# n00b001/neuro-genetic-pong-self-play

Hardware: AMD Instinct MI355X
Metric: env-steps/sec (GA evaluation loop, self-play) + generations/sec at pop=65536 per GPU (higher is better)
Workload: dtype f32 hidden + certified f64 argmax; genomes f64

## Files before the change

### include/pong_ga.h

```cpp
#ifndef PONG_GA_H
#define PONG_GA_H

#include <stddef.h>
#include <stdint.h>

#ifdef __cplusplus
extern "C" {
#endif

#define PG_ABI_VERSION 13
#define PG_MAX_NODES 9

typedef enum pg_status {
  PG_OK = 0,
  PG_ERR_INVALID = -1,
  PG_ERR_HIP = -2,
  PG_ERR_UNSUPPORTED = -3
} pg_status;

typedef enum pg_dtype { PG_F32 = 0, PG_F64 = 1 } pg_dtype;

typedef enum pg_activation {
  PG_ACT_SIGMOID = 0,
  PG_ACT_RELU = 1
} pg_activation;

typedef enum pg_opp_kind {
  PG_OPP_HARDCODED = 0,
  PG_OPP_ROM_CPU = 1,
  PG_OPP_SCORE = 2,
  PG_OPP_NN = 3
} pg_opp_kind;

typedef enum pg_precision {
  PG_PREC_CERTIFIED = 0,
  PG_PREC_F64 = 1
} pg_precision;

typedef enum pg_kernel {
  PG_KERNEL_AUTO = 0,
  PG_KERNEL_GENERAL = 1,
  PG_KERNEL_RESIDENT = 2,
  PG_KERNEL_SPLIT = 3      ,
  PG_KERNEL_WIDE = 4,
  PG_KERNEL_STAGED = 5,
  PG_KERNEL_RELU = 6
} pg_kernel;

typedef enum pg_prep {
  PG_PREP_ALL = 0,
  PG_PREP_GENOMES = 1,
  PG_PREP_REST = 2
} pg_prep;

typedef struct pg_net {
  int32_t n_nodes;
  int32_t nodes[PG_MAX_NODES];
  int32_t bias;
  int32_t dtype;
  int32_t activation;
} pg_net;

typedef struct pg_eval_args {
  uint32_t struct_size;
  pg_net net;
  int32_t n_genomes;
  int32_t n_games;
  const void *genomes;
  int64_t genome_stride;
  const void *opponents;
  int64_t opponent_stride;
  int32_t n_opponents;
  int32_t precision;
  const int32_t *game_kind;
  const int32_t *game_opp;
  const double *game_mult;
  uint64_t seed;
  double *fitness;
  double *rewards;
  int32_t *scores;
  int32_t *frames;
  double *total_frames;
  int32_t *status;
  uint64_t *counters;
  uint8_t *trace;
  int32_t trace_games;
  int32_t trace_cap;
  int32_t kernel;
  int32_t group_lanes;
  void *workspace;
  size_t workspace_bytes;
  uint32_t *hard_log;
  int32_t hard_cap;
  const int32_t *genome_rows;
  const int32_t *n_active;
  int32_t prep;
  int32_t horizon;
  int32_t timeout_thresh;
  int32_t win_score;
} pg_eval_args;


typedef struct pg_forward_args {
  pg_net net;
  int32_t n;
  const void *genomes;
  int64_t genome_stride;
  const int32_t *genome_index;
  const double *x;
  int32_t precision;
  int32_t *index;
  double *act;
  uint64_t *counters;
  double *z_all;
  double *h_all;
} pg_forward_args;

typedef struct pg_decide_args {
  pg_net net;
  int32_t n;
  const void *genomes;
  int64_t genome_stride;
  const int32_t *genome_index;
  const int32_t *k;
  int32_t *index;
  int32_t *stage;
} pg_decide_args;

typedef struct pg_wide_decide_args {
  pg_net net;
  int32_t n;
  const void *genomes;
  int64_t genome_stride;
  const int32_t *genome_index;
  const int32_t *k;
  int32_t *index;
  double *act;
  void *workspace;
  size_t workspace_bytes;
} pg_wide_decide_args;

typedef struct pg_relu_decide_args {
  pg_net net;
  int32_t n;
  const void *genomes;
  int64_t genome_stride;
  const int32_t *genome_index;
  const int32_t *k;
  int32_t *index;
  int32_t *stage;
  float *z32;
  float *bound;
} pg_relu_decide_args;

enum {
  PG_S_BALL_X = 0, PG_S_BALL_Y, PG_S_BALL_VX, PG_S_BALL_VY, PG_S_BALL_VISIBLE,
  PG_S_SERVE_TIMER, PG_S_SERVE_DIR, PG_S_HITS, PG_S_POINT, PG_S_LEFT_Y, PG_S_RIGHT_Y,
  PG_S_SCORE1, PG_S_SCORE2, PG_S_ONE_PLAYER, PG_S_SEED_LO, PG_S_SEED_HI,
  PG_STATE_FIELDS
};

typedef struct pg_ga_args {
  int32_t n;
  int64_t genes;
  int32_t dtype;
  const void *parents;
  int64_t stride;
  int32_t n_parents;
  const int32_t *chosen;
  void *offspring;
  uint8_t *invalid;
  double cxpb, mutpb;
  double alpha;
  double mu, sigma, indpb;
  uint64_t seed;
  uint64_t generation;
  const uint8_t *pair_mask;
  const int32_t *pair_list;
  const int32_t *pair_count;
  int32_t pair_cap;
} pg_ga_args;

typedef struct pg_select_args {
  int32_t n_pop;
  int32_t k;
  int32_t tournsize;
  const double *fitness;
  int32_t *chosen;
  uint64_t seed;
  uint64_t generation;
} pg_select_args;

typedef enum pg_schedule_mode {
  PG_SCHED_REFERENCE = 0,
  PG_SCHED_SELFPLAY = 1
} pg_schedule_mode;

typedef struct pg_schedule_args {
  int32_t mode;
  int32_t n;
  int32_t n_games;
  int64_t row_offset;
  int32_t n_hof;
  const double *hof_fitness;
  uint64_t seed;
  uint64_t generation;
  int32_t *kind;
  int32_t *opp;
  double *mult;
  const int32_t *rows;
  int32_t hof_slices;
  int32_t block_rows;
  int32_t slice_local;
} pg_schedule_args;

typedef struct pg_hof_args {
  int32_t maxsize;
  int32_t hof_n;
  const double *hof_fitness;
  const uint64_t *hof_hash;
  int32_t pop_n;
  const double *pop_fitness;
  const uint64_t *pop_hash;
  const int32_t *rank;
  int32_t *new_n;
  int32_t *new_src;
  double *new_fitness;
} pg_hof_args;

typedef struct pg_hof_packed_args {
  int32_t maxsize;
  int32_t hof_n;
  const double *hof_fitness;
  int32_t k;
  const int64_t *packed;
  int32_t *new_n;
  int32_t *new_src;
  double *new_fitness;
  const int32_t *slot_in;
  int32_t *slot_out;
} pg_hof_packed_args;
int32_t pg_hof_update_packed(const pg_hof_packed_args *args);

typedef struct pg_hof_rank_args {
  int32_t hof_n;
  const double *hof_fitness;
  const uint64_t *hof_hash;
  int32_t k;
  const double *cand_fitness;
  const uint64_t *cand_hash;
  int64_t *packed;
  void *workspace;
  size_t workspace_bytes;
} pg_hof_rank_args;

typedef struct pg_hof_prepare_args {
  const double *fitness;
  int32_t pop_n;
  int32_t filter;
  double worst;
  const void *rows;
  int64_t stride;
  int64_t genes;
  int32_t dtype;
  int32_t hof_n;
  const double *hof_fitness;
  const uint64_t *hof_hash;
  int32_t *k;
  int64_t *cand;
  uint64_t *hashes;
  int64_t *packed;
  void *workspace;
  size_t workspace_bytes;
} pg_hof_prepare_args;

const char *pg_version(void);
int32_t pg_abi_version(void);
int32_t pg_build_flags(void);
const char *pg_last_error(void);
int32_t pg_device_count(void);
size_t pg_eval_workspace_bytes(const pg_eval_args *args);
int32_t pg_gene_count(const pg_net *net);

int32_t pg_eval_population(const pg_eval_args *args, void *stream);
int32_t pg_forward(const pg_forward_args *args, void *stream);
int32_t pg_decide(const pg_decide_args *args, void *stream);
size_t pg_wide_decide_workspace_bytes(const pg_wide_decide_args *args);
int32_t pg_wide_decide(const pg_wide_decide_args *args, void *stream);
int32_t pg_relu_decide(const pg_relu_decide_args *args, void *stream);
int32_t pg_physics_reset(int32_t *state, int32_t n, const uint64_t *seeds,
                         const int32_t *one_player, void *stream);
int32_t pg_physics_step(int32_t *state, int32_t n, const uint8_t *actions, void *stream);
int32_t pg_ga_select_tournament(const pg_select_args *args, void *stream);
int32_t pg_ga_select_tournament_ranked(const pg_select_args *args, const double *sorted_fitness,
                                       const int32_t *order, void *stream);
int32_t pg_ga_vary(const pg_ga_args *args, void *stream);
int32_t pg_ga_mark_pairs(uint8_t *pair_mask, int32_t n_pairs, const int32_t *rows, int32_t n_rows,
                         int32_t skip_lo, int32_t skip_hi, const uint8_t *exclude, void *stream);
int32_t pg_ga_list_pairs(const uint8_t *pair_mask, int32_t n_pairs, int32_t *list, int32_t *count, void *stream);
int32_t pg_ga_schedule(const pg_schedule_args *args, void *stream);
int32_t pg_row_hash(const void *rows, int64_t stride, const int32_t *index, int32_t n, int64_t genes,
                    int32_t dtype, uint64_t *hash, void *stream);
int32_t pg_hof_update(const pg_hof_args *args);
size_t pg_hof_rank_classes_workspace_bytes(int32_t n);
int32_t pg_hof_rank_classes(const pg_hof_rank_args *args, void *stream);
size_t pg_hof_prepare_workspace_bytes(int32_t hof_n, int32_t pop_n);
int32_t pg_hof_prepare(const pg_hof_prepare_args *args, void *stream);

typedef struct pg_scatter_args {
  int32_t n;
  int32_t n_games;
  int32_t row_lo;
  const double *fitness;
  const int32_t *frames;
  const int32_t *rows;
  const int32_t *n_active;
  double *shard_fitness;
  float *lineage;
} pg_scatter_args;
int32_t pg_ga_scatter_fitness(const pg_scatter_args *args, void *stream);

typedef struct pg_merge_args {
  int32_t pop_n;
  const double *fitness;
  const uint8_t *invalid;
  const double *inherited;
  double *new_fitness;
  int32_t filter;
  double worst;
  int32_t *cand;
  double *cand_fitness;
  double *summary;
  void *workspace;
  size_t workspace_bytes;
} pg_merge_args;
size_t pg_ga_merge_workspace_bytes(int32_t pop_n);
int32_t pg_ga_merge_fitness(const pg_merge_args *args, void *stream);

size_t pg_ga_select_workspace_bytes(int32_t n_pop);
int32_t pg_ga_select_ranked(const pg_select_args *args, void *workspace, size_t workspace_bytes, void *stream);

int32_t pg_ga_inherit(const int32_t *chosen, int32_t n, const double *fitness, double *inherited,
                      const float *lineage_in, float *lineage_out, void *stream);

size_t pg_ga_order_workspace_bytes(int32_t n);
int32_t pg_ga_order(int32_t n, int32_t row_lo, const uint8_t *invalid, const float *lineage, int32_t by_length,
                    int32_t *rows, int32_t *count, void *workspace, size_t workspace_bytes, void *stream);

typedef struct pg_hof_cand_args {
  int32_t hof_n;
  const double *hof_fitness;
  const uint64_t *hof_hash;
  int32_t k;
  const int32_t *cand;
  const double *cand_fitness;
  const void *rows;
  int64_t stride;
  int64_t genes;
  int32_t dtype;
  uint64_t *cand_hash;
  int64_t *packed;
  void *workspace;
  size_t workspace_bytes;
} pg_hof_cand_args;
size_t pg_hof_prepare_cand_workspace_bytes(int32_t hof_n, int32_t k);
int32_t pg_hof_prepare_cand(const pg_hof_cand_args *args, void *stream);

typedef struct pg_hof_commit_args {
  void *dst;
  int64_t dst_stride;
  const void *old_rows;
  int64_t old_stride;
  const void *rows;
  int64_t rows_stride;
  const int32_t *cand;
  const int32_t *src;
  int32_t n_old;
  int32_t m;
  int64_t genes;
  int32_t dtype;
  const uint64_t *old_hash;
  const uint64_t *cand_hash;
  uint64_t *new_hash;
  const double *fitness_in;
  double *new_fitness;
  const int32_t *dst_slot;
} pg_hof_commit_args;
int32_t pg_hof_commit(const pg_hof_commit_args *args, void *stream);

int32_t pg_gather_rows(void *dst, int64_t dst_stride, const void *old_rows, int64_t old_stride, const void *rows,
                       int64_t rows_stride, const int64_t *index, const int32_t *src, int32_t n_old, int32_t n,
                       int64_t genes, int32_t dtype, void *stream);
int32_t pg_render_frames(const int32_t *state, int32_t n, uint8_t *frames, void *stream);
int32_t pg_find_stuff(const uint8_t *frames, int64_t frame_stride, int32_t n, double *out, void *stream);

#ifdef __cplusplus
}
#endif
#endif
```

### neuro-genetic-pong-self-play_amd/csrc/pg_cascade.hpp

```cpp
#pragma once

#include <hip/hip_runtime.h>
#include <stdint.h>

#include "pg_device.hpp"
#include "pg_eval.hpp"
#include "pg_f64math.h"

namespace pg {

#ifndef PG_SLOW_INLINE
#define PG_SLOW_INLINE __forceinline__
#endif
#ifndef PG_LOAD_BATCH
#define PG_LOAD_BATCH 2
#endif
#ifndef PG_RES_WAVES
#define PG_RES_WAVES 0
#endif
#if PG_RES_WAVES > 0
#define PG_RES_BOUNDS __launch_bounds__(256, PG_RES_WAVES)
#else
#define PG_RES_BOUNDS __launch_bounds__(256)
#endif
// ... 211 lines not shown

template <int U, int O>
__device__ __forceinline__ void load_rec_out(NetP<U, O> &n, const float *__restrict__ r) {
  constexpr int P = NetP<U, O>::P;
  constexpr int F = rec_floats<U, O>();
  constexpr int B = P * 14 / 4 * 4;
  constexpr int D = P * 14 - B;
  const float4 *s = reinterpret_cast<const float4 *>(r + B);
  float v[F - B];
#pragma unroll
  for (int q = 0; q < (F - B) / 4; ++q) {
    const float4 x = s[q];
    v[4 * q] = x.x;
    v[4 * q + 1] = x.y;
    v[4 * q + 2] = x.z;
    v[4 * q + 3] = x.w;
  }
#pragma unroll
  for (int p = 0; p < P; ++p)
#pragma unroll
    for (int o = 0; o < O; ++o) n.w2[p][o] = float2v{v[D + (p * O + o) * 2], v[D + (p * O + o) * 2 + 1]};
#pragma unroll
  for (int o = 0; o < O; ++o) n.c[o] = v[D + P * O * 2 + o];
  n.e = v[D + P * O * 2 + O];
  n.ct = make_cert(n.e);
}

template <int U, int O>
__device__ __forceinline__ void load_rec(NetP<U, O> &n, const float *__restrict__ r) {
  constexpr int P = NetP<U, O>::P;
  constexpr int F = rec_floats<U, O>();
  const float4 *s = reinterpret_cast<const float4 *>(r);
  float v[F];
#pragma unroll
  for (int q = 0; q < F / 4; ++q) {
    const float4 x = s[q];
    v[4 * q] = x.x;
    v[4 * q + 1] = x.y;
    v[4 * q + 2] = x.z;
    v[4 * q + 3] = x.w;
  }
#pragma unroll
  for (int p = 0; p < P; ++p)
#pragma unroll
    for (int i = 0; i < 7; ++i) n.w1[p][i] = float2v{v[(p * 7 + i) * 2], v[(p * 7 + i) * 2 + 1]};
#pragma unroll
  for (int p = 0; p < P; ++p)
#pragma unroll
    for (int o = 0; o < O; ++o) n.w2[p][o] = float2v{v[P * 14 + (p * O + o) * 2], v[P * 14 + (p * O + o) * 2 + 1]};
#pragma unroll
  for (int o = 0; o < O; ++o) n.c[o] = v[P * 14 + P * O * 2 + o];
  n.e = v[P * 14 + P * O * 2 + O];
  n.ct = make_cert(n.e);
}

template <int U, int O, bool kBiasIn = false>
__device__ __forceinline__ void partial_pk(const NetP<U, O> &n, const int k[6], float acc[O]) {
  constexpr int P = NetP<U, O>::P;
  float2v kx[6];
#pragma unroll
  for (int i = 0; i < 6; ++i) {
    const float f = (float)k[i];
    kx[i] = float2v{f, f};
  }
  float2v a2[O];
#pragma unroll
  for (int o = 0; o < O; ++o) a2[o] = kBiasIn ? float2v{n.c[o], n.c[o]} : float2v{0.f, 0.f};
#pragma unroll
  for (int p = 0; p < P; p += 2) {
    constexpr int kStep = 2;
    const bool two = p + 1 < P;
    float2v a = n.w1[p][6], b = two ? n.w1[p + 1][6] : float2v{0.f, 0.f};
#pragma unroll
    for (int i = 0; i < 6; ++i) {
      a = __builtin_elementwise_fma(n.w1[p][i], kx[i], a);
      if (two) b = __builtin_elementwise_fma(n.w1[p + 1][i], kx[i], b);
    }
    const float2v qa = float2v{__builtin_amdgcn_exp2f(a.x), __builtin_amdgcn_exp2f(a.y)} + 1.0f;
    const float2v qb = float2v{__builtin_amdgcn_exp2f(b.x), __builtin_amdgcn_exp2f(b.y)} + 1.0f;
    const float2v sa = float2v{__builtin_amdgcn_rcpf(qa.x), __builtin_amdgcn_rcpf(qa.y)};
    const float2v sb = float2v{__builtin_amdgcn_rcpf(qb.x), __builtin_amdgcn_rcpf(qb.y)};
#pragma unroll
    for (int o = 0; o < O; ++o) {
      a2[o] = __builtin_elementwise_fma(n.w2[p][o], sa, a2[o]);
      if (two) a2[o] = __builtin_elementwise_fma(n.w2[p + 1][o], sb, a2[o]);
    }
    (void)kStep;
  }
#pragma unroll
  for (int o = 0; o < O; ++o) acc[o] = a2[o].x + a2[o].y;
}

template <int HL, int U, int O>
__device__ __forceinline__ float frame_bound_wave(const float *__restrict__ rec, const int k[6], int lane64) {
  constexpr int P = NetP<U, O>::P;
  constexpr int F = rec_floats<U, O>();
  constexpr float kOR = (float)out_roundings<HL, U>();
  float acc[O];
#pragma unroll
  for (int o = 0; o < O; ++o) acc[o] = 0.f;
#pragma unroll 1
  for (int t = lane64; t < HL * 2 * P; t += 64) {
    const int hl = t % HL, u = t / HL, p = u >> 1, h = u & 1;
    const float *r = rec + hl * F;
    float w[7];
#pragma unroll
// ... 516 lines not shown
```

### neuro-genetic-pong-self-play_amd/csrc/pg_eval.hpp

```cpp
#pragma once

#include <hip/hip_runtime.h>
#include <stdint.h>

#include "../../include/pong_ga.h"
#include "pg_device.hpp"

namespace pg {

int32_t fail(int32_t code, const char *fmt, ...);

#define PG_HIP(call)                                                                  \
  do {                                                                                \
    hipError_t e_ = (call);                                                           \
    if (e_ != hipSuccess)                                                             \
      return fail(PG_ERR_HIP, "%s failed: %s", #call, hipGetErrorString(e_));        \
  } while (0)

struct EvalParams {
  const void *genomes;
  const void *opponents;
  const int32_t *rows;
  const int32_t *n_active;
  const int32_t *kind;
  const int32_t *opp;
  const double *mult;
  double *rewards;
  int32_t *scores;
  int32_t *frames;
  double *total_frames;
  int32_t *status_game;
  uint64_t *counters;
  uint8_t *trace;
  uint32_t *hard_log;
  int hard_cap;
  unsigned int *work;
  int64_t gstride, ostride;
  uint64_t seed;
  int n_genomes, n_games, total, n_opponents;
  int trace_games, trace_cap;
  int nodes[PG_MAX_NODES];
  int n_nodes, bias, max_width;
  float *recs;
  int horizon;
  int timeout_thresh;
  int win_score;
  int prep;
  void *wide_scratch;
  int wide_w3_resident;
  const int32_t *wide_probe_k;
  int32_t *wide_probe_index;
  double *wide_probe_act;
  int activation;
};

__device__ inline int active_genomes(const EvalParams &p) {
  if (!p.n_active) return p.n_genomes;
  const int a = __builtin_amdgcn_readfirstlane(*p.n_active);
  return a < 0 ? 0 : (a < p.n_genomes ? a : p.n_genomes);
}
__device__ inline int active_total(const EvalParams &p) {
  return p.n_active ? active_genomes(p) * p.n_games : p.total;
}

__device__ inline int genome_row(const EvalParams &p, int i) { return p.rows ? p.rows[i] : i; }

template <class S>
__device__ inline double episode_reward(const S &st, int total, double mult, int &zero_div) {
  zero_div = 0;
  if (st.s1 == st.s2) return 0.0;
  const double tf = (double)total;
  if (tf == 0.0) {
    zero_div = 1;
    return __builtin_nan("");
  }
  const double diff = (double)(st.s2 - st.s1);
  const double bonus = __dmul_rn((double)st.s2, mult);
  return __dadd_rn(diff, bonus) / (tf / 100.0);
}

template <class S>
__device__ inline void finish_game(const EvalParams &p, int w, const S &st, int frames, int total) {
  int zero_div;
  const double reward = episode_reward(st, total, p.mult[w], zero_div);
  p.rewards[w] = reward;
  p.scores[2 * w] = st.s1;
  p.scores[2 * w + 1] = st.s2;
  p.frames[w] = frames;
  p.total_frames[w] = (double)total;
  p.status_game[w] = zero_div;
}

__device__ inline double feat64(int k) { return __dmul_rn(0.5, (double)k) / 160.0; }
__device__ inline double feat64_flip(int k) { return (160.0 - __dmul_rn(0.5, (double)k)) / 160.0; }


int num_cus();

__device__ inline void log_hard_raw(uint32_t *hard_log, uint64_t *counters, int hard_cap, int row, int is_opp, int idx,
                                    int source, const int k[6]) {
  if (!hard_log || !counters) return;
  const unsigned long long r = atomicAdd((unsigned long long *)&counters[9], 1ull);
  if (r >= (unsigned long long)hard_cap) return;
  uint32_t *rec = hard_log + r * 8;
  rec[0] = (uint32_t)row;
  rec[1] = (uint32_t)(is_opp & 1) | ((uint32_t)(idx & 255) << 8) | ((uint32_t)(source & 255) << 16);
  for (int i = 0; i < 6; ++i) rec[2 + i] = (uint32_t)k[i];
}
__device__ inline void log_hard(const EvalParams &p, int row, int is_opp, int idx, int source, const int k[6]) {
  log_hard_raw(p.hard_log, p.counters, p.hard_cap, row, is_opp, idx, source, k);
}

struct DecideParams {
  const void *genomes;
  const int32_t *gidx;
  const int32_t *k;
  int32_t *index;
  int32_t *stage;
  int64_t gstride;
  int n, H, b;
};
int32_t launch_decide(const DecideParams &p, int L, int O, bool f64, size_t lds, hipStream_t s);

bool wide_shape_ok(const pg_net &n, int n_games);
size_t wide_workspace_bytes(const pg_eval_args *a);
int32_t launch_wide(const EvalParams &p, int dtype, void *scratch, hipStream_t s);

bool relu_shape_ok(const pg_net &n);
int32_t launch_relu(const EvalParams &p, int dtype, hipStream_t s);


}
```

### neuro-genetic-pong-self-play_amd/csrc/pg_gen.hip

```cpp
#include <hip/hip_runtime.h>

#include <algorithm>

#include <rocprim/device/device_radix_sort.hpp>

#include "pg_eval.hpp"


namespace pg {
namespace {

constexpr int kT = 256;
constexpr int kChunk = 8 * kT;
inline unsigned blocks(long n, int per = kT) { return (unsigned)((n + per - 1) / per); }
inline size_t align_up(size_t x) { return (x + 255) & ~size_t(255); }

__global__ void k_scatter_fitness(pg_scatter_args a) {
  const int i = blockIdx.x * kT + threadIdx.x;
  if (i >= a.n) return;
  const int played = a.n_active ? __builtin_amdgcn_readfirstlane(*a.n_active) : a.n;
  const int row = a.rows ? a.rows[i] : a.row_lo + i;
  const bool p = i < played;
  a.shard_fitness[row - a.row_lo] = p ? a.fitness[i] : 0.0;
  if (p && a.lineage) {
    int m = 0;
    for (int g = 0; g < a.n_games; ++g) m = max(m, a.frames[(long)i * a.n_games + g]);
    a.lineage[row] = (float)m;
  }
}

struct Part {
  double n, mean, m2, mn, mx;
  int32_t nan, nevals, cand, pad;
};

__device__ inline void chan(double &n, double &mean, double &m2, double nb, double meanb, double m2b) {
  if (nb == 0.0) return;
  if (n == 0.0) {
    n = nb, mean = meanb, m2 = m2b;
    return;
  }
  const double t = n + nb, d = meanb - mean;
  mean += d * (nb / t);
  m2 += m2b + d * d * (n * nb / t);
  n = t;
}

__device__ inline void part_merge(Part &x, const Part &y) {
  chan(x.n, x.mean, x.m2, y.n, y.mean, y.m2);
  x.mn = fmin(x.mn, y.mn);
  x.mx = fmax(x.mx, y.mx);
  x.nan |= y.nan;
  x.nevals += y.nevals;
  x.cand += y.cand;
}

__device__ inline bool is_cand(const pg_merge_args &a, double f) { return !a.filter || f > a.worst; }

__device__ inline double merged(const pg_merge_args &a, int i) {
// ... 206 lines not shown
    packed[hn + j] = (int64_t)(uint32_t)rank | ((int64_t)cls << 32);
    return;
  }
  packed[e] = (int64_t)(uint32_t)rank | ((int64_t)cls << 32);
}

unsigned table_cap(int n) {
  unsigned c = 64;
  while (c < 2u * (unsigned)(n > 0 ? n : 1)) c <<= 1;
  return c;
}

struct CandLayout {
  size_t mt, ct, sort_keys, sort_vals, sort_temp, total, temp_bytes;
  unsigned mcap, ccap;
};

int32_t cand_layout(int hn, int k, CandLayout *L) {
  size_t tb = 0;
  if (rocprim::radix_sort_pairs(nullptr, tb, (const double *)nullptr, (double *)nullptr, (const int32_t *)nullptr,
                                (int32_t *)nullptr, (unsigned)(k > 0 ? k : 1)) != hipSuccess)
    return fail(PG_ERR_HIP, "hof_prepare_cand: rocPRIM storage query failed");
  L->mcap = table_cap(hn);
  L->ccap = table_cap(k);
  size_t off = 0;
  auto take = [&](size_t b) {
    const size_t at = off;
    off += align_up(b);
    return at;
  };
  L->mt = take((size_t)(L->mcap + 1) * sizeof(Slot));
  L->ct = take((size_t)(L->ccap + 1) * sizeof(Slot));
  const size_t kk = (size_t)(k > 0 ? k : 1);
  L->sort_keys = take(kk * 8 * 2);
  L->sort_vals = take(kk * 4 * 2);
  L->temp_bytes = tb > 0 ? tb : 1;
  L->sort_temp = take(L->temp_bytes);
  L->total = off;
  return PG_OK;
}

__global__ void k_iota(int32_t *v, int n) {
  const int i = blockIdx.x * kT + threadIdx.x;
  if (i < n) v[i] = i;
}

__global__ void k_cand_keys(const double *f, int k, double *keys, int32_t *iota) {
  const int i = blockIdx.x * kT + threadIdx.x;
  if (i >= k) return;
  keys[i] = f[i] + 0.0;
  iota[i] = i;
}

template <typename WT>
__global__ __launch_bounds__(256) void k_hof_commit(WT *dst, int64_t dst_stride, const WT *old_rows, int64_t old_stride,
                                                    const WT *rows, int64_t rows_stride, const int32_t *cand,
                                                    const int32_t *src, int m, int n_old, int64_t genes,
                                                    const uint64_t *old_hash, const uint64_t *cand_hash,
                                                    uint64_t *new_hash, const double *fit_in, double *new_fitness,
                                                    const int32_t *dst_slot) {
  const int lane = threadIdx.x & 63;
  for (int j = blockIdx.x * 4 + (threadIdx.x >> 6); j < m; j += gridDim.x * 4) {
    const int s = src[j];
    if (!dst_slot || s >= n_old) {
      const WT *from = s < n_old ? old_rows + (long)s * old_stride : rows + (long)cand[s - n_old] * rows_stride;
      WT *to = dst + (long)(dst_slot ? dst_slot[j] : j) * dst_stride;
      for (int64_t g = lane; g < genes; g += 64) to[g] = from[g];
    }
    if (lane == 0) {
      new_hash[j] = s < n_old ? old_hash[s] : cand_hash[s - n_old];
      new_fitness[j] = fit_in[j];
    }
  }
}

}
}

using namespace pg;

extern "C" {

int32_t pg_ga_scatter_fitness(const pg_scatter_args *a, void *stream) {
  if (!a) return fail(PG_ERR_INVALID, "args is NULL");
  if (a->n < 0 || a->n_games < 1 || a->row_lo < 0 || (a->n > 0 && (!a->fitness || !a->shard_fitness)) ||
      (a->n > 0 && a->lineage && !a->frames))
    return fail(PG_ERR_INVALID, "ga_scatter_fitness: bad sizes or NULL buffers");
  if (a->n == 0) return PG_OK;
  hipLaunchKernelGGL(k_scatter_fitness, dim3(blocks(a->n)), dim3(kT), 0, (hipStream_t)stream, *a);
  PG_HIP(hipGetLastError());
  return PG_OK;
}

size_t pg_ga_merge_workspace_bytes(int32_t pop_n) {
  if (pop_n < 0) return 0;
  const size_t nb = blocks(pop_n > 0 ? pop_n : 1, kChunk);
  return align_up(nb * sizeof(Part)) + align_up(nb * sizeof(int32_t));
}

int32_t pg_ga_merge_fitness(const pg_merge_args *a, void *stream) {
  if (!a) return fail(PG_ERR_INVALID, "args is NULL");
  const int n = a->pop_n;
  if (n < 0 || !a->summary || (n > 0 && (!a->fitness || !a->new_fitness || !a->cand || !a->cand_fitness)) ||
      (n > 0 && a->invalid && !a->inherited))
    return fail(PG_ERR_INVALID, "ga_merge_fitness: bad sizes or NULL buffers");
  const size_t need = pg_ga_merge_workspace_bytes(n);
  if (!a->workspace || a->workspace_bytes < need)
    return fail(PG_ERR_INVALID, "ga_merge_fitness: workspace of %zu bytes needed", need);
  const unsigned nb = blocks(n > 0 ? n : 1, kChunk);
  Part *parts = (Part *)a->workspace;
  int32_t *offsets = (int32_t *)((char *)a->workspace + align_up(nb * sizeof(Part)));
  const hipStream_t s = (hipStream_t)stream;
  hipLaunchKernelGGL(k_merge_partials, dim3(nb), dim3(kT), 0, s, *a, parts);
  hipLaunchKernelGGL(k_merge_finish, dim3(1), dim3(64), 0, s, *a, (const Part *)parts, (int)nb, offsets);
  hipLaunchKernelGGL(k_merge_compact, dim3(nb), dim3(kT), 0, s, *a, (const int32_t *)offsets);
  PG_HIP(hipGetLastError());
  return PG_OK;
}

size_t pg_ga_select_workspace_bytes(int32_t n_pop) {
// ... 65 lines not shown
  hipLaunchKernelGGL(k_order_keys, dim3(blocks(n)), dim3(kT), 0, s, (int)n, (int)row_lo, invalid, lineage,
                     (int)by_length, keys, vals, count);
  PG_HIP(rocprim::radix_sort_pairs(temp, tb, keys, keys_out, vals, rows, (unsigned)n, 0, 32, s));
  return PG_OK;
}

size_t pg_hof_prepare_cand_workspace_bytes(int32_t hof_n, int32_t k) {
  CandLayout L;
  if (hof_n < 0 || k < 0 || cand_layout(hof_n, k, &L) != PG_OK) return 0;
  return L.total;
}

int32_t pg_hof_prepare_cand(const pg_hof_cand_args *a, void *stream) {
  if (!a) return fail(PG_ERR_INVALID, "args is NULL");
  const int hn = a->hof_n, k = a->k;
  if (hn < 0 || k < 0 || (long)hn + k > 0x7fffffffL || (hn > 0 && (!a->hof_fitness || !a->hof_hash)) ||
      (k > 0 && (!a->cand || !a->cand_fitness || !a->rows || !a->cand_hash || !a->packed)) || a->genes < 0 ||
      (k > 0 && a->stride < a->genes) || (a->dtype != PG_F32 && a->dtype != PG_F64))
    return fail(PG_ERR_INVALID, "hof_prepare_cand: bad sizes, dtype or NULL buffers");
  if (k == 0) return PG_OK;
  CandLayout L;
  if (cand_layout(hn, k, &L) != PG_OK) return PG_ERR_HIP;
  if (!a->workspace || a->workspace_bytes < L.total)
    return fail(PG_ERR_INVALID, "hof_prepare_cand: workspace of %zu bytes needed", L.total);
  char *ws = (char *)a->workspace;
  const hipStream_t s = (hipStream_t)stream;
  const int32_t rc = pg_row_hash(a->rows, a->stride, a->cand, k, a->genes, a->dtype, a->cand_hash, stream);
  if (rc != PG_OK) return rc;
  Slot *mt = (Slot *)(ws + L.mt), *ct = (Slot *)(ws + L.ct);
  PG_HIP(hipMemsetAsync(ws + L.mt, 0xFF, L.ct + (size_t)(L.ccap + 1) * sizeof(Slot) - L.mt, s));
  hipLaunchKernelGGL(k_hof_insert, dim3(blocks(hn + k)), dim3(kT), 0, s, a->hof_hash, hn, mt, L.mcap,
                     a->cand_hash, k, ct, L.ccap);
  double *keys = (double *)(ws + L.sort_keys), *sorted = keys + k;
  int32_t *iota = (int32_t *)(ws + L.sort_vals), *order = iota + k;
  hipLaunchKernelGGL(k_cand_keys, dim3(blocks(k)), dim3(kT), 0, s, a->cand_fitness, k, keys, iota);
  size_t tb = L.temp_bytes;
  PG_HIP(rocprim::radix_sort_pairs(ws + L.sort_temp, tb, (const double *)keys, sorted, iota, order, (unsigned)k, 0, 64,
                                   s));
  hipLaunchKernelGGL(k_hof_rank_pack, dim3(blocks(hn + k)), dim3(kT), 0, s, a->hof_fitness,
                     a->hof_hash, hn, a->cand_fitness, a->cand_hash, k,
                     (const double *)sorted, (const int32_t *)order, (const Slot *)mt, L.mcap, (const Slot *)ct,
                     L.ccap, a->packed);
  PG_HIP(hipGetLastError());
  return PG_OK;
}

int32_t pg_hof_commit(const pg_hof_commit_args *a, void *stream) {
  if (!a) return fail(PG_ERR_INVALID, "args is NULL");
  if (a->m < 0 || a->n_old < 0 || a->genes < 0 || (a->dtype != PG_F32 && a->dtype != PG_F64) ||
      (a->m > 0 && (!a->dst || !a->src || !a->new_hash || !a->fitness_in || !a->new_fitness)) ||
      (a->m > 0 && a->n_old > 0 && ((!a->old_rows && !a->dst_slot) || !a->old_hash)) ||
      (a->m > 0 && (!a->rows || !a->cand || !a->cand_hash)))
    return fail(PG_ERR_INVALID, "hof_commit: bad sizes, dtype or NULL buffers");
  if (a->m == 0) return PG_OK;
  const hipStream_t s = (hipStream_t)stream;
  const dim3 grid((unsigned)std::min<int64_t>(((int64_t)a->m + 3) / 4, 2048));
  if (a->dtype == PG_F64)
    hipLaunchKernelGGL(k_hof_commit<double>, grid, dim3(256), 0, s, (double *)a->dst, a->dst_stride,
                       (const double *)a->old_rows, a->old_stride, (const double *)a->rows, a->rows_stride, a->cand,
                       a->src, (int)a->m, a->n_old, a->genes, a->old_hash, a->cand_hash,
                       a->new_hash, a->fitness_in, a->new_fitness, a->dst_slot);
  else
    hipLaunchKernelGGL(k_hof_commit<float>, grid, dim3(256), 0, s, (float *)a->dst, a->dst_stride,
                       (const float *)a->old_rows, a->old_stride, (const float *)a->rows, a->rows_stride, a->cand,
                       a->src, (int)a->m, a->n_old, a->genes, a->old_hash, a->cand_hash,
                       a->new_hash, a->fitness_in, a->new_fitness, a->dst_slot);
  PG_HIP(hipGetLastError());
  return PG_OK;
}

}
```

### neuro-genetic-pong-self-play_amd/csrc/pg_service.hpp

```cpp
#pragma once

#include <hip/hip_runtime.h>

#include "../../include/pong_ga.h"
#include "pg_cascade.hpp"
#include "pg_device.hpp"
#include "pg_eval.hpp"
#include "pg_f64math.h"

namespace pg {

#ifndef PG_SVC_PRIO
#define PG_SVC_PRIO 3
#endif
#ifndef PG_SVC_BATCH
#define PG_SVC_BATCH 1
#endif

#ifndef PG_INLINE_SVC
#define PG_INLINE_SVC 1
#endif
#ifndef PG_INLINE_PRIO
#define PG_INLINE_PRIO 3
#endif
// ... 48 lines not shown
  uint64_t st_t = __builtin_amdgcn_s_memtime();
  const auto stage_mark = [&](int i) {
    asm volatile("s_waitcnt vmcnt(0) lgkmcnt(0)" ::: "memory");
    const uint64_t now = __builtin_amdgcn_s_memtime();
    st_acc[i] += now - st_t;
    st_acc[6 + i] += 1;
    st_t = now;
  };
#define PG_STAGE(i) stage_mark(i)
#else
#define PG_STAGE(i)
#endif
  int d = PG_INLINE_FRAME_BOUND ? -1 : plateau_decide<O>(zf, r.e, lane64);
  PG_STAGE(0);
  if (d >= 0) PG_LOG_REQ(1, d);
  if (PG_INLINE_FRAME_BOUND && d < 0 && r.e < __builtin_inff()) {
    const float ef = fminf(r.e, frame_bound_wave<HL, U, O>(r.rec, r.kr, lane64));
#ifdef PG_INLINE_LOG
    ef_log = ef;
#endif
    PG_STAGE(1);
    d = certify_c<O>(zf, make_cert(ef));
    if (d < 0) d = plateau_f32<O>(zf, ef);
    if (d < 0) d = plateau_decide<O>(zf, ef, lane64);
    PG_STAGE(2);
    if (d >= 0) {
      PG_LOG_REQ(2, d);
      return d | 1024;
    }
  }
  if (d < 0) {
    d = fast_f64_decide<O, WT>(g, H, b, r.k, lane64);
    PG_STAGE(3);
    if (d >= 0) PG_LOG_REQ(3, d);
  }
  if (d >= 0) return d | 512;
  d = forward_f64_group<64, (U * HL + 63) / 64, O, WT>(g, H, b, r.k, lds, lane64);
  PG_LOG_REQ(4, d);
  PG_STAGE(4);
#undef PG_LOG_REQ
#undef PG_STAGE
#if defined(PG_INLINE_LOG) || defined(PG_SERVE_STAGES)
  if (false) {
#else
  if (p.hard_log && lane64 == 0) {
#endif
    const long oo = g - (const WT *)p.opponents;
    const bool opp = p.opponents != p.genomes && oo >= 0 && oo < (long)p.n_opponents * p.ostride;
    log_hard(p, (int)(opp ? oo / p.ostride : (g - (const WT *)p.genomes) / p.gstride), opp ? 1 : 0, d, 0, r.k);
  }
  return d | 256;
}

template <int L, int U, int O, typename WT>
__global__ __launch_bounds__(256) void k_prep_records(EvalParams p) {
  constexpr int HL = L / 2;
  constexpr int F = rec_floats<U, O>();
  if (p.prep != PG_PREP_GENOMES && blockIdx.x == 0) {
    if (threadIdx.x < 64) p.work[threadIdx.x] = 0u;
    if (p.counters && threadIdx.x < 16) p.counters[threadIdx.x] = 0ull;
  }
  const long t = (long)blockIdx.x * 256 + threadIdx.x;
  const long net = t / HL + (p.prep == PG_PREP_REST ? p.n_genomes : 0);
  const int hl = (int)(t % HL);
  const long end = p.prep == PG_PREP_GENOMES ? (long)p.n_genomes : (long)p.n_genomes + p.n_opponents;
  if (net >= end) return;
  const WT *g;
  int flip;
  if (net < p.n_genomes) {
    if (net >= active_genomes(p)) return;
    g = (const WT *)p.genomes + (long)genome_row(p, (int)net) * p.gstride;
    flip = 0;
  } else {
    g = (const WT *)p.opponents + (net - p.n_genomes) * p.ostride;
    flip = 1;
  }
  NetP<U, O> n;
  load_net_pk<HL, U, O, WT>(n, g, p.nodes[1], p.bias, hl, flip);
  store_rec<U, O>(n, p.recs + (net * HL + hl) * F);
}

#ifdef PG_PROBE_EXTRA
template <int M>
__device__ __forceinline__ void pg_probe_extra(float2v w, float2v w2, float a, float b, float &v, float2v &pp,
                                               int &sv) {
#pragma unroll
  for (int r = 0; r < (M == 4 || M == 9 ? 48 : (M <= 2 ? 16 : 24)); ++r) {
    if constexpr (M == 1) asm volatile("v_rcp_f32 %0, %1" : "=v"(v) : "v"((r & 1) ? a : b));
    if constexpr (M == 2) asm volatile("v_exp_f32 %0, %1" : "=v"(v) : "v"((r & 1) ? a : b));
    if constexpr (M == 3) asm volatile("v_pk_fma_f32 %0, %1, %2, %3" : "=v"(pp) : "v"(w), "v"(w2), "v"((r & 1) ? w : w2));
    if constexpr (M == 4) asm volatile("v_fma_f32 %0, %1, %2, %3" : "=v"(v) : "v"(a), "v"(b), "v"((r & 1) ? a : b));
    if constexpr (M == 5) asm volatile("v_add_u32 %0, %1, %2" : "=v"(v) : "v"(a), "v"(b));
    if constexpr (M == 7) asm volatile("v_mov_b32 %0, %1" : "=v"(v) : "v"((r & 1) ? a : b));
    if constexpr (M == 8) asm volatile("v_pk_add_f32 %0, %1, %2" : "=v"(pp) : "v"(w), "v"((r & 1) ? w : w2));
    if constexpr (M == 9) asm volatile("v_add_f32 %0, %1, %2" : "=v"(v) : "v"(a), "v"((r & 1) ? a : b));
  }
}
#endif

template <int L, int U, int O, typename WT, bool kUntraced = false, bool kHorizon = false>
__global__ __launch_bounds__(svc_threads<U>()) void k_service(EvalParams p) {
  constexpr int kSvcThreads = svc_threads<U>();
  constexpr bool kInline = inline_service<L, U, kHorizon>();
  static_assert(!kInline || O <= 4, "InlineReq.z");
  constexpr int kSvcGameWaves = kSvcThreads / 64 - (kInline ? 0 : 1);
  constexpr int HL = L / 2;
  constexpr int kSlots = kSvcGameWaves * (64 / L) * 2;
  __shared__ SlowSlot slots[kSlots];
  __shared__ HorizonSlot hz[kHorizon ? kSlots / 2 : 1];
  __shared__ int waves_done;
  __shared__ int posted;
  __shared__ uint32_t serve_tab[kServeTabSlots * kServeTabPoints];
  extern __shared__ double lds_svc[];
  const int H = p.nodes[1];
  const int b = p.bias;
  const int wave = threadIdx.x >> 6;
  const int lane64 = threadIdx.x & 63;
  for (int i = threadIdx.x; i < kSlots; i += kSvcThreads) {
    lds_st(&slots[i].flag, 0);
    slots[i].rec = 0;
  }
  const bool tabbed = p.n_games <= kServeTabSlots;
  if (tabbed)
    for (int i = threadIdx.x; i < p.n_games * kServeTabPoints; i += kSvcThreads)
      serve_tab[i] = Pong::serve_entry(game_seed(p.seed, i / kServeTabPoints), i % kServeTabPoints);
  if (threadIdx.x == 0) {
    lds_st(&waves_done, 0);
    lds_st(&posted, 0);
  }
  __syncthreads();

  if (!kInline && wave == kSvcGameWaves) {
// ... 123 lines not shown
    tend = 0x7fffffff;
    fstart = 0x3fffffff;
    fresh = false;
  };
  if (kInline && !live) park();
  int w_scripted = 1, w_onep = 1;
  int top = 1;
#ifdef PG_PROBE_EXTRA
  float probe_v = 0.f;
  float2v probe_p = float2v{0.f, 0.f};
  int probe_s = 0;
#endif
#ifdef PG_START_PROBE
  uint64_t probe_fresh = 0;
  const uint64_t probe_t0 = __builtin_amdgcn_s_memtime();
#endif
#ifdef PG_SERVE_STAGES
  uint64_t st_acc[24];
#pragma unroll
  for (int i = 0; i < 24; ++i) st_acc[i] = 0;
#endif
#ifdef PG_DECIDE_PROBE
  uint64_t probe_dec = 0;
  const uint64_t probe_t0 = __builtin_amdgcn_s_memtime();
#endif
#ifdef PG_TIMELINE
  uint64_t t_start = 0;
  uint32_t g_fails = 0, g_slow = 0;
#endif
#ifdef PG_PATH_PROBE
  uint32_t pp_frames = 0, pp_rally = 0, pp_face = 0, pp_fail = 0, pp_hidden = 0;
#define PG_PP(cnt, cond) \
  if (__builtin_amdgcn_ballot_w64(cond) != 0) cnt += 1
#else
#define PG_PP(cnt, cond)
#endif
  if (kInline ? __builtin_amdgcn_ballot_w64(live) != 0 : live) for (;;) {
#ifdef PG_START_PROBE
    const bool any_fresh = __builtin_amdgcn_ballot_w64(fresh) != 0;
    const uint64_t probe_f0 = __builtin_amdgcn_s_memtime();
#endif
    PG_PP(pp_frames, true);
    sframe += 1;
#ifdef PG_TIMELINE
    constexpr bool kJumps = !kHorizon;
#else
    const bool kJumps = !kHorizon && (kUntraced || p.trace == nullptr);
#endif
    if (top) {
    if (fresh) {
      const int i = w / p.n_games;
      const int g = w - i * p.n_games;
      kind = p.kind[w];
      const WT *gr = genomes + (long)genome_row(p, i) * p.gstride;
      const bool nn = side && kind == kOppNN && p.n_opponents > 0;
      const int oj = nn ? min(max(p.opp[w], 0), p.n_opponents - 1) : 0;
      gm = nn ? opponents + (long)oj * p.ostride : gr;
      const int rec = nn ? p.n_genomes + oj : i;
      load_rec<U, O>(net, p.recs + ((long)rec * HL + hl) * rec_floats<U, O>());
      const int sx = slot_me();
      if (kInline && hl == 0) slots[sx].rec = rec;
#pragma unroll
      for (int o = 0; o < O; ++o) net.c[o] = hl == 0 ? 0.5f * net.c[o] : 0.f;
      st.reset(0, kind == kOppRomCpu);
      if (kHorizon || !tabbed) st.seed = game_seed(p.seed, g);
      tab_off = g * kServeTabPoints;
      act_r = act_l = total = 0;
      c_vis = kVisByFrames ? sframe - 1 : 0;
      fstart = sframe - 1;
      tend = sframe + p.timeout_thresh;
      fresh = false;
      if (hl == 0) slots[sx].n_memo = 0;
      if (lig == 0) slots[sx].rally_at = -1;
      if (kHorizon && lig == 0) {
        const int gx = threadIdx.x / L;
        hz[gx].sum = 0.0;
        hz[gx].eps = hz[gx].s1 = hz[gx].s2 = hz[gx].zd = 0;
      }
#ifdef PG_TIMELINE
      t_start = wall_clock64();
      g_fails = g_slow = 0;
#endif
    }
#ifdef PG_START_PROBE
    if (any_fresh) probe_fresh += __builtin_amdgcn_s_memtime() - probe_f0;
#endif
#ifndef PG_NO_HIDDEN_JUMP
    {
      const bool hid = !st.vis && st.timer >= 2;
      PG_PP(pp_hidden, hid);
      if (kJumps && hid) {
        const int h = st.timer - 1;
        st.rc2 = PongK::drift2(st.rc2, h);
        if (!st.one_player) st.lc2 = PongK::drift2(st.lc2, h);
        st.timer = 1;
        act_r = clamp_move(st.rc2, 0);
        act_l = clamp_move(st.lc2, 0);
        fstart -= h;
        tend -= h;
        hidden += h;
      }
    }
#endif
    w_scripted = __builtin_amdgcn_readfirstlane(__builtin_amdgcn_ballot_w64(kind != kOppNN) != 0);
    w_onep = __builtin_amdgcn_readfirstlane(__builtin_amdgcn_ballot_w64(st.one_player != 0) != 0);
    top = 0;
    }
    const int pvis = st.vis, pbx2 = st.bx2, pby2 = st.by2;
#ifdef PG_PATH_PROBE
    const int pt_b = st.point, hits_b = st.hits;
#endif
    const int ev = st.step(act_r, act_l, [&](int pt) {
// ... 27 lines not shown
      if (PG_ANY(code == -1)) {
      if (code == -1) {
        fails += 1;
#ifdef PG_TIMELINE
        g_fails += 1;
#endif
#ifndef PG_NO_TIGHT
        int mv = tight_gap_move<O>(z, net.e, net.ct);
        if (mv == -1)
#else
        int mv = -1;
#endif
        {
          const int idx = plateau_f32<O>(z, net.e);
          mv = idx >= 0 ? index_to_move(idx) : -1;
        }
        inwave += mv != -1 ? 1 : 0;
        code = mv;
      }
#ifdef PG_ABLATE_SERVE
      if (code == -1) code = z[1] > z[0] ? 6 : -6;
#endif
      if (kInline && PG_ANY(code == -1)) {
        uint64_t key = 0;
        int nm = 0;
        const int sx = slot_me();
        if (code == -1) {
          key = memo_key(k);
          nm = slots[sx].n_memo;
          int hit = -1;
#pragma unroll 1
          for (int c = 0; c < kMemo && c < nm; ++c)
            if (slots[sx].memo_key[c] == key) hit = slots[sx].memo_idx[c];
          code = hit;
        }
        const int kn[6] = {side ? 320 - bx2 : bx2, by2, side ? 320 - lbx2 : lbx2, lby2, side ? lc2 : rc2,
                           side ? rc2 : lc2};
        const float my_e = net.e;
        uint64_t need = __builtin_amdgcn_ballot_w64(code == -1 && hl == 0);
        if (need) {
#ifdef PG_DECIDE_PROBE
        const uint64_t probe_d0 = __builtin_amdgcn_s_memtime();
#endif
        if constexpr (PG_INLINE_PRIO > 0) __builtin_amdgcn_s_setprio(PG_INLINE_PRIO);
#pragma unroll 1
        do {
          const int src = (int)__builtin_ctzll(need);
          need &= need - 1;
          InlineReq r;
#pragma unroll
          for (int i = 0; i < 6; ++i) r.k[i] = __builtin_amdgcn_readlane(kn[i], src);
#pragma unroll
          for (int i = 0; i < 6; ++i) r.kr[i] = __builtin_amdgcn_readlane(k[i], src);
          r.rec = p.recs + (long)__builtin_amdgcn_readlane(slots[sx].rec, src) * HL * rec_floats<U, O>();
#pragma unroll
          for (int o = O; o < 4; ++o) r.z[o] = 0.f;
#pragma unroll
          for (int o = 0; o < O; ++o) r.z[o] = __int_as_float(__builtin_amdgcn_readlane(__float_as_int(z[o]), src));
          r.e = __int_as_float(__builtin_amdgcn_readlane(__float_as_int(my_e), src));
          const uint64_t ga = (uint64_t)gm;
          const WT *g = (const WT *)(((uint64_t)__builtin_amdgcn_readlane((int)(ga >> 32), src) << 32) |
                                     (uint32_t)__builtin_amdgcn_readlane((int)(uint32_t)ga, src));
#if defined(PG_SERVE_TWICE)
          serve_inline<U, HL, O, WT>(p, g, r, lds_svc + wave * f64_lds_doubles(H, O), lane64, st_acc);
          const int ans = serve_inline<U, HL, O, WT>(p, g, r, lds_svc + wave * f64_lds_doubles(H, O), lane64, st_acc + 12);
#elif defined(PG_SERVE_STAGES)
          const int ans = serve_inline<U, HL, O, WT>(p, g, r, lds_svc + wave * f64_lds_doubles(H, O), lane64, st_acc);
#else
          const int ans = serve_inline<U, HL, O, WT>(p, g, r, lds_svc + wave * f64_lds_doubles(H, O), lane64);
#endif
          if ((lane64 & ~(HL - 1)) == src) {
            slow += (ans >> 8) & 1;
            plateau += (ans >> 9) & 1;
            inwave += ans >> 10;
            code = index_to_move(ans & 255);
            if (hl == 0) {
              const int c = nm % kMemo;
              slots[sx].memo_key[c] = key;
              slots[sx].memo_idx[c] = code;
              slots[sx].n_memo = nm + 1;
            }
          }
        } while (need);
        if constexpr (PG_INLINE_PRIO > 0) __builtin_amdgcn_s_setprio(0);
        {
#if defined(PG_RELOAD_ALL)
          load_rec<U, O>(net, p.recs + ((long)slots[sx].rec * HL + hl) * rec_floats<U, O>());
#elif !defined(PG_NO_RELOAD)
          load_rec_out<U, O>(net, p.recs + ((long)slots[sx].rec * HL + hl) * rec_floats<U, O>());
#endif
#ifndef PG_NO_RELOAD
#pragma unroll
          for (int o = 0; o < O; ++o) net.c[o] = hl == 0 ? 0.5f * net.c[o] : 0.f;
#endif
#ifdef PG_SERVE_STAGES
          {
            const uint64_t r0 = __builtin_amdgcn_s_memtime();
            asm volatile("s_waitcnt vmcnt(0) lgkmcnt(0)" ::: "memory");
            st_acc[5] += __builtin_amdgcn_s_memtime() - r0;
            st_acc[11] += 1;
          }
#endif
#ifdef PG_DECIDE_PROBE
          asm volatile("s_waitcnt vmcnt(0)" ::: "memory");
          probe_dec += __builtin_amdgcn_s_memtime() - probe_d0;
#endif
        }
        }
      }
      if (!kInline && PG_ANY(code == -1) && code == -1) {
        const int sx = slot_me();
        const uint64_t key = memo_key(k);
        const int nm = slots[sx].n_memo;
        int hit = -1;
#pragma unroll 1
        for (int c = 0; c < kMemo && c < nm; ++c)
          if (slots[sx].memo_key[c] == key) hit = slots[sx].memo_idx[c];
        if (hit != -1) {
          code = hit;
        } else {
          if (hl == 0) {
            const int kn[6] = {side ? 320 - bx2 : bx2, by2, side ? 320 - lbx2 : lbx2, lby2, side ? lc2 : rc2,
                               side ? rc2 : lc2};
            slots[sx].g = gm;
#pragma unroll
            for (int i = 0; i < 6; ++i) slots[sx].k[i] = kn[i];
#pragma unroll
            for (int o = 0; o < O; ++o) slots[sx].z[o] = z[o];
            slots[sx].e = net.e;
            __threadfence_block();
            lds_st(&slots[sx].flag, 1);
            __hip_atomic_fetch_add(&posted, 1, __ATOMIC_RELAXED, __HIP_MEMORY_SCOPE_WORKGROUP);
          }
          while (lds_ld(&slots[sx].flag) != 2) __builtin_amdgcn_s_sleep(1);
          __threadfence_block();
          const int ans = slots[sx].idx;
          slow += (ans >> 8) & 1;
#ifdef PG_TIMELINE
          g_slow += 1;
#endif
          plateau += ans >> 9;
          code = index_to_move(ans & 255);
// ... 155 lines not shown
    if (lig == 0) {
      atomicAdd((unsigned long long *)&p.counters[0], (unsigned long long)(c_steps - skipped - hidden));
      if (hidden) atomicAdd((unsigned long long *)&p.counters[12], (unsigned long long)hidden);
      atomicAdd((unsigned long long *)&p.counters[1], (unsigned long long)c_fwd);
      atomicAdd((unsigned long long *)&p.counters[3], (unsigned long long)c_games);
      if (skipped) atomicAdd((unsigned long long *)&p.counters[8], (unsigned long long)skipped);
    }
    if (hl == 0 && slow) atomicAdd((unsigned long long *)&p.counters[2], (unsigned long long)slow);
    if (hl == 0 && fails) atomicAdd((unsigned long long *)&p.counters[4], (unsigned long long)fails);
    if (hl == 0 && plateau) atomicAdd((unsigned long long *)&p.counters[5], (unsigned long long)plateau);
    if (hl == 0 && inwave) atomicAdd((unsigned long long *)&p.counters[6], (unsigned long long)inwave);
  }
#ifdef PG_DECIDE_PROBE
  if (p.counters && lane64 == 0) {
    atomicAdd((unsigned long long *)&p.counters[13], (unsigned long long)probe_dec);
    atomicAdd((unsigned long long *)&p.counters[14], (unsigned long long)(__builtin_amdgcn_s_memtime() - probe_t0));
    atomicAdd((unsigned long long *)&p.counters[15], 1ull);
  }
#endif
#ifdef PG_START_PROBE
  if (p.counters && lane64 == 0) {
    atomicAdd((unsigned long long *)&p.counters[13], (unsigned long long)probe_fresh);
    atomicAdd((unsigned long long *)&p.counters[14], (unsigned long long)(__builtin_amdgcn_s_memtime() - probe_t0));
    atomicAdd((unsigned long long *)&p.counters[15], 1ull);
  }
#endif
#ifdef PG_PATH_PROBE
  if (p.counters && lane64 == 0) {
    atomicAdd((unsigned long long *)&p.counters[11], (unsigned long long)pp_frames);
    atomicAdd((unsigned long long *)&p.counters[10], (unsigned long long)pp_rally);
    atomicAdd((unsigned long long *)&p.counters[13], (unsigned long long)pp_face);
    atomicAdd((unsigned long long *)&p.counters[14], (unsigned long long)pp_fail);
    atomicAdd((unsigned long long *)&p.counters[15], (unsigned long long)pp_hidden);
  }
#endif
#ifdef PG_PROBE_EXTRA
  if (p.counters && probe_v == 1234.5f && probe_p.x == 1234.5f && probe_s == 1234567) p.counters[15] = 1;
#endif
#ifdef PG_SERVE_STAGES
  if (p.hard_log && lane64 == 0)
#pragma unroll
    for (int i = 0; i < 24; ++i)
      if (st_acc[i]) atomicAdd((unsigned long long *)&((uint64_t *)p.hard_log)[i], (unsigned long long)st_acc[i]);
#endif
  if (lane64 == 0) atomicAdd(&waves_done, 1);
}

inline size_t service_records_bytes(int n_genomes, int n_opponents, int L, int U, int O) {
  const int F = ((U + 1) / 2 * 2 * (7 + O) + O + 1 + 3) / 4 * 4;
  return ((size_t)n_genomes + (size_t)(n_opponents > 0 ? n_opponents : 0)) * (size_t)(L / 2) * F * sizeof(float);
}

template <int L, int U, int O, typename WT, bool kSplitTrace = false>
inline int32_t launch_service(const EvalParams &p, hipStream_t s) {
  constexpr int kSvcThreads = svc_threads<U>();
  const bool inl = p.horizon > 0 ? inline_service<L, U, true>() : inline_service<L, U, false>();
  const int GPB = (kSvcThreads / 64 - (inl ? 0 : 1)) * (64 / L);
  const size_t lds = (size_t)f64_lds_doubles(p.nodes[1], O) * sizeof(double) * (inl ? kSvcThreads / 64 : 1);
  const int want = (p.total + GPB - 1) / GPB;
  const int cap = num_cus() * 2;
  const int grid = want < cap ? want : cap;
  if (grid <= 0) return PG_OK;
  if (!p.recs) return fail(PG_ERR_INVALID, "split kernel: no lane-record workspace");
  if (!kSplitTrace && p.horizon > 0)
    return fail(PG_ERR_UNSUPPORTED, "horizon mode: [6, 33..64, 3] networks on 8-lane groups only");
  const long nets = p.prep == PG_PREP_GENOMES ? (long)p.n_genomes
                   : (p.prep == PG_PREP_REST ? (long)p.n_opponents : (long)p.n_genomes + p.n_opponents);
  const long prep_threads = nets * (L / 2);
  const unsigned prep_blocks = (unsigned)((prep_threads + 255) / 256);
  hipLaunchKernelGGL((k_prep_records<L, U, O, WT>), dim3(prep_blocks > 0 ? prep_blocks : 1u), dim3(256), 0, s, p);
  if (p.prep == PG_PREP_GENOMES) {
    PG_HIP(hipGetLastError());
    return PG_OK;
  }
  if (kSplitTrace && p.horizon > 0)
    hipLaunchKernelGGL((k_service<L, U, O, WT, true, true>), dim3(grid), dim3(kSvcThreads), lds, s, p);
  else if (kSplitTrace && !p.trace)
    hipLaunchKernelGGL((k_service<L, U, O, WT, true>), dim3(grid), dim3(kSvcThreads), lds, s, p);
  else
    hipLaunchKernelGGL((k_service<L, U, O, WT, false>), dim3(grid), dim3(kSvcThreads), lds, s, p);
  PG_HIP(hipGetLastError());
  return PG_OK;
}

int32_t launch_service_more(const EvalParams &p, int L, int O, bool f64, hipStream_t s);

inline int service_units(int L, int H) {
  if (L == 8 && H > 32 && H <= 64) return 16;
  for (int u = 1; u <= 8; u *= 2)
    if ((L / 2) * u >= H) return u;
  return 0;
}

}
```

### neuro-genetic-pong-self-play_amd/csrc/pong_ga.hip

```cpp
#include <hip/hip_runtime.h>

#include <cmath>
#include <cstdarg>
#include <cstdio>
#include <cstring>
#include <string>
#include <algorithm>
#include <memory>
#include <unordered_map>
#include <utility>
#include <vector>

#include "../../include/pong_ga.h"
#include "pg_device.hpp"
#include "pg_eval.hpp"
#include "pg_f64math.h"
#include "pg_cascade.hpp"
#include "pg_service.hpp"

#ifndef PG_VERSION_STRING
#define PG_VERSION_STRING "pong_ga 0.1.0 (gfx950)"
#endif

namespace pg {
// ... 259 lines not shown
}

__device__ __forceinline__ double u01(uint64_t seed, uint64_t gen, uint64_t stream, uint64_t a,
                                      uint64_t b) {
  uint64_t k = splitmix64(seed + 0x9E3779B97F4A7C15ull * (gen + 1));
  k = splitmix64(k ^ (stream * 0xD6E8FEB86659FD93ull + a));
  k = splitmix64(k ^ b);
  return (double)(k >> 11) * 0x1.0p-53;
}

__global__ void k_select(pg_select_args a) {
  const int j = blockIdx.x * blockDim.x + threadIdx.x;
  if (j >= a.k) return;
  int best = -1;
  double bf = 0.0;
  for (int t = 0; t < a.tournsize; ++t) {
    const int idx = (int)(u01(a.seed, a.generation, 1, (uint64_t)j, (uint64_t)t) * (double)a.n_pop);
    const double f = a.fitness[idx];
    if (best < 0 || f > bf) {
      best = idx;
      bf = f;
    }
  }
  a.chosen[j] = best;
}

__global__ void k_select_ranked(pg_select_args a, const double *sorted, const int32_t *order) {
  const int j = blockIdx.x * blockDim.x + threadIdx.x;
  if (j >= a.k) return;
  const int n = a.n_pop;
  const double v = u01(a.seed, a.generation, 8, (uint64_t)j, 0);
  int r = (int)((double)n * exp(log(v) / (double)a.tournsize));
  r = r < 0 ? 0 : (r > n - 1 ? n - 1 : r);
  const double f = sorted[r];
  int lo = 0, hi = n;
  int a0 = 0, b0 = r;
  while (a0 < b0) { const int m = (a0 + b0) >> 1; if (sorted[m] < f) a0 = m + 1; else b0 = m; }
  lo = a0;
  a0 = r; b0 = n;
  while (a0 < b0) { const int m = (a0 + b0) >> 1; if (sorted[m] <= f) a0 = m + 1; else b0 = m; }
  hi = a0;
  const int pick = lo + (int)(u01(a.seed, a.generation, 9, (uint64_t)j, 0) * (double)(hi - lo));
  a.chosen[j] = order[pick < hi ? pick : hi - 1];
}

__device__ __forceinline__ uint64_t rng_key(uint64_t seed, uint64_t gen, uint64_t stream, uint64_t a) {
  const uint64_t k = splitmix64(seed + 0x9E3779B97F4A7C15ull * (gen + 1));
  return splitmix64(k ^ (stream * 0xD6E8FEB86659FD93ull + a));
}
__device__ __forceinline__ double rng_u01(uint64_t key, uint64_t b) {
  return (double)(splitmix64(key ^ b) >> 11) * 0x1.0p-53;
}

template <typename WT>
__device__ __forceinline__ void vary_pair(const pg_ga_args &a, int pair);

template <typename WT>
__global__ __launch_bounds__(256) void k_vary(pg_ga_args a) {
  const int wave = (int)blockIdx.x * 4 + __builtin_amdgcn_readfirstlane((int)(threadIdx.x >> 6));
  if (a.pair_list) {
    const int count = __builtin_amdgcn_readfirstlane(*a.pair_count);
    const int waves = (int)gridDim.x * 4;
#pragma unroll 1
    for (int w = wave; w < count; w += waves) vary_pair<WT>(a, __builtin_amdgcn_readfirstlane(a.pair_list[w]));
    return;
  }
  vary_pair<WT>(a, wave);
}

template <typename WT>
__device__ __forceinline__ void vary_pair(const pg_ga_args &a, int pair) {
  const int pairs = (a.n + 1) / 2;
  if (pair >= pairs) return;
  const int lane = threadIdx.x & 63;
  const int i0 = 2 * pair, i1 = 2 * pair + 1;
  const bool has1 = i1 < a.n;
  const bool cx = has1 && rng_u01(rng_key(a.seed, a.generation, 2, (uint64_t)pair), 0) < a.cxpb;
  const bool mut0 = rng_u01(rng_key(a.seed, a.generation, 4, (uint64_t)i0), 0) < a.mutpb;
  const bool mut1 = has1 && rng_u01(rng_key(a.seed, a.generation, 4, (uint64_t)i1), 0) < a.mutpb;
  if (lane == 0) {
    a.invalid[i0] = (uint8_t)(cx || mut0);
    if (has1) a.invalid[i1] = (uint8_t)(cx || mut1);
  }
  if (!a.pair_list && a.pair_mask && !a.pair_mask[pair]) return;
  const uint64_t k3 = rng_key(a.seed, a.generation, 3, (uint64_t)pair);
  const uint64_t k5 = rng_key(a.seed, a.generation, 5, (uint64_t)pair);
  const uint64_t k6 = rng_key(a.seed, a.generation, 6, (uint64_t)pair);
  const WT *p1 = (const WT *)a.parents + (long)a.chosen[i0] * a.stride;
  const WT *p2 = (const WT *)a.parents + (long)(has1 ? a.chosen[i1] : a.chosen[i0]) * a.stride;
  WT *o1 = (WT *)a.offspring + (long)i0 * a.stride;
  WT *o2 = (WT *)a.offspring + (long)i1 * a.stride;
  const auto one = [&](long gene, double x1, double x2) {
    if (cx) {
      const double u = rng_u01(k3, (uint64_t)gene);
      const double gamma = __dadd_rn(__dmul_rn(1.0 + 2.0 * a.alpha, u), -a.alpha);
      const double y1 = __dadd_rn(__dmul_rn(1.0 - gamma, x1), __dmul_rn(gamma, x2));
      const double y2 = __dadd_rn(__dmul_rn(gamma, x1), __dmul_rn(1.0 - gamma, x2));
      x1 = y1;
      x2 = y2;
    }
    const uint64_t hb = splitmix64(k5 ^ (uint64_t)gene);
    const bool h0 = mut0 && (double)(uint32_t)hb * 0x1.0p-32 < a.indpb;
    const bool h1 = mut1 && (double)(uint32_t)(hb >> 32) * 0x1.0p-32 < a.indpb;
    if (h0 || h1) {
      const uint64_t nb = splitmix64(k6 ^ (uint64_t)gene);
      const float u1 = 1.0f - (float)(nb >> 40) * 0x1.0p-24f;
      const float u2 = (float)((nb >> 8) & 0xFFFFFFu) * 0x1.0p-24f;
      const float r = sqrtf(-2.0f * logf(u1));
      float sn, cs;
      sincosf(6.2831853f * u2, &sn, &cs);
      if (h0) x1 = __dadd_rn(x1, __dadd_rn(a.mu, __dmul_rn(a.sigma, (double)(r * cs))));
      if (h1) x2 = __dadd_rn(x2, __dadd_rn(a.mu, __dmul_rn(a.sigma, (double)(r * sn))));
    }
    o1[gene] = (WT)x1;
    if (has1) o2[gene] = (WT)x2;
  };
  constexpr int kVaryChunk = 4;
  for (long g0 = 0; g0 < a.genes; g0 += 128 * kVaryChunk) {
    double x[kVaryChunk][2][2];
#pragma unroll
    for (int c = 0; c < kVaryChunk; ++c) {
#pragma unroll
      for (int h = 0; h < 2; ++h) {
        const long g = g0 + c * 128 + h * 64 + lane;
        const bool v = g < a.genes;
        x[c][h][0] = v ? (double)p1[g] : 0.0;
        x[c][h][1] = v && has1 ? (double)p2[g] : 0.0;
      }
    }
#pragma unroll
    for (int c = 0; c < kVaryChunk; ++c) {
#pragma unroll
      for (int h = 0; h < 2; ++h) {
        const long g = g0 + c * 128 + h * 64 + lane;
        if (g < a.genes) one(g, x[c][h][0], x[c][h][1]);
      }
    }
  }
}

__global__ void k_mark_pairs(uint8_t *mask, int n_pairs, const int32_t *rows, int n_rows, int skip_lo, int skip_hi,
                             const uint8_t *exclude) {
  const int i = blockIdx.x * blockDim.x + threadIdx.x;
  if (i >= n_rows) return;
  const int r = rows[i];
  if (r < 0 || r >= 2 * n_pairs) return;
  const int j = r >> 1;
  if ((j < skip_lo || j >= skip_hi) && !(exclude && exclude[j])) mask[j] = 1;
}

__global__ void k_list_pairs(const uint8_t *mask, int n_pairs, int32_t *list, int32_t *count) {
  const int j = blockIdx.x * blockDim.x + threadIdx.x;
  if (j < n_pairs && mask[j]) list[atomicAdd(count, 1)] = j;
}

__global__ void k_schedule(pg_schedule_args a) {
  const long w = (long)blockIdx.x * blockDim.x + threadIdx.x;
  if (w >= (long)a.n * a.n_games) return;
  const long i = w / a.n_games;
  const int g = (int)(w % a.n_games);
  const long row = a.rows ? (long)a.rows[i] : a.row_offset + i;
  int kind = kOppHard, opp = 0;
  double mult = 1.0;
  if (a.mode == PG_SCHED_SELFPLAY) {
    if (a.n_hof > 0) {
      kind = kOppNN;
      const int K = a.hof_slices > 1 && a.n_hof >= a.hof_slices ? a.hof_slices : 1;
      if (K == 1) {
        opp = (int)((row * a.n_games + g) % a.n_hof);
      } else {
        const int b = (int)((row / a.block_rows) % K);
        const long m = (a.n_hof - b + K - 1) / K;
        const int k = (int)((row * a.n_games + g) % m);
        opp = a.slice_local ? k : k * K + b;
      }
    }
  } else if (g < 3) {
    kind = g == 0 ? kOppHard : (g == 1 ? kOppRomCpu : kOppScore);
  } else if (a.n_hof > 0) {
    kind = kOppNN;
    opp = (int)(u01(a.seed, a.generation, 10, (uint64_t)row, (uint64_t)g) * (double)a.n_hof);
    opp = opp < a.n_hof ? opp : a.n_hof - 1;
    mult = a.hof_fitness[opp];
  }
  a.kind[w] = kind;
  a.opp[w] = opp;
  a.mult[w] = mult;
}

template <typename WT>
// ... 97 lines not shown
  return 64;
}

template <typename WT>
static int32_t launch_service_any(const EvalParams &p, int L, int O, hipStream_t s) {
  const int H = p.nodes[1];
#ifdef PG_DEV_MIN
  const bool here = L == 8 && H <= 64;
#else
  const bool here = L == 8 && H > 32 && H <= 64;
#endif
  if (here && O == 3) return launch_service<8, 16, 3, WT, true>(p, s);
#ifdef PG_DEV_MIN
  return fail(PG_ERR_UNSUPPORTED, "no service kernel for L=%d H=%d O=%d", L, H, O);
#else
  return launch_service_more(p, L, O, sizeof(WT) == 8, s);
#endif
}


template <int L, int U, int O, typename WT>
static int32_t launch_fwd_resident(const FwdParams &p, hipStream_t s) {
  constexpr int GPB = 256 / L;
  const size_t lds = (size_t)GPB * f64_lds_doubles(p.nodes[1], O) * sizeof(double);
  const int want = (p.n + GPB - 1) / GPB;
  const int cap = num_cus() * 8;
  const int grid = want < cap ? want : cap;
  if (grid <= 0) return PG_OK;
  hipLaunchKernelGGL((k_forward_resident<L, U, O, WT>), dim3(grid), dim3(256), lds, s, p);
  PG_HIP(hipGetLastError());
  return PG_OK;
}

template <typename WT>
static int32_t launch_fwd_resident_any(const FwdParams &p, ResidentChoice c, int O, hipStream_t s) {
#define PG_FRES(LL, UU)                                                  \
  if (c.L == LL && c.U == UU) {                                          \
    if (O == 2) return launch_fwd_resident<LL, UU, 2, WT>(p, s);         \
    if (O == 3) return launch_fwd_resident<LL, UU, 3, WT>(p, s);         \
    if (O == 4) return launch_fwd_resident<LL, UU, 4, WT>(p, s);         \
  }
#ifndef PG_DEV_MIN
  PG_FRES(4, 1) PG_FRES(8, 1) PG_FRES(16, 1) PG_FRES(32, 1) PG_FRES(64, 1)
  PG_FRES(16, 2) PG_FRES(32, 2) PG_FRES(64, 2) PG_FRES(16, 4) PG_FRES(32, 4) PG_FRES(64, 4)
#endif
#undef PG_FRES
  return fail(PG_ERR_UNSUPPORTED, "no resident forward kernel for L=%d U=%d O=%d", c.L, c.U, O);
}

static bool resident_shape_ok(const pg_net &n) {
  return n.n_nodes == 3 && n.nodes[0] == 6 && n.nodes[1] <= 256 && n.nodes[2] >= 2 && n.nodes[2] <= 4;
}

}

using namespace pg;

extern "C" {

const char *pg_version(void) { return PG_VERSION_STRING; }
int32_t pg_abi_version(void) { return PG_ABI_VERSION; }
int32_t pg_build_flags(void) { return 0; }
const char *pg_last_error(void) { return g_last_error.c_str(); }

int32_t pg_device_count(void) {
  int n = 0;
  hipError_t e = hipGetDeviceCount(&n);
  if (e != hipSuccess) return fail(PG_ERR_HIP, "hipGetDeviceCount: %s", hipGetErrorString(e));
  return n;
}

static size_t eval_base_workspace(const pg_eval_args *a) {
  const size_t games = a ? (size_t)(a->n_genomes > 0 ? a->n_genomes : 0) * (size_t)(a->n_games > 0 ? a->n_games : 0) : 0;
  return 256 + ((games * sizeof(int32_t) + 255) / 256) * 256;
}

static int resolve_kernel(const pg_eval_args *a) {
  if (a->kernel != PG_KERNEL_AUTO) return a->kernel;
  if (a->net.activation == PG_ACT_RELU)
    return relu_shape_ok(a->net) && a->precision == PG_PREC_CERTIFIED ? PG_KERNEL_RELU : PG_KERNEL_GENERAL;
  if (resident_shape_ok(a->net) && a->precision == PG_PREC_CERTIFIED) return PG_KERNEL_SPLIT;
  if (wide_shape_ok(a->net, a->n_games) && (a->net.nodes[1] >= 64 || a->net.nodes[2] >= 64)) return PG_KERNEL_WIDE;
  return PG_KERNEL_GENERAL;
}

static size_t split_records_bytes(const pg_eval_args *a) {
  if (!resident_shape_ok(a->net) || a->n_genomes <= 0) return 0;
  const int H = a->net.nodes[1];
  const int L = a->group_lanes > 0 ? a->group_lanes : choose_split_lanes(H);
  const int U = (L == 8 && H <= 64) ? 16 : service_units(L, H);
  if (U <= 0) return 0;
  return (service_records_bytes(a->n_genomes, a->opponents ? a->n_opponents : 0, L, U, a->net.nodes[2]) + 255) /
         256 * 256;
}

static int32_t check_struct_size(const pg_eval_args *a) {
  if (a->struct_size != sizeof(pg_eval_args))
    return fail(PG_ERR_INVALID, "pg_eval_args.struct_size=%u, this library's struct is %zu bytes (ABI %d)",
                a->struct_size, sizeof(pg_eval_args), PG_ABI_VERSION);
  return PG_OK;
}

size_t pg_eval_workspace_bytes(const pg_eval_args *a) {
  if (a && check_struct_size(a) != PG_OK) return 0;
  size_t n = eval_base_workspace(a);
  if (!a) return n;
  const int kernel = resolve_kernel(a);
  if (kernel == PG_KERNEL_SPLIT) n += split_records_bytes(a);
  if (kernel == PG_KERNEL_WIDE && wide_shape_ok(a->net, a->n_games)) n += (wide_workspace_bytes(a) + 255) / 256 * 256;
  return n;
}

int32_t pg_gene_count(const pg_net *net) {
  if (!net) return fail(PG_ERR_INVALID, "net is NULL");
  int32_t rc = check_net(*net, false);
  if (rc != PG_OK) return rc;
  return gene_count(*net);
}

int32_t pg_eval_population(const pg_eval_args *a, void *stream) {
  if (!a) return fail(PG_ERR_INVALID, "args is NULL");
  int32_t rc = check_struct_size(a);
  if (rc != PG_OK) return rc;
  rc = check_net(a->net, true);
  if (rc != PG_OK) return rc;
  if (a->n_genomes < 0) return fail(PG_ERR_INVALID, "n_genomes=%d < 0", a->n_genomes);
  if (a->n_games < 1 || a->n_games > 64) return fail(PG_ERR_INVALID, "n_games=%d not in [1, 64]", a->n_games);
  if (a->horizon < 0) return fail(PG_ERR_INVALID, "horizon=%d < 0", a->horizon);
  if (a->timeout_thresh != 0 && (a->timeout_thresh < 32 || a->timeout_thresh > (1 << 20)))
    return fail(PG_ERR_INVALID, "timeout_thresh=%d not 0 or in [32, 1048576]", a->timeout_thresh);
  if (a->win_score < 0) return fail(PG_ERR_INVALID, "win_score=%d < 0", a->win_score);
  if (a->n_genomes == 0) {
    if (a->counters) PG_HIP(hipMemsetAsync(a->counters, 0, 16 * sizeof(uint64_t), (hipStream_t)stream));
    return PG_OK;
  }
  const long total = (long)a->n_genomes * a->n_games;
  if (total > 0x7fffffffL) return fail(PG_ERR_INVALID, "too many games (%ld)", total);
  const int G = gene_count(a->net);
  if (!a->genomes || a->genome_stride < G)
    return fail(PG_ERR_INVALID, "genomes NULL or genome_stride=%lld < gene count %d", (long long)a->genome_stride, G);
  if (!a->game_kind || !a->game_opp || !a->game_mult || !a->fitness || !a->rewards || !a->scores ||
      !a->frames || !a->total_frames || !a->status)
    return fail(PG_ERR_INVALID, "a required per-game array is NULL");
  if (a->n_opponents > 0 && (!a->opponents || a->opponent_stride < G))
    return fail(PG_ERR_INVALID, "opponents NULL or opponent_stride < gene count");
  if (a->precision != PG_PREC_CERTIFIED && a->precision != PG_PREC_F64)
    return fail(PG_ERR_INVALID, "precision=%d", a->precision);
  if (a->trace && (a->trace_games < 0 || a->trace_cap < 1))
    return fail(PG_ERR_INVALID, "trace needs trace_games >= 0 and trace_cap >= 1");
  if (a->prep < PG_PREP_ALL || a->prep > PG_PREP_REST) return fail(PG_ERR_INVALID, "prep=%d", a->prep);
  if (a->net.activation == PG_ACT_RELU) {
    if (a->kernel == PG_KERNEL_SPLIT || a->kernel == PG_KERNEL_WIDE)
      return fail(PG_ERR_UNSUPPORTED, "activation relu: the %s kernel evaluates sigmoid networks only (use RELU or GENERAL)",
                  a->kernel == PG_KERNEL_SPLIT ? "split" : "wide");
    if (a->horizon > 0) return fail(PG_ERR_UNSUPPORTED, "activation relu: no fixed-horizon mode (horizon must be 0)");
    if (a->hard_log) return fail(PG_ERR_UNSUPPORTED, "activation relu: no hard-case log (hard_log must be NULL)");
  } else if (a->kernel == PG_KERNEL_RELU) {
    return fail(PG_ERR_UNSUPPORTED, "activation sigmoid: the relu kernel evaluates PG_ACT_RELU networks only");
  }
  if (a->horizon > 0 && a->trace) return fail(PG_ERR_INVALID, "horizon mode runs untraced (trace must be NULL)");
  if (a->horizon > 0 && resolve_kernel(a) != PG_KERNEL_SPLIT)
    return fail(PG_ERR_UNSUPPORTED, "horizon mode runs on the SPLIT kernel ([6, H<=64, 3], certified)");
  const size_t need = pg_eval_workspace_bytes(a);
  if (!a->workspace || a->workspace_bytes < need)
    return fail(PG_ERR_INVALID, "workspace of %zu bytes required (got %zu)", need, a->workspace_bytes);

  hipStream_t s = (hipStream_t)stream;
  EvalParams p;
  memset(&p, 0, sizeof(p));
  p.genomes = a->genomes;
  p.opponents = a->opponents ? a->opponents : a->genomes;
  p.kind = a->game_kind;
  p.opp = a->game_opp;
  p.mult = a->game_mult;
  p.rewards = a->rewards;
  p.scores = a->scores;
  p.frames = a->frames;
  p.total_frames = a->total_frames;
  p.counters = a->counters;
  p.trace = a->trace;
  p.trace_games = a->trace ? a->trace_games : 0;
  p.trace_cap = a->trace_cap;
  p.hard_log = a->hard_cap > 0 ? a->hard_log : nullptr;
  p.hard_cap = a->hard_cap;
  p.work = (unsigned int *)a->workspace;
  p.status_game = (int32_t *)((char *)a->workspace + 256);
  p.gstride = a->genome_stride;
  p.ostride = a->opponent_stride;
  p.n_opponents = a->opponents ? a->n_opponents : 0;
  p.rows = a->genome_rows;
  p.n_active = a->n_active;
  p.seed = a->seed;
  p.n_genomes = a->n_genomes;
  p.n_games = a->n_games;
  p.total = (int)total;
  for (int i = 0; i < a->net.n_nodes; ++i) p.nodes[i] = a->net.nodes[i];
  p.n_nodes = a->net.n_nodes;
  p.bias = a->net.bias ? 1 : 0;
  p.max_width = max_width(a->net);
  p.activation = a->net.activation;

  p.prep = a->prep;
  p.horizon = a->horizon;
  p.timeout_thresh = a->timeout_thresh > 0 ? a->timeout_thresh : kTimeoutThresh;
  p.win_score = a->win_score > 0 ? (a->win_score < kDoneScore ? a->win_score : kDoneScore) : kWinScore;
  const int kernel = resolve_kernel(a);
  if (kernel != PG_KERNEL_SPLIT) {
    if (a->prep == PG_PREP_GENOMES) return PG_OK;
    p.prep = PG_PREP_ALL;
    PG_HIP(hipMemsetAsync(a->workspace, 0, 256, s));
    if (a->counters) PG_HIP(hipMemsetAsync(a->counters, 0, 16 * sizeof(uint64_t), s));
  }
  const bool res_ok = resident_shape_ok(a->net);
  const bool wide_ok = wide_shape_ok(a->net, a->n_games);
  if (kernel == PG_KERNEL_WIDE) {
    if (!wide_ok)
      return fail(PG_ERR_UNSUPPORTED, "wide kernel needs NETWORK_SHAPE [6, H1<=512, H2<=512, 1..4] and n_games <= 8");
    rc = launch_wide(p, a->net.dtype, (char *)a->workspace + eval_base_workspace(a), s);
    if (rc != PG_OK) return rc;
  } else if (kernel == PG_KERNEL_SPLIT) {
    if (!res_ok) return fail(PG_ERR_UNSUPPORTED, "split kernel needs NETWORK_SHAPE [6, H<=256, 2..4]");
    if (a->precision != PG_PREC_CERTIFIED) return fail(PG_ERR_UNSUPPORTED, "split kernel is the certified-precision path");
    const int H = a->net.nodes[1];
    const int L = a->group_lanes > 0 ? a->group_lanes : choose_split_lanes(H);
    p.recs = (float *)((char *)a->workspace + eval_base_workspace(a));
    rc = a->net.dtype == PG_F64 ? launch_service_any<double>(p, L, a->net.nodes[2], s)
                                : launch_service_any<float>(p, L, a->net.nodes[2], s);
    if (rc != PG_OK) return rc;
    if (a->prep == PG_PREP_GENOMES) return PG_OK;
  } else if (kernel == PG_KERNEL_RESIDENT || kernel == PG_KERNEL_STAGED) {
    return fail(PG_ERR_UNSUPPORTED, "the %s kernel was retired (DESIGN 4.1b-c); use SPLIT",
                kernel == PG_KERNEL_RESIDENT ? "resident" : "staged");
  } else if (kernel == PG_KERNEL_RELU) {
    if (!relu_shape_ok(a->net))
      return fail(PG_ERR_UNSUPPORTED, "relu kernel needs NETWORK_SHAPE [6, H<=256, 2..4] with bias");
    if (a->precision != PG_PREC_CERTIFIED) return fail(PG_ERR_UNSUPPORTED, "relu kernel is the certified-precision path");
    rc = launch_relu(p, a->net.dtype, s);
    if (rc != PG_OK) return rc;
  } else if (kernel == PG_KERNEL_GENERAL) {
    const size_t lds = 2 * (size_t)(p.max_width + 1) * sizeof(double);
    if (lds > 160 * 1024) return fail(PG_ERR_UNSUPPORTED, "layer width %d too large for LDS", p.max_width);
    const int cap = num_cus() * 16;
    const int grid = total < cap ? (int)total : cap;
    if (a->net.dtype == PG_F64)
      hipLaunchKernelGGL(k_general<double>, dim3(grid), dim3(64), lds, s, p);
    else
      hipLaunchKernelGGL(k_general<float>, dim3(grid), dim3(64), lds, s, p);
    PG_HIP(hipGetLastError());
  } else {
    return fail(PG_ERR_INVALID, "kernel=%d", a->kernel);
  }
  hipLaunchKernelGGL(k_fitness, dim3((a->n_genomes + 255) / 256), dim3(256), 0, s, a->rewards,
                     p.status_game, a->n_genomes, a->n_active, a->n_games, a->fitness, a->status);
  PG_HIP(hipGetLastError());
  return PG_OK;
}

int32_t pg_forward(const pg_forward_args *a, void *stream) {
  if (!a) return fail(PG_ERR_INVALID, "args is NULL");
  int32_t rc = check_net(a->net, false);
  if (rc != PG_OK) return rc;
  if (a->n < 0) return fail(PG_ERR_INVALID, "n=%d < 0", a->n);
  if (a->n == 0) return PG_OK;
  const int G = gene_count(a->net);
  if (!a->genomes || a->genome_stride < G || !a->x || !a->index)
    return fail(PG_ERR_INVALID, "genomes/x/index NULL or genome_stride < gene count %d", G);
  hipStream_t s = (hipStream_t)stream;
  FwdParams p;
  memset(&p, 0, sizeof(p));
  p.genomes = a->genomes;
  p.gidx = a->genome_index;
  p.x = a->x;
  p.index = a->index;
  p.act = a->act;
  p.z_all = a->z_all;
  p.h_all = a->h_all;
  p.counters = a->counters;
  p.gstride = a->genome_stride;
// ... 112 lines not shown
int32_t pg_physics_reset(int32_t *state, int32_t n, const uint64_t *seeds, const int32_t *one_player,
                         void *stream) {
  if (n < 0 || (n > 0 && !state)) return fail(PG_ERR_INVALID, "state NULL or n < 0");
  if (n == 0) return PG_OK;
  hipLaunchKernelGGL(k_physics_reset, dim3((n + 255) / 256), dim3(256), 0, (hipStream_t)stream, state, n,
                     seeds, one_player);
  PG_HIP(hipGetLastError());
  return PG_OK;
}

int32_t pg_physics_step(int32_t *state, int32_t n, const uint8_t *actions, void *stream) {
  if (n < 0 || (n > 0 && (!state || !actions))) return fail(PG_ERR_INVALID, "state/actions NULL or n < 0");
  if (n == 0) return PG_OK;
  hipLaunchKernelGGL(k_physics_step, dim3((n + 255) / 256), dim3(256), 0, (hipStream_t)stream, state, n,
                     actions);
  PG_HIP(hipGetLastError());
  return PG_OK;
}

int32_t pg_ga_select_tournament(const pg_select_args *a, void *stream) {
  if (!a) return fail(PG_ERR_INVALID, "args is NULL");
  if (a->k < 0 || a->n_pop < 1 || a->tournsize < 1 || !a->fitness || !a->chosen)
    return fail(PG_ERR_INVALID, "selTournament needs k >= 0, n_pop >= 1, tournsize >= 1 and buffers");
  if (a->k == 0) return PG_OK;
  hipLaunchKernelGGL(k_select, dim3((a->k + 255) / 256), dim3(256), 0, (hipStream_t)stream, *a);
  PG_HIP(hipGetLastError());
  return PG_OK;
}

int32_t pg_ga_select_tournament_ranked(const pg_select_args *a, const double *sorted_fitness,
                                       const int32_t *order, void *stream) {
  if (!a || !sorted_fitness || !order) return fail(PG_ERR_INVALID, "args/sorted_fitness/order is NULL");
  if (a->k < 0 || a->n_pop < 1 || a->tournsize < 1 || !a->chosen)
    return fail(PG_ERR_INVALID, "selTournament needs k >= 0, n_pop >= 1, tournsize >= 1 and buffers");
  if (a->k == 0) return PG_OK;
  hipLaunchKernelGGL(k_select_ranked, dim3((a->k + 255) / 256), dim3(256), 0, (hipStream_t)stream, *a,
                     sorted_fitness, order);
  PG_HIP(hipGetLastError());
  return PG_OK;
}

int32_t pg_ga_vary(const pg_ga_args *a, void *stream) {
  if (!a) return fail(PG_ERR_INVALID, "args is NULL");
  if (a->n < 0 || a->genes < 1 || a->stride < a->genes || !a->parents || !a->chosen || !a->offspring ||
      !a->invalid || (a->dtype != PG_F32 && a->dtype != PG_F64))
    return fail(PG_ERR_INVALID, "varAnd: bad sizes or NULL buffers");
  if (a->n == 0) return PG_OK;
  const int pairs = (a->n + 1) / 2;
  if (a->pair_list && (!a->pair_count || a->pair_cap < 0)) return fail(PG_ERR_INVALID, "varAnd: pair_list needs pair_count and pair_cap >= 0");
  constexpr int kListWaves = 8192;
  int waves = a->pair_list ? (a->pair_cap < pairs ? a->pair_cap : pairs) : pairs;
  if (a->pair_list && waves > kListWaves) waves = kListWaves;
  if (waves == 0) return PG_OK;
  const dim3 grid((unsigned)((waves + 3) / 4));
  if (a->dtype == PG_F64)
    hipLaunchKernelGGL(k_vary<double>, grid, dim3(256), 0, (hipStream_t)stream, *a);
  else
    hipLaunchKernelGGL(k_vary<float>, grid, dim3(256), 0, (hipStream_t)stream, *a);
  PG_HIP(hipGetLastError());
  return PG_OK;
}

int32_t pg_ga_list_pairs(const uint8_t *mask, int32_t n_pairs, int32_t *list, int32_t *count, void *stream) {
  if (n_pairs < 0 || !count || (n_pairs && (!mask || !list))) return fail(PG_ERR_INVALID, "list_pairs: bad sizes or NULL buffers");
  PG_HIP(hipMemsetAsync(count, 0, sizeof(int32_t), (hipStream_t)stream));
  if (n_pairs == 0) return PG_OK;
  hipLaunchKernelGGL(k_list_pairs, dim3((unsigned)((n_pairs + 255) / 256)), dim3(256), 0, (hipStream_t)stream, mask,
                     n_pairs, list, count);
  PG_HIP(hipGetLastError());
  return PG_OK;
}

int32_t pg_ga_mark_pairs(uint8_t *mask, int32_t n_pairs, const int32_t *rows, int32_t n_rows, int32_t skip_lo,
                         int32_t skip_hi, const uint8_t *exclude, void *stream) {
  if (n_pairs < 0 || n_rows < 0 || (n_rows && (!mask || !rows)))
    return fail(PG_ERR_INVALID, "mark_pairs: bad sizes or NULL buffers");
  if (n_rows == 0) return PG_OK;
  hipLaunchKernelGGL(k_mark_pairs, dim3((unsigned)((n_rows + 255) / 256)), dim3(256), 0, (hipStream_t)stream, mask,
                     n_pairs, rows, n_rows, skip_lo, skip_hi, exclude);
  PG_HIP(hipGetLastError());
  return PG_OK;
}

int32_t pg_ga_schedule(const pg_schedule_args *a, void *stream) {
  if (!a) return fail(PG_ERR_INVALID, "args is NULL");
  if (a->n < 0 || a->n_games < 1 || a->n_hof < 0 || a->row_offset < 0 ||
      (a->mode != PG_SCHED_REFERENCE && a->mode != PG_SCHED_SELFPLAY))
    return fail(PG_ERR_INVALID, "schedule: bad sizes or mode");
  if (a->n == 0) return PG_OK;
  if (!a->kind || !a->opp || !a->mult || (a->mode == PG_SCHED_REFERENCE && a->n_hof > 0 && !a->hof_fitness))
    return fail(PG_ERR_INVALID, "schedule: NULL output or hof_fitness");
  const long total = (long)a->n * a->n_games;
  if (a->hof_slices > 1 && a->block_rows < 1) return fail(PG_ERR_INVALID, "schedule: hof_slices > 1 needs block_rows >= 1");
  hipLaunchKernelGGL(k_schedule, dim3((unsigned)((total + 255) / 256)), dim3(256), 0, (hipStream_t)stream, *a);
  PG_HIP(hipGetLastError());
  return PG_OK;
}

int32_t pg_gather_rows(void *dst, int64_t dst_stride, const void *old_rows, int64_t old_stride, const void *rows,
                       int64_t rows_stride, const int64_t *index, const int32_t *src, int32_t n_old, int32_t n,
                       int64_t genes, int32_t dtype, void *stream) {
  if (n < 0 || n_old < 0 || genes < 1 || (dtype != PG_F32 && dtype != PG_F64) ||
      (n > 0 && (!dst || !src || (n_old > 0 && !old_rows) || dst_stride < genes || old_stride < genes ||
                 rows_stride < genes)))
    return fail(PG_ERR_INVALID, "gather_rows: bad sizes, dtype or NULL buffers");
  if (n == 0) return PG_OK;
  if (dtype == PG_F64)
    hipLaunchKernelGGL(k_gather_rows<double>, dim3(n), dim3(256), 0, (hipStream_t)stream, (double *)dst, dst_stride,
                       (const double *)old_rows, old_stride, (const double *)rows, rows_stride, index, src, n_old,
                       genes);
  else
// ... 276 lines not shown
```

### neuro-genetic-pong-self-play_amd/pong_amd/_lib.py

```python
from __future__ import annotations

import ctypes
import os
import threading

PKG_DIR = os.path.dirname(os.path.dirname(os.path.abspath(__file__)))
REPO_DIR = os.path.dirname(PKG_DIR)
LIB_NAME = "libpong_ga.so"
LIB_PATH = os.environ.get("PONG_GA_LIB") or os.path.join(PKG_DIR, LIB_NAME)
HEADER_PATH = os.path.join(REPO_DIR, "include", "pong_ga.h")

PG_ABI_VERSION = 13
PG_MAX_NODES = 9

PG_OK, PG_ERR_INVALID, PG_ERR_HIP, PG_ERR_UNSUPPORTED = 0, -1, -2, -3
PG_F32, PG_F64 = 0, 1
PG_ACT_SIGMOID, PG_ACT_RELU = 0, 1
PG_OPP_HARDCODED, PG_OPP_ROM_CPU, PG_OPP_SCORE, PG_OPP_NN = 0, 1, 2, 3
PG_PREP_ALL, PG_PREP_GENOMES, PG_PREP_REST = 0, 1, 2
PG_PREC_CERTIFIED, PG_PREC_F64 = 0, 1
PG_SCHED_REFERENCE, PG_SCHED_SELFPLAY = 0, 1
PG_KERNEL_AUTO, PG_KERNEL_GENERAL, PG_KERNEL_RESIDENT, PG_KERNEL_SPLIT, PG_KERNEL_WIDE, PG_KERNEL_STAGED = 0, 1, 2, 3, 4, 5
PG_KERNEL_RELU = 6
PG_STATE_FIELDS = 16
STATE_FIELD_NAMES = ("ball_x", "ball_y", "ball_vx", "ball_vy", "ball_visible", "serve_timer",
                     "serve_dir", "hits", "point", "lpy", "rpy", "score1", "score2",
                     "one_player", "seed_lo", "seed_hi")

_vp = ctypes.c_void_p


class PgNet(ctypes.Structure):
    _fields_ = [("n_nodes", ctypes.c_int32), ("nodes", ctypes.c_int32 * PG_MAX_NODES),
                ("bias", ctypes.c_int32), ("dtype", ctypes.c_int32),
                ("activation", ctypes.c_int32)]


class PgEvalArgs(ctypes.Structure):
    _fields_ = [
        ("struct_size", ctypes.c_uint32),
        ("net", PgNet),
        ("n_genomes", ctypes.c_int32), ("n_games", ctypes.c_int32),
        ("genomes", _vp), ("genome_stride", ctypes.c_int64),
        ("opponents", _vp), ("opponent_stride", ctypes.c_int64), ("n_opponents", ctypes.c_int32),
        ("precision", ctypes.c_int32),
        ("game_kind", _vp), ("game_opp", _vp), ("game_mult", _vp),
        ("seed", ctypes.c_uint64),
        ("fitness", _vp), ("rewards", _vp), ("scores", _vp), ("frames", _vp),
        ("total_frames", _vp), ("status", _vp), ("counters", _vp),
        ("trace", _vp), ("trace_games", ctypes.c_int32), ("trace_cap", ctypes.c_int32),
        ("kernel", ctypes.c_int32), ("group_lanes", ctypes.c_int32),
        ("workspace", _vp), ("workspace_bytes", ctypes.c_size_t),
        ("hard_log", _vp), ("hard_cap", ctypes.c_int32), ("genome_rows", _vp),
        ("n_active", _vp),
        ("prep", ctypes.c_int32), ("horizon", ctypes.c_int32),
        ("timeout_thresh", ctypes.c_int32), ("win_score", ctypes.c_int32),
    ]

    def __init__(self, *args, **kw):
        super().__init__(*args, **kw)
        self.struct_size = ctypes.sizeof(PgEvalArgs)


class PgForwardArgs(ctypes.Structure):
    _fields_ = [
        ("net", PgNet), ("n", ctypes.c_int32), ("genomes", _vp), ("genome_stride", ctypes.c_int64),
        ("genome_index", _vp), ("x", _vp), ("precision", ctypes.c_int32), ("index", _vp),
        ("act", _vp), ("counters", _vp), ("z_all", _vp), ("h_all", _vp),
    ]


class PgDecideArgs(ctypes.Structure):
    _fields_ = [
        ("net", PgNet), ("n", ctypes.c_int32), ("genomes", _vp), ("genome_stride", ctypes.c_int64),
        ("genome_index", _vp), ("k", _vp), ("index", _vp), ("stage", _vp),
    ]


class PgWideDecideArgs(ctypes.Structure):
    _fields_ = [
        ("net", PgNet), ("n", ctypes.c_int32), ("genomes", _vp), ("genome_stride", ctypes.c_int64),
        ("genome_index", _vp), ("k", _vp), ("index", _vp), ("act", _vp),
        ("workspace", _vp), ("workspace_bytes", ctypes.c_size_t),
    ]


class PgReluDecideArgs(ctypes.Structure):
    _fields_ = [
        ("net", PgNet), ("n", ctypes.c_int32), ("genomes", _vp), ("genome_stride", ctypes.c_int64),
        ("genome_index", _vp), ("k", _vp), ("index", _vp), ("stage", _vp), ("z32", _vp), ("bound", _vp),
    ]


class PgGaArgs(ctypes.Structure):
    _fields_ = [
        ("n", ctypes.c_int32), ("genes", ctypes.c_int64), ("dtype", ctypes.c_int32),
        ("parents", _vp), ("stride", ctypes.c_int64), ("n_parents", ctypes.c_int32),
        ("chosen", _vp), ("offspring", _vp), ("invalid", _vp),
        ("cxpb", ctypes.c_double), ("mutpb", ctypes.c_double), ("alpha", ctypes.c_double),
        ("mu", ctypes.c_double), ("sigma", ctypes.c_double), ("indpb", ctypes.c_double),
        ("seed", ctypes.c_uint64), ("generation", ctypes.c_uint64), ("pair_mask", _vp),
        ("pair_list", _vp), ("pair_count", _vp), ("pair_cap", ctypes.c_int32),
    ]


class PgSelectArgs(ctypes.Structure):
    _fields_ = [
        ("n_pop", ctypes.c_int32), ("k", ctypes.c_int32), ("tournsize", ctypes.c_int32),
        ("fitness", _vp), ("chosen", _vp), ("seed", ctypes.c_uint64), ("generation", ctypes.c_uint64),
    ]


class PgScheduleArgs(ctypes.Structure):
    _fields_ = [
        ("mode", ctypes.c_int32), ("n", ctypes.c_int32), ("n_games", ctypes.c_int32),
        ("row_offset", ctypes.c_int64), ("n_hof", ctypes.c_int32), ("hof_fitness", _vp),
        ("seed", ctypes.c_uint64), ("generation", ctypes.c_uint64),
        ("kind", _vp), ("opp", _vp), ("mult", _vp), ("rows", _vp),
        ("hof_slices", ctypes.c_int32), ("block_rows", ctypes.c_int32), ("slice_local", ctypes.c_int32),
    ]


class PgHofPackedArgs(ctypes.Structure):
    _fields_ = [("maxsize", ctypes.c_int32), ("hof_n", ctypes.c_int32), ("hof_fitness", _vp), ("k", ctypes.c_int32),
                ("packed", _vp), ("new_n", _vp), ("new_src", _vp), ("new_fitness", _vp),
                ("slot_in", _vp), ("slot_out", _vp)]


class PgHofArgs(ctypes.Structure):
    _fields_ = [
        ("maxsize", ctypes.c_int32), ("hof_n", ctypes.c_int32), ("hof_fitness", _vp), ("hof_hash", _vp),
        ("pop_n", ctypes.c_int32), ("pop_fitness", _vp), ("pop_hash", _vp), ("rank", _vp),
        ("new_n", _vp), ("new_src", _vp), ("new_fitness", _vp),
    ]


class PgHofRankArgs(ctypes.Structure):
    _fields_ = [
        ("hof_n", ctypes.c_int32), ("hof_fitness", _vp), ("hof_hash", _vp), ("k", ctypes.c_int32),
        ("cand_fitness", _vp), ("cand_hash", _vp), ("packed", _vp), ("workspace", _vp),
        ("workspace_bytes", ctypes.c_size_t),
    ]


class PgHofPrepareArgs(ctypes.Structure):
    _fields_ = [
        ("fitness", _vp), ("pop_n", ctypes.c_int32), ("filter", ctypes.c_int32), ("worst", ctypes.c_double),
        ("rows", _vp), ("stride", ctypes.c_int64), ("genes", ctypes.c_int64), ("dtype", ctypes.c_int32),
        ("hof_n", ctypes.c_int32), ("hof_fitness", _vp), ("hof_hash", _vp), ("k", _vp), ("cand", _vp),
        ("hashes", _vp), ("packed", _vp), ("workspace", _vp), ("workspace_bytes", ctypes.c_size_t),
    ]


class PgScatterArgs(ctypes.Structure):
    _fields_ = [
        ("n", ctypes.c_int32), ("n_games", ctypes.c_int32), ("row_lo", ctypes.c_int32),
        ("fitness", _vp), ("frames", _vp), ("rows", _vp), ("n_active", _vp), ("shard_fitness", _vp),
        ("lineage", _vp),
    ]


class PgMergeArgs(ctypes.Structure):
    _fields_ = [
        ("pop_n", ctypes.c_int32), ("fitness", _vp), ("invalid", _vp), ("inherited", _vp), ("new_fitness", _vp),
        ("filter", ctypes.c_int32), ("worst", ctypes.c_double), ("cand", _vp), ("cand_fitness", _vp),
        ("summary", _vp), ("workspace", _vp), ("workspace_bytes", ctypes.c_size_t),
    ]


class PgHofCandArgs(ctypes.Structure):
    _fields_ = [
        ("hof_n", ctypes.c_int32), ("hof_fitness", _vp), ("hof_hash", _vp), ("k", ctypes.c_int32),
        ("cand", _vp), ("cand_fitness", _vp), ("rows", _vp), ("stride", ctypes.c_int64),
        ("genes", ctypes.c_int64), ("dtype", ctypes.c_int32), ("cand_hash", _vp), ("packed", _vp),
        ("workspace", _vp), ("workspace_bytes", ctypes.c_size_t),
    ]


class PgHofCommitArgs(ctypes.Structure):
    _fields_ = [
        ("dst", _vp), ("dst_stride", ctypes.c_int64), ("old_rows", _vp), ("old_stride", ctypes.c_int64),
        ("rows", _vp), ("rows_stride", ctypes.c_int64), ("cand", _vp), ("src", _vp), ("n_old", ctypes.c_int32),
        ("m", ctypes.c_int32), ("genes", ctypes.c_int64), ("dtype", ctypes.c_int32), ("old_hash", _vp),
        ("cand_hash", _vp), ("new_hash", _vp), ("fitness_in", _vp), ("new_fitness", _vp),
        ("dst_slot", _vp),
    ]


SIGNATURES = {
    "pg_version": (ctypes.c_char_p, []),
    "pg_abi_version": (ctypes.c_int32, []),
    "pg_build_flags": (ctypes.c_int32, []),
    "pg_last_error": (ctypes.c_char_p, []),
    "pg_device_count": (ctypes.c_int32, []),
    "pg_eval_workspace_bytes": (ctypes.c_size_t, [ctypes.POINTER(PgEvalArgs)]),
    "pg_gene_count": (ctypes.c_int32, [ctypes.POINTER(PgNet)]),
    "pg_eval_population": (ctypes.c_int32, [ctypes.POINTER(PgEvalArgs), _vp]),
    "pg_forward": (ctypes.c_int32, [ctypes.POINTER(PgForwardArgs), _vp]),
    "pg_decide": (ctypes.c_int32, [ctypes.POINTER(PgDecideArgs), _vp]),
    "pg_wide_decide_workspace_bytes": (ctypes.c_size_t, [ctypes.POINTER(PgWideDecideArgs)]),
    "pg_wide_decide": (ctypes.c_int32, [ctypes.POINTER(PgWideDecideArgs), _vp]),
    "pg_relu_decide": (ctypes.c_int32, [ctypes.POINTER(PgReluDecideArgs), _vp]),
    "pg_physics_reset": (ctypes.c_int32, [_vp, ctypes.c_int32, _vp, _vp, _vp]),
    "pg_physics_step": (ctypes.c_int32, [_vp, ctypes.c_int32, _vp, _vp]),
    "pg_ga_select_tournament": (ctypes.c_int32, [ctypes.POINTER(PgSelectArgs), _vp]),
    "pg_ga_select_tournament_ranked": (ctypes.c_int32, [ctypes.POINTER(PgSelectArgs), _vp, _vp, _vp]),
    "pg_ga_vary": (ctypes.c_int32, [ctypes.POINTER(PgGaArgs), _vp]),
    "pg_ga_list_pairs": (ctypes.c_int32, [_vp, ctypes.c_int32, _vp, _vp, _vp]),
    "pg_ga_mark_pairs": (ctypes.c_int32, [_vp, ctypes.c_int32, _vp, ctypes.c_int32, ctypes.c_int32, ctypes.c_int32,
                                          _vp, _vp]),
    "pg_ga_schedule": (ctypes.c_int32, [ctypes.POINTER(PgScheduleArgs), _vp]),
    "pg_row_hash": (ctypes.c_int32, [_vp, ctypes.c_int64, _vp, ctypes.c_int32, ctypes.c_int64, ctypes.c_int32, _vp,
                                     _vp]),
    "pg_hof_update": (ctypes.c_int32, [ctypes.POINTER(PgHofArgs)]),
    "pg_hof_update_packed": (ctypes.c_int32, [ctypes.POINTER(PgHofPackedArgs)]),
    "pg_hof_rank_classes_workspace_bytes": (ctypes.c_size_t, [ctypes.c_int32]),
    "pg_hof_rank_classes": (ctypes.c_int32, [ctypes.POINTER(PgHofRankArgs), _vp]),
    "pg_hof_prepare_workspace_bytes": (ctypes.c_size_t, [ctypes.c_int32, ctypes.c_int32]),
    "pg_hof_prepare": (ctypes.c_int32, [ctypes.POINTER(PgHofPrepareArgs), _vp]),
    "pg_gather_rows": (ctypes.c_int32, [_vp, ctypes.c_int64, _vp, ctypes.c_int64, _vp, ctypes.c_int64, _vp, _vp,
                                        ctypes.c_int32, ctypes.c_int32, ctypes.c_int64, ctypes.c_int32, _vp]),
    "pg_ga_scatter_fitness": (ctypes.c_int32, [ctypes.POINTER(PgScatterArgs), _vp]),
    "pg_ga_merge_workspace_bytes": (ctypes.c_size_t, [ctypes.c_int32]),
    "pg_ga_merge_fitness": (ctypes.c_int32, [ctypes.POINTER(PgMergeArgs), _vp]),
    "pg_ga_select_workspace_bytes": (ctypes.c_size_t, [ctypes.c_int32]),
    "pg_ga_select_ranked": (ctypes.c_int32, [ctypes.POINTER(PgSelectArgs), _vp, ctypes.c_size_t, _vp]),
    "pg_ga_inherit": (ctypes.c_int32, [_vp, ctypes.c_int32, _vp, _vp, _vp, _vp, _vp]),
    "pg_ga_order_workspace_bytes": (ctypes.c_size_t, [ctypes.c_int32]),
    "pg_ga_order": (ctypes.c_int32, [ctypes.c_int32, ctypes.c_int32, _vp, _vp, ctypes.c_int32, _vp, _vp, _vp,
                                     ctypes.c_size_t, _vp]),
    "pg_hof_prepare_cand_workspace_bytes": (ctypes.c_size_t, [ctypes.c_int32, ctypes.c_int32]),
    "pg_hof_prepare_cand": (ctypes.c_int32, [ctypes.POINTER(PgHofCandArgs), _vp]),
    "pg_hof_commit": (ctypes.c_int32, [ctypes.POINTER(PgHofCommitArgs), _vp]),
    "pg_render_frames": (ctypes.c_int32, [_vp, ctypes.c_int32, _vp, _vp]),
    "pg_find_stuff": (ctypes.c_int32, [_vp, ctypes.c_int64, ctypes.c_int32, _vp, _vp]),
}

_lock = threading.Lock()
_lib = None


class PongGAError(RuntimeError):

    def __init__(self, func: str, code: int, message: str):
        super().__init__(f"{func} failed ({code}): {message}")
        self.code = code


def lib() -> ctypes.CDLL:
    global _lib
    if _lib is not None:
        return _lib
    with _lock:
        if _lib is None:
            if not os.path.exists(LIB_PATH):
                raise RuntimeError(
                    f"{LIB_PATH} is missing: build it with `python -c 'import __graft_entry__ as g; g.build()'` "
                    "(hipcc --offload-arch=gfx950). There is no CPU fallback.")
            L = ctypes.CDLL(LIB_PATH)
            for name, (res, args) in SIGNATURES.items():
                fn = getattr(L, name)
                fn.restype = res
                fn.argtypes = args
            if L.pg_abi_version() != PG_ABI_VERSION:
                raise RuntimeError(f"{LIB_PATH}: ABI {L.pg_abi_version()} != {PG_ABI_VERSION}")
            _lib = L
    return _lib


def check(func: str, rc: int) -> None:
    if rc != PG_OK:
        msg = lib().pg_last_error()
        raise PongGAError(func, rc, msg.decode() if msg else "")


def make_net(nodes, bias=True, dtype=PG_F64, activation=PG_ACT_SIGMOID) -> PgNet:
    nodes = [int(n) for n in nodes]
    if not 2 <= len(nodes) <= PG_MAX_NODES:
        raise ValueError(f"NETWORK_SHAPE must have 2..{PG_MAX_NODES} entries, got {nodes}")
    arr = (ctypes.c_int32 * PG_MAX_NODES)(*(nodes + [0] * (PG_MAX_NODES - len(nodes))))
    return PgNet(len(nodes), arr, 1 if bias else 0, dtype, int(activation))
```

### neuro-genetic-pong-self-play_amd/pong_amd/device.py

```python
from __future__ import annotations

import ctypes
from dataclasses import dataclass
from typing import Optional

import torch

from . import _lib as L

PRECISIONS = {"certified": L.PG_PREC_CERTIFIED, "f64": L.PG_PREC_F64}
PREPS = {"all": L.PG_PREP_ALL, "genomes": L.PG_PREP_GENOMES, "rest": L.PG_PREP_REST}
KERNELS = {"auto": L.PG_KERNEL_AUTO, "general": L.PG_KERNEL_GENERAL, "split": L.PG_KERNEL_SPLIT,
           "wide": L.PG_KERNEL_WIDE, "relu": L.PG_KERNEL_RELU}
ACTIVATIONS = {"sigmoid": L.PG_ACT_SIGMOID, "relu": L.PG_ACT_RELU}
DTYPES = {torch.float32: L.PG_F32, torch.float64: L.PG_F64}


def gene_count(nodes, bias=True) -> int:
    b = 1 if bias else 0
    return sum((int(nodes[i]) + b) * int(nodes[i + 1]) for i in range(len(nodes) - 1))


def _ptr(t: Optional[torch.Tensor]):
    return ctypes.c_void_p(t.data_ptr()) if t is not None else None


def _stream(device) -> ctypes.c_void_p:
    return ctypes.c_void_p(torch.cuda.current_stream(device).cuda_stream)


def _need(t: torch.Tensor, name: str, dtype, device, shape=None):
    if t.dtype != dtype:
        raise TypeError(f"{name} must be {dtype}, got {t.dtype}")
    if t.device != device:
        raise ValueError(f"{name} must live on {device}, got {t.device}")
    if not t.is_contiguous():
        raise ValueError(f"{name} must be contiguous")
    if shape is not None and tuple(t.shape) != tuple(shape):
        raise ValueError(f"{name} must have shape {tuple(shape)}, got {tuple(t.shape)}")


def _need_rows(t: torch.Tensor, name: str, dtype, device):
    if t.dtype != dtype:
        raise TypeError(f"{name} must be {dtype}, got {t.dtype}")
    if t.device != device:
        raise ValueError(f"{name} must live on {device}, got {t.device}")
    if t.dim() != 2 or (t.shape[1] > 1 and t.stride(1) != 1) or (t.shape[0] > 1 and t.stride(0) < t.shape[1]):
        raise ValueError(f"{name} must be row-major rows (unit column stride, row stride >= row length)")


@dataclass
class EvalResult:

    fitness: torch.Tensor
    rewards: torch.Tensor
    scores: torch.Tensor
    frames: torch.Tensor
    total_frames: torch.Tensor
    status: torch.Tensor
    counters: torch.Tensor


class Evaluator:

    def __init__(self, nodes, bias=True, dtype=torch.float64, device=None, n_games=6,
                 precision="certified", kernel="auto", group_lanes=0, seed=0, horizon=0,
                 timeout_thresh=0, win_score=0, activation="sigmoid"):
        if activation not in ACTIVATIONS:
            raise ValueError(f"activation must be one of {sorted(ACTIVATIONS)}, got {activation!r}")
        if not torch.cuda.is_available():
            raise RuntimeError("pong_amd.Evaluator needs a HIP device (no CPU fallback)")
        L.lib()
        self.nodes = [int(n) for n in nodes]
        self.bias = bool(bias)
        self.dtype = dtype
        self.device = torch.device(device) if device is not None else torch.device("cuda", torch.cuda.current_device())
        self.n_games = int(n_games)
        self.precision = precision
        self.kernel = kernel
        self.group_lanes = int(group_lanes)
        self.seed = int(seed)
        self.horizon = int(horizon)
        self.timeout_thresh = int(timeout_thresh)
        self.win_score = int(win_score)
        self.genes = gene_count(self.nodes, self.bias)
        self.activation = activation
        self.net = L.make_net(self.nodes, self.bias, DTYPES[dtype], ACTIVATIONS[activation])
        self._ws = None
        self._prep_key = self._prep_ws = None

    def selfplay_schedule(self, n: int, n_opponents: int, offset: int = 0):
        dev = self.device
        gi = (torch.arange(n, device=dev, dtype=torch.int64) + offset)[:, None] * self.n_games
        gi = gi + torch.arange(self.n_games, device=dev, dtype=torch.int64)[None, :]
        kind = torch.full((n, self.n_games), L.PG_OPP_NN, dtype=torch.int32, device=dev)
        opp = (gi % max(n_opponents, 1)).to(torch.int32)
        mult = torch.ones((n, self.n_games), dtype=torch.float64, device=dev)
        return kind, opp, mult

    def _workspace(self, args: L.PgEvalArgs) -> torch.Tensor:
        need = L.lib().pg_eval_workspace_bytes(ctypes.byref(args))
        if self._ws is None or self._ws.numel() < need:
            self._ws = torch.empty(max(need, 4096), dtype=torch.uint8, device=self.device)
        return self._ws

    def evaluate(self, genomes: torch.Tensor, kind: torch.Tensor, opp: torch.Tensor, mult: torch.Tensor,
                 opponents: Optional[torch.Tensor] = None, trace_games: int = 0, trace_cap: int = 0,
                 out: Optional[EvalResult] = None, precision: Optional[str] = None,
                 kernel: Optional[str] = None, group_lanes: Optional[int] = None, validate: bool = True,
                 hard_log: Optional[torch.Tensor] = None, rows: Optional[torch.Tensor] = None,
                 n_active: Optional[torch.Tensor] = None, prep: str = "all", horizon: Optional[int] = None):
        dev = self.device
        n = genomes.shape[0] if rows is None else rows.shape[0]
        games = self.n_games
        _need(genomes, "genomes", self.dtype, dev)
        if genomes.dim() != 2 or genomes.shape[1] < self.genes:
            raise ValueError(f"genomes must be [n, >= {self.genes}], got {tuple(genomes.shape)}")
        _need(kind, "kind", torch.int32, dev, (n, games))
        _need(opp, "opp", torch.int32, dev, (n, games))
        _need(mult, "mult", torch.float64, dev, (n, games))
        if opponents is not None:
            _need_rows(opponents, "opponents", self.dtype, dev)
            if opponents.dim() != 2 or opponents.shape[1] < self.genes:
                raise ValueError(f"opponents must be [H, >= {self.genes}], got {tuple(opponents.shape)}")
        if rows is not None:
            _need(rows, "rows", torch.int32, dev, (n,))
        if validate and n:
            if rows is not None and bool(((rows < 0) | (rows >= genomes.shape[0])).any()):
                raise ValueError(f"rows must index the {genomes.shape[0]}-row genomes tensor")
            nn_games = kind == L.PG_OPP_NN
            if bool(((kind < 0) | (kind > L.PG_OPP_NN)).any()):
                raise ValueError("kind values must be pg_opp_kind codes 0..3")
            if bool(nn_games.any()):
                h = 0 if opponents is None else opponents.shape[0]
                bad = nn_games & ((opp < 0) | (opp >= h))
                if bool(bad.any()):
                    raise ValueError(f"opp rows must index the {h}-row opponents tensor")
        if out is None:
            out = EvalResult(
                fitness=torch.empty(n, dtype=torch.float64, device=dev),
                rewards=torch.empty((n, games), dtype=torch.float64, device=dev),
                scores=torch.empty((n, games, 2), dtype=torch.int32, device=dev),
                frames=torch.empty((n, games), dtype=torch.int32, device=dev),
                total_frames=torch.empty((n, games), dtype=torch.float64, device=dev),
                status=torch.empty(n, dtype=torch.int32, device=dev),
                counters=torch.empty(16, dtype=torch.int64, device=dev))
        trace = None
        if trace_games and trace_cap:
            trace = torch.zeros((trace_games, trace_cap), dtype=torch.uint8, device=dev)
        a = L.PgEvalArgs()
        a.net = self.net
        a.n_genomes = n
        a.n_games = games
        a.genomes = _ptr(genomes)
        a.genome_stride = genomes.stride(0) if genomes.shape[0] > 1 else genomes.shape[1]
        a.genome_rows = _ptr(rows)
        if n_active is not None:
            _need(n_active, "n_active", torch.int32, dev, (1,))
            a.n_active = _ptr(n_active)
        if opponents is not None and opponents.shape[0] > 0:
            a.opponents = _ptr(opponents)
            a.opponent_stride = opponents.stride(0) if opponents.shape[0] > 1 else opponents.shape[1]
            a.n_opponents = opponents.shape[0]
        a.precision = PRECISIONS[precision or self.precision]
        a.game_kind, a.game_opp, a.game_mult = _ptr(kind), _ptr(opp), _ptr(mult)
        a.seed = self.seed
        a.fitness, a.rewards, a.scores = _ptr(out.fitness), _ptr(out.rewards), _ptr(out.scores)
        a.frames, a.total_frames, a.status = _ptr(out.frames), _ptr(out.total_frames), _ptr(out.status)
        a.counters = _ptr(out.counters)
        if trace is not None:
            a.trace, a.trace_games, a.trace_cap = _ptr(trace), trace_games, trace_cap
        if hard_log is not None:
            _need(hard_log, "hard_log", torch.int32, dev)
            if hard_log.dim() != 2 or hard_log.shape[1] != 8:
                raise ValueError("hard_log must be [cap, 8] int32")
            a.hard_log, a.hard_cap = _ptr(hard_log), hard_log.shape[0]
        a.prep = PREPS[prep]
        if prep == "rest" and n and self._prep_key != self._prep_of(genomes, rows, n_active, n):
            raise ValueError("prep='rest' needs a preceding prep='genomes' call with the same genomes, rows, "
                             "n_active and row count on this evaluator")
        a.horizon = self.horizon if horizon is None else int(horizon)
        a.timeout_thresh, a.win_score = self.timeout_thresh, self.win_score
        a.kernel = KERNELS[kernel or self.kernel]
        a.group_lanes = self.group_lanes if group_lanes is None else int(group_lanes)
        ws = self._workspace(a)
        a.workspace, a.workspace_bytes = _ptr(ws), ws.numel()
        if prep == "rest" and n and self._prep_ws != ws.data_ptr():
            raise ValueError("prep='rest': the workspace holding the genome records was reallocated")
        with torch.cuda.device(dev):
            L.check("pg_eval_population", L.lib().pg_eval_population(ctypes.byref(a), _stream(dev)))
        self._prep_key = self._prep_of(genomes, rows, n_active, n) if prep == "genomes" else None
        self._prep_ws = ws.data_ptr() if prep == "genomes" else None
        return out, trace

    @staticmethod
    def _prep_of(genomes, rows, n_active, n):
        return (genomes.data_ptr(), genomes.stride(0), None if rows is None else rows.data_ptr(),
                None if n_active is None else n_active.data_ptr(), int(n))

    def forward(self, genomes: torch.Tensor, x: torch.Tensor, genome_index: Optional[torch.Tensor] = None,
                precision: Optional[str] = None, want_act: bool = True, want_layers: bool = False):
        dev = self.device
        _need(genomes, "genomes", self.dtype, dev)
        n = x.shape[0]
        _need(x, "x", torch.float64, dev, (n, self.nodes[0]))
        if genome_index is not None:
            _need(genome_index, "genome_index", torch.int32, dev, (n,))
        index = torch.empty(n, dtype=torch.int32, device=dev)
        act = torch.empty((n, self.nodes[-1]), dtype=torch.float64, device=dev) if want_act else None
        counters = torch.zeros(4, dtype=torch.int64, device=dev)
        a = L.PgForwardArgs()
        a.net = self.net
        a.n = n
        a.genomes = _ptr(genomes)
        a.genome_stride = genomes.stride(0) if genomes.shape[0] > 1 else genomes.shape[1]
        a.genome_index = _ptr(genome_index)
        a.x = _ptr(x)
        a.precision = PRECISIONS[precision or self.precision]
        a.index = _ptr(index)
        a.act = _ptr(act)
        a.counters = _ptr(counters)
        if want_layers:
            units = sum(self.nodes[1:])
            z_all = torch.empty((n, units), dtype=torch.float64, device=dev)
            h_all = torch.empty((n, units), dtype=torch.float64, device=dev)
            a.z_all, a.h_all = _ptr(z_all), _ptr(h_all)
            self.last_layers = (z_all, h_all)
        with torch.cuda.device(dev):
            L.check("pg_forward", L.lib().pg_forward(ctypes.byref(a), _stream(dev)))
        self.last_forward_counters = counters
# ... 77 lines not shown


class Physics:

    def __init__(self, n: int, device=None):
        L.lib()
        self.n = int(n)
        self.device = torch.device(device) if device is not None else torch.device("cuda", torch.cuda.current_device())
        self.state = torch.zeros((L.PG_STATE_FIELDS, self.n), dtype=torch.int32, device=self.device)

    def reset(self, seeds: torch.Tensor, one_player: Optional[torch.Tensor] = None):
        _need(seeds, "seeds", torch.int64, self.device, (self.n,))
        if one_player is not None:
            _need(one_player, "one_player", torch.int32, self.device, (self.n,))
        with torch.cuda.device(self.device):
            L.check("pg_physics_reset", L.lib().pg_physics_reset(
                _ptr(self.state), self.n, _ptr(seeds), _ptr(one_player), _stream(self.device)))

    def step(self, actions: torch.Tensor):
        _need(actions, "actions", torch.uint8, self.device, (self.n,))
        with torch.cuda.device(self.device):
            L.check("pg_physics_step", L.lib().pg_physics_step(
                _ptr(self.state), self.n, _ptr(actions), _stream(self.device)))

    def fields(self) -> dict:
        s = self.state.cpu()
        return {name: s[i] for i, name in enumerate(L.STATE_FIELD_NAMES)}


def select_tournament(fitness: torch.Tensor, k: int, tournsize: int, seed: int, generation: int) -> torch.Tensor:
    _need(fitness, "fitness", torch.float64, fitness.device)
    chosen = torch.empty(k, dtype=torch.int32, device=fitness.device)
    a = L.PgSelectArgs(fitness.shape[0], k, tournsize, _ptr(fitness), _ptr(chosen), seed, generation)
    with torch.cuda.device(fitness.device):
        L.check("pg_ga_select_tournament", L.lib().pg_ga_select_tournament(ctypes.byref(a), _stream(fitness.device)))
    return chosen


def select_tournament_ranked(fitness: torch.Tensor, k: int, tournsize: int, seed: int, generation: int) -> torch.Tensor:
    _need(fitness, "fitness", torch.float64, fitness.device)
    sorted_fit, order = torch.sort(fitness, stable=True)
    order = order.to(torch.int32)
    chosen = torch.empty(k, dtype=torch.int32, device=fitness.device)
    a = L.PgSelectArgs(fitness.shape[0], k, tournsize, _ptr(fitness), _ptr(chosen), seed, generation)
    with torch.cuda.device(fitness.device):
        L.check("pg_ga_select_tournament_ranked", L.lib().pg_ga_select_tournament_ranked(
            ctypes.byref(a), _ptr(sorted_fit), _ptr(order), _stream(fitness.device)))
    return chosen


def vary(parents: torch.Tensor, chosen: torch.Tensor, genes: int, cxpb: float, mutpb: float, alpha: float,
         mu: float, sigma: float, indpb: float, seed: int, generation: int, out: Optional[torch.Tensor] = None,
         pair_mask: Optional[torch.Tensor] = None, invalid: Optional[torch.Tensor] = None,
         pair_list: Optional[tuple] = None):
    dev = parents.device
    n = chosen.shape[0]
    _need(chosen, "chosen", torch.int32, dev, (n,))
    if pair_mask is not None:
        _need(pair_mask, "pair_mask", torch.uint8, dev, ((n + 1) // 2,))
    if out is None:
        out = torch.empty((n, parents.shape[1]), dtype=parents.dtype, device=dev)
    if invalid is None:
        invalid = torch.empty(n, dtype=torch.uint8, device=dev)
    _need(invalid, "invalid", torch.uint8, dev, (n,))
    a = L.PgGaArgs()
    a.n, a.genes, a.dtype = n, genes, DTYPES[parents.dtype]
    a.parents, a.stride, a.n_parents = _ptr(parents), parents.stride(0), parents.shape[0]
    a.chosen, a.offspring, a.invalid = _ptr(chosen), _ptr(out), _ptr(invalid)
    a.cxpb, a.mutpb, a.alpha, a.mu, a.sigma, a.indpb = cxpb, mutpb, alpha, mu, sigma, indpb
    a.seed, a.generation = seed, generation
    a.pair_mask = _ptr(pair_mask)
    if pair_list is not None:
        lst, cnt, cap = pair_list
        _need(lst, "pair_list", torch.int32, dev)
        _need(cnt, "pair_count", torch.int32, dev, (1,))
        a.pair_list, a.pair_count, a.pair_cap = _ptr(lst), _ptr(cnt), int(min(cap, lst.numel()))
    if out.stride(0) != parents.stride(0):
        raise ValueError("offspring and parents must share the row stride")
    with torch.cuda.device(dev):
        L.check("pg_ga_vary", L.lib().pg_ga_vary(ctypes.byref(a), _stream(dev)))
    return out, invalid


def list_pairs(mask: torch.Tensor, out: torch.Tensor, count: torch.Tensor) -> None:
    dev = mask.device
    _need(mask, "pair_mask", torch.uint8, dev)
    _need(out, "pair_list", torch.int32, dev)
    _need(count, "pair_count", torch.int32, dev, (1,))
    if out.numel() < mask.numel():
        raise ValueError("pair_list must hold every pair")
    with torch.cuda.device(dev):
        L.check("pg_ga_list_pairs", L.lib().pg_ga_list_pairs(_ptr(mask), mask.numel(), _ptr(out), _ptr(count),
                                                             _stream(dev)))


def mark_pairs(mask: torch.Tensor, rows: torch.Tensor, skip: tuple = (0, 0),
               exclude: Optional[torch.Tensor] = None) -> None:
    dev = mask.device
    _need(mask, "pair_mask", torch.uint8, dev)
    _need(rows, "rows", torch.int32, dev)
    if exclude is not None:
        _need(exclude, "exclude", torch.uint8, dev, tuple(mask.shape))
    with torch.cuda.device(dev):
        L.check("pg_ga_mark_pairs", L.lib().pg_ga_mark_pairs(_ptr(mask), mask.shape[0], _ptr(rows), rows.numel(),
                                                             int(skip[0]), int(skip[1]), _ptr(exclude), _stream(dev)))


SCHEDULES = {"reference": L.PG_SCHED_REFERENCE, "selfplay": L.PG_SCHED_SELFPLAY}


def schedule(mode: str, n: int, n_games: int, row_offset: int, hof_fitness: Optional[torch.Tensor], n_hof: int,
             seed: int, generation: int, device, rows: Optional[torch.Tensor] = None, hof_slices: int = 1,
             block_rows: int = 0, slice_local: bool = False, out: Optional[tuple] = None):
    dev = torch.device(device)
    if out is None:
        kind = torch.empty((n, n_games), dtype=torch.int32, device=dev)
        opp = torch.empty((n, n_games), dtype=torch.int32, device=dev)
        mult = torch.empty((n, n_games), dtype=torch.float64, device=dev)
    else:
        kind, opp, mult = out
        _need(kind, "kind", torch.int32, dev, (n, n_games))
        _need(opp, "opp", torch.int32, dev, (n, n_games))
        _need(mult, "mult", torch.float64, dev, (n, n_games))
    if hof_fitness is not None:
        _need(hof_fitness, "hof_fitness", torch.float64, dev)
        if hof_fitness.numel() < n_hof:
            raise ValueError(f"hof_fitness holds {hof_fitness.numel()} values, n_hof={n_hof}")
    elif n_hof and mode == "reference":
        raise ValueError("reference schedule with a hall of fame needs hof_fitness")
    if rows is not None:
        _need(rows, "rows", torch.int32, dev, (n,))
    a = L.PgScheduleArgs(SCHEDULES[mode], n, n_games, row_offset, n_hof, _ptr(hof_fitness), seed, generation,
                         _ptr(kind), _ptr(opp), _ptr(mult), _ptr(rows), int(hof_slices), int(block_rows),
                         1 if slice_local else 0)
# ... 240 lines not shown

def inherit(chosen: torch.Tensor, fitness: torch.Tensor, inherited: torch.Tensor, lineage_in: torch.Tensor,
            lineage_out: torch.Tensor) -> None:
    dev = chosen.device
    n = chosen.shape[0]
    _need(chosen, "chosen", torch.int32, dev, (n,))
    _need(inherited, "inherited", torch.float64, dev, (n,))
    _need(lineage_out, "lineage_out", torch.float32, dev, (n,))
    with torch.cuda.device(dev):
        L.check("pg_ga_inherit", L.lib().pg_ga_inherit(_ptr(chosen), n, _ptr(fitness), _ptr(inherited),
                                                       _ptr(lineage_in), _ptr(lineage_out), _stream(dev)))


def order(n: int, row_lo: int, invalid: Optional[torch.Tensor], lineage: Optional[torch.Tensor], by_length: bool,
          rows: torch.Tensor, count: torch.Tensor, ws: Workspaces) -> None:
    dev = rows.device
    _need(rows, "rows", torch.int32, dev, (n,))
    _need(count, "count", torch.int32, dev, (1,))
    nbytes = int(L.lib().pg_ga_order_workspace_bytes(n))
    w = ws.get("order", nbytes)
    with torch.cuda.device(dev):
        L.check("pg_ga_order", L.lib().pg_ga_order(n, row_lo, _ptr(invalid), _ptr(lineage), 1 if by_length else 0,
                                                   _ptr(rows), _ptr(count), _ptr(w), w.numel(), _stream(dev)))


def hof_prepare_cand(hof_fitness: torch.Tensor, hof_hash: torch.Tensor, cand: torch.Tensor,
                     cand_fitness: torch.Tensor, rows: torch.Tensor, genes: int, cand_hash: torch.Tensor,
                     packed: torch.Tensor, ws: Workspaces) -> None:
    dev = cand.device
    hn, k = hof_fitness.shape[0], cand.shape[0]
    _need(hof_fitness, "hof_fitness", torch.float64, dev, (hn,))
    _need(hof_hash, "hof_hash", torch.int64, dev, (hn,))
    _need(cand, "cand", torch.int32, dev, (k,))
    _need(cand_fitness, "cand_fitness", torch.float64, dev, (k,))
    _need(cand_hash, "cand_hash", torch.int64, dev, (k,))
    _need(packed, "packed", torch.int64, dev, (hn + 2 * k,))
    if rows.dim() != 2 or rows.dtype not in DTYPES or rows.stride(1) != 1 or rows.device != dev:
        raise ValueError("rows must be a row-major [n, G] f32/f64 tensor on the candidates' device")
    nbytes = int(L.lib().pg_hof_prepare_cand_workspace_bytes(hn, k))
    if nbytes == 0:
        msg = L.lib().pg_last_error()
        raise L.PongGAError("pg_hof_prepare_cand_workspace_bytes", -1, msg.decode() if msg else "")
    w = ws.get("hof_cand", nbytes)
    stride = rows.stride(0) if rows.shape[0] > 1 else rows.shape[1]
    a = L.PgHofCandArgs(hn, _ptr(hof_fitness), _ptr(hof_hash), k, _ptr(cand), _ptr(cand_fitness), _ptr(rows), stride,
                        int(genes), DTYPES[rows.dtype], _ptr(cand_hash), _ptr(packed), _ptr(w), w.numel())
    with torch.cuda.device(dev):
        L.check("pg_hof_prepare_cand", L.lib().pg_hof_prepare_cand(ctypes.byref(a), _stream(dev)))


def hof_commit(dst: torch.Tensor, old_rows: Optional[torch.Tensor], rows: torch.Tensor, cand: torch.Tensor,
               src: torch.Tensor, n_old: int, genes: int, old_hash: torch.Tensor, cand_hash: torch.Tensor,
               new_hash: torch.Tensor, fitness_in: torch.Tensor, new_fitness: torch.Tensor,
               dst_slot: Optional[torch.Tensor] = None) -> None:
    dev = dst.device
    m = src.shape[0]
    _need(src, "src", torch.int32, dev, (m,))
    _need(fitness_in, "fitness_in", torch.float64, dev, (m,))
    if dst_slot is not None:
        _need(dst_slot, "dst_slot", torch.int32, dev, (m,))
        old_rows = None
    elif old_rows is None:
        raise ValueError("old_rows is required without dst_slot")
    for name, t in (("dst", dst), ("old_rows", old_rows), ("rows", rows)):
        if t is None:
            continue
        if t.dim() != 2 or t.dtype != dst.dtype or t.device != dev or t.stride(1) != 1:
            raise ValueError(f"{name} must be a row-major [n, G] tensor of dst's dtype on dst's device")
    if m > dst.shape[0] or m > new_hash.shape[0] or m > new_fitness.shape[0]:
        raise ValueError("more members than destination rows")
    a = L.PgHofCommitArgs(_ptr(dst), dst.stride(0), _ptr(old_rows) if old_rows is not None else None,
                          old_rows.stride(0) if old_rows is not None else 0, _ptr(rows), rows.stride(0),
                          _ptr(cand), _ptr(src), int(n_old), m, int(genes), DTYPES[dst.dtype], _ptr(old_hash),
                          _ptr(cand_hash), _ptr(new_hash), _ptr(fitness_in), _ptr(new_fitness),
                          _ptr(dst_slot) if dst_slot is not None else None)
    with torch.cuda.device(dev):
        L.check("pg_hof_commit", L.lib().pg_hof_commit(ctypes.byref(a), _stream(dev)))
```

### neuro-genetic-pong-self-play_amd/pong_amd/evolve.py

```python
from __future__ import annotations

from typing import Optional

import numpy as np
import torch
import torch.distributed as dist

from . import device as D
from . import dist as PD

STAT_FIELDS = ("avg", "std", "min", "max")


class DeviceGA:

    def __init__(self, nodes, population_size: int, hof_size: Optional[int] = None,
                 tournsize: Optional[int] = None, *, bias: bool = True, dtype=torch.float64, device=None,
                 n_games: int = 6, schedule: str = "reference", cxpb: float = 0.9, mutpb: float = 0.9,
                 alpha: float = 0.9, mu: float = 0.0, sigma: float = 0.9, indpb: float = 0.9,
                 seed: int = 0, physics_seed: int = 0, precision: str = "certified", kernel: str = "auto",
                 group=None, hof_block_rows: int = 0, timeout_thresh: int = 0, win_score: int = 0,
                 activation: str = "sigmoid"):
        if schedule not in D.SCHEDULES:
            raise ValueError(f"schedule must be one of {sorted(D.SCHEDULES)}")
        self.nodes = [int(v) for v in nodes]
        self.P = int(population_size)
        self.H = int(hof_size) if hof_size is not None else max(self.P // 4, 1)
        self.tournsize = int(tournsize) if tournsize is not None else max(self.P // 4, 1)
        if self.P < 1 or self.H < 0 or self.tournsize < 1:
            raise ValueError("population_size >= 1, hof_size >= 0 and tournsize >= 1 required")
        self.ev = D.Evaluator(self.nodes, bias=bias, dtype=dtype, device=device, n_games=n_games,
                              precision=precision, kernel=kernel, seed=physics_seed,
                              timeout_thresh=timeout_thresh, win_score=win_score, activation=activation)
        self.activation = activation
        self.device, self.dtype, self.G = self.ev.device, dtype, self.ev.genes
        self.bias, self.n_games, self.schedule = bool(bias), int(n_games), schedule
        self.cxpb, self.mutpb, self.alpha = float(cxpb), float(mutpb), float(alpha)
        self.mu, self.sigma, self.indpb = float(mu), float(sigma), float(indpb)
        self.seed, self.physics_seed = int(seed), int(physics_seed)
        self.precision, self.kernel = precision, kernel
        self.group = group
        self.world = dist.get_world_size(group) if dist.is_initialized() else 1
        self.rank = dist.get_rank(group) if dist.is_initialized() else 0
        self.lo, self.hi = PD.shard_range(self.P, self.rank, self.world)
        self.hof_block_rows = int(hof_block_rows)
        self.hof_slices = 1
        if self.hof_block_rows > 0 and schedule == "selfplay":
            self.hof_slices = max(1, min(-(-self.P // self.hof_block_rows), max(self.H, 1)))
        B = self.hof_block_rows
        self._slice = ((self.lo // B) % self.hof_slices
                       if self.hof_slices > 1 and self.hi > self.lo and self.lo // B == (self.hi - 1) // B else None)
        self.store = torch.zeros((self.H + self.P, self.G), dtype=dtype, device=self.device)
        self.spare = torch.empty_like(self.store)
        self.in_place_hall = True
        self._hall_buf = self.store[: self.H]
        M = max(self.H, 1)
        self._up_dev = torch.zeros(4 * M, dtype=torch.int32, device=self.device)
        self.hof_slot = self._up_dev[3 * M:]
        self.hof_slot.copy_(torch.arange(M, dtype=torch.int32, device=self.device))
        self._hof_slot_h = np.zeros(0, np.int32)
        self._slots_identity = True
        self._up_keep = None
        self.fitness = torch.zeros(self.P, dtype=torch.float64, device=self.device)
        self.valid = torch.zeros(self.P, dtype=torch.bool, device=self.device)
        self.hof_fitness = torch.zeros(max(self.H, 1), dtype=torch.float64, device=self.device)
        self.hof_n = 0
        self._hof_fit_host = np.zeros(0, np.float64)
        self.hof_hash = torch.zeros(max(self.H, 1), dtype=torch.int64, device=self.device)
        self.generation = -1
        self.logbook = []
        self.last = None
        self.last_rows = None
        self.last_count = None
        self.eval_events = None
        self.profile = None
        self._t_mark = self._t_sub = 0.0
        self._next = None
        self.early_prep = True
        self.hard_log = None
        self.on_evaluate = None
        self.order_by_length = True
        self.lineage_frames = torch.zeros(self.P, dtype=torch.float32, device=self.device)
        self.native_prepare = True
        self.fused = True
        self.side_stream = True
        self._side = None
        self.prepare_first = True
        self.presubmit = True
        self._pinned = {}
        self.persistent_bufs = True
        self._up_flip = 0
        self._iota_P = None
        self.shard_vary = self.world > 1
        self.balance_shards = False
        self._dealt = {}
        self._n_pairs = (self.P + 1) // 2
        self._skip = (self.lo >> 1, (self.hi + 1) >> 1) if self.hi > self.lo else (0, 0)
        self._shard_pairs = None
        self.ws = D.Workspaces(self.device)
        self._lineage_alt = torch.zeros_like(self.lineage_frames)
        self._hof_hash_alt = torch.zeros_like(self.hof_hash)
        self._hof_fitness_alt = torch.zeros_like(self.hof_fitness)
        self._fit_alt = torch.zeros_like(self.fitness)
        self._summary_h = torch.zeros(8, dtype=torch.float64, pin_memory=True)

    def _sliced(self, n_hof: int) -> bool:
        return self._slice is not None and n_hof >= self.hof_slices

    def _opponents(self, buf: torch.Tensor, n_hof: int) -> Optional[torch.Tensor]:
        if not n_hof:
            return None
        if self._in_place():
            if self._sliced(n_hof):
                idx = self.hof_slot[self._slice:n_hof:self.hof_slices].long()
                out = self._buf("hall_slice", (idx.shape[0], self.G), self.dtype)
                torch.index_select(self._hall_buf, 0, idx, out=out)
                return out
            return self._hall_buf[:n_hof]
        return buf[self._slice:n_hof:self.hof_slices] if self._sliced(n_hof) else buf[:n_hof]

    def _in_place(self) -> bool:
        return bool(self.in_place_hall and self.fused and self.H > 0)

    def _opp_slots(self, opp: torch.Tensor, n_hof: int) -> torch.Tensor:
        if not self._in_place() or not n_hof or self._sliced(n_hof) or self._slots_identity:
            return opp
        out = self._buf("opp_slots", opp.numel(), torch.int32) if self.persistent_bufs else None
        return torch.index_select(self.hof_slot[:n_hof], 0, opp.reshape(-1), out=out).view_as(opp)

    def _opponents_by_position(self, n_hof: int) -> Optional[torch.Tensor]:
        if not n_hof:
# ... 58 lines not shown
    def hall_of_fame(self) -> torch.Tensor:
        if self._in_place():
            return self._hall_buf[self.hof_slot[: self.hof_n].long()]
        return self.store[: self.hof_n]

    @property
    def hof_member_fitness(self) -> np.ndarray:
        return self._hof_fit_host.copy()

    def initialize(self, init: str = "uniform", init_sigma: float = 3.0):
        gen = torch.Generator(device=self.device).manual_seed(self.seed)
        rows = max(1, (1 << 28) // (8 * self.G))
        for r0 in range(0, self.P, rows):
            r1 = min(self.P, r0 + rows)
            if init == "uniform":
                blk = torch.rand((r1 - r0, self.G), generator=gen, dtype=torch.float64, device=self.device)
            elif init == "normal":
                blk = torch.randn((r1 - r0, self.G), generator=gen, dtype=torch.float64,
                                  device=self.device).mul_(init_sigma)
            else:
                raise ValueError("init must be 'uniform' or 'normal'")
            self.store[self.H + r0:self.H + r1] = blk.to(self.dtype)
        self.valid.zero_()
        self.fitness.zero_()
        self._set_hof_empty()
        self._next = None
        self.generation = -1
        self.logbook = []

    def set_population(self, genomes: torch.Tensor, fitness: Optional[torch.Tensor] = None,
                       valid: Optional[torch.Tensor] = None):
        if tuple(genomes.shape) != (self.P, self.G):
            raise ValueError(f"genomes must be [{self.P}, {self.G}], got {tuple(genomes.shape)}")
        self._next = None
        self._rows.copy_(genomes.to(device=self.device, dtype=self.dtype))
        if fitness is None:
            self.valid.zero_()
            self.fitness.zero_()
        else:
            self.fitness.copy_(fitness.to(device=self.device, dtype=torch.float64))
            v = torch.ones(self.P, dtype=torch.bool) if valid is None else valid.to(torch.bool)
            self.valid.copy_(v.to(self.device))

    def set_hall_of_fame(self, genomes: Optional[torch.Tensor], fitness):
        fit = np.asarray(fitness, dtype=np.float64)
        n = fit.shape[0]
        if n > self.H or (genomes is not None and tuple(genomes.shape) != (n, self.G)):
            raise ValueError(f"hall of fame must be [<= {self.H}, {self.G}] with matching fitness")
        if n and np.any(np.diff(fit) > 0):
            raise ValueError("hall-of-fame members must be ordered best first")
        if genomes is not None:
            self.store[:n] = genomes.to(device=self.device, dtype=self.dtype)
        self._next = None
        self.hof_n = n
        self._hof_fit_host = fit.copy()
        if n and self._hall_buf.data_ptr() != self.store.data_ptr():
            self._hall_buf[:n] = self.store[:n]
        if self.H:
            self.hof_slot.copy_(torch.arange(self.hof_slot.shape[0], dtype=torch.int32, device=self.device))
        self._hof_slot_h = np.arange(n, dtype=np.int32)
        self._slots_identity = True
        if n:
            self.hof_fitness[:n] = torch.from_numpy(fit).to(self.device)
            self.hof_hash[:n] = D.row_hash(self.store[:n], self.G)

    def _set_hof_empty(self):
        self.hof_n = 0
        self._hof_fit_host = np.zeros(0, np.float64)
        self._hof_slot_h = np.zeros(0, np.int32)
        self._slots_identity = True

    def _evaluate(self, g: int, rows: torch.Tensor, inv: Optional[torch.Tensor] = None) -> torch.Tensor:
        lo, hi = self.lo, self.hi
        n = hi - lo
        local = count = None
        if inv is not None:
            inv_s = inv[lo:hi]
            c_inv = torch.cumsum(inv_s, 0, dtype=torch.int32)
            count = c_inv[-1:] if n else torch.zeros(1, dtype=torch.int32, device=self.device)
            if self.order_by_length:
                key = torch.where(inv_s, self.lineage_frames[lo:hi], torch.full_like(self.lineage_frames[lo:hi], -1.0))
                local = (torch.argsort(key, descending=True, stable=True) + lo).to(torch.int32)
            else:
                c_val = torch.cumsum(~inv_s, 0, dtype=torch.int32)
                dest = torch.where(inv_s, c_inv - 1, count + c_val - 1).long()
                local = torch.empty(n, dtype=torch.int32, device=self.device)
                local[dest] = torch.arange(lo, hi, dtype=torch.int32, device=self.device)
        kind, opp, mult = self.eval_schedule(g, rows=local)
        opponents = self._opponents(self.store, self.hof_n)
        out = self.last if (self.last is not None and self.last.fitness.shape[0] == n) else None
        if self.eval_events is not None:
            self.eval_events[0].record()
        if local is None:
            res, _ = self.ev.evaluate(rows[lo:hi], kind, opp, mult, opponents=opponents, out=out, validate=False,
                                      hard_log=self.hard_log)
        else:
            res, _ = self.ev.evaluate(rows, kind, opp, mult, opponents=opponents, out=out, validate=False,
                                      hard_log=self.hard_log, rows=local, n_active=count)
        if self.eval_events is not None:
            self.eval_events[1].record()
        self.last, self.last_rows, self.last_count = res, local, count
        if self.on_evaluate is not None:
            self.on_evaluate(g, rows if local is not None else rows[lo:hi], opponents, res)
        longest = res.frames.max(dim=1).values.to(torch.float32)
        if local is None:
            self.lineage_frames[lo:hi] = longest
        else:
            played = torch.arange(n, device=self.device) < count
            at = local.long()
            self.lineage_frames[at] = torch.where(played, longest, self.lineage_frames[at])
        fit = res.fitness
        if local is not None:
            shard = torch.zeros(n, dtype=torch.float64, device=self.device)
            shard[local.long() - lo] = fit
            fit = torch.where(inv_s, shard, torch.zeros_like(shard))
        return PD.gather_fitness(fit, self.P, self.group) if dist.is_initialized() else fit

    @staticmethod
    def _check(fit: torch.Tensor):
        if bool(torch.isnan(fit).any()):
            raise ZeroDivisionError("float division by zero (calculate_reward with total_frames == 0)")

    def _select_vary(self, g: int, parents: torch.Tensor, fitness: torch.Tensor, out: torch.Tensor):
        chosen = D.select_tournament_ranked(fitness, self.P, self.tournsize, seed=self.seed, generation=g)
        _, invalid = D.vary(parents, chosen, self.G, self.cxpb, self.mutpb, self.alpha, self.mu,
                            self.sigma, self.indpb, seed=self.seed, generation=g, out=out)
        inherited = fitness[chosen.long()]
        self.lineage_frames = self.lineage_frames[chosen.long()]
        return invalid.bool(), inherited

    def _hof_update(self, fit: torch.Tensor, rows: torch.Tensor, dst: torch.Tensor, overlap=None):
        if self.H == 0:
            if overlap:
                overlap()
            return
        old_n = self.hof_n
        worst = float(self._hof_fit_host[-1]) if old_n >= self.H else None
        if self.native_prepare:
            k, cand, hashes, packed_d = D.hof_prepare(fit, worst, rows, self.G, self.hof_fitness[:old_n],
                                                      self.hof_hash[:old_n])
        elif worst is not None:
            cand = torch.nonzero(fit > worst).flatten()
        else:
            cand = torch.arange(self.P, device=self.device)
        if not self.native_prepare:
            k = int(cand.numel())
        if k == 0:
            dst[:old_n] = self.store[:old_n]
            if overlap:
                overlap()
            return
        n = old_n + k
        if self.profile is not None:
            self.profile["hof_candidates"] = self.profile.get("hof_candidates", 0) + k
        if not self.native_prepare:
            h = D.row_hash(rows, self.G, index=cand.to(torch.int32))
            fc = fit[cand]
            hashes = torch.cat([self.hof_hash[:old_n], h])
            by_age = torch.cat([self.hof_fitness[:old_n].flip(0), fc])
            order = torch.sort(by_age, stable=True).indices
            rank_age = torch.empty_like(order)
            rank_age[order] = torch.arange(n, device=self.device)
            rank = torch.cat([rank_age[:old_n].flip(0), rank_age[old_n:]])
            cls = torch.unique(hashes, return_inverse=True)[1]
            packed_d = torch.cat([rank | (cls << 32), fc.view(torch.int64)])
        packed_h = torch.empty(packed_d.shape, dtype=torch.int64, pin_memory=True)
        packed_h.copy_(packed_d, non_blocking=True)
        copied = torch.cuda.Event()
        copied.record()
        if overlap:
            overlap()
        copied.synchronize()
        packed = packed_h.numpy()
        self._mark("hof_prepare", sub=True)
        rank_np = (packed[:n] & 0xFFFFFFFF).astype(np.int32)
        cls_np = packed[:n] >> 32
        src, new_fit = D.hof_update(self.H, self._hof_fit_host, cls_np[:old_n], packed[n:].view(np.float64),
                                    cls_np[old_n:], rank=rank_np)
        self._mark("hof_scan", sub=True)
        m = src.shape[0]
        up = torch.empty(3 * m, dtype=torch.int32, pin_memory=True)
        upn = up.numpy()
        upn[: 2 * m].view(np.float64)[:] = new_fit
        upn[2 * m:] = src
# ... 11 lines not shown
                         invalid.sum().double()]).tolist()
        if v[0]:
            raise ZeroDivisionError("float division by zero (calculate_reward with total_frames == 0)")
        return v[1:5], int(v[5])

    def _record(self, g: int, nevals: int, vals=None) -> dict:
        if vals is None:
            f = self.fitness
            vals = torch.stack([f.mean(), f.std(unbiased=False), f.min(), f.max()]).tolist()
        rec = {"gen": g, "nevals": nevals, **dict(zip(STAT_FIELDS, vals))}
        self.logbook.append(rec)
        return rec

    def step(self) -> dict:
        return self._step_fused() if self.fused else self._step_torch()

    def _step_torch(self) -> dict:
        if self.generation < 0:
            fit = self._evaluate(0, self._rows, ~self.valid)
            nevals = int((~self.valid).sum())
            new_fit = torch.where(self.valid, self.fitness, fit)
            self._check(new_fit)
            self.fitness, self.valid = new_fit, torch.ones_like(self.valid)
            self._hof_update(new_fit, self._rows, self.spare,
                             overlap=lambda: self._prefetch(1, self._rows, new_fit, self.spare))
            self.store[: self.hof_n] = self.spare[: self.hof_n]
            self.generation = 0
            return self._record(0, nevals)
        g = self.generation + 1
        self._mark(None)
        off = self.spare[self.H:]
        if self._next is not None and self._next[0] == g:
            inv, inherited = self._next[1:]
        else:
            inv, inherited = self._select_vary(g, self._rows, self.fitness, off)
        self._next = None
        self._mark("select_vary")
        fit = self._evaluate(g, off, inv)
        new_fit = torch.where(inv, fit, inherited)
        self._mark("evaluate")
        stats, nevals = self._summary(new_fit, inv)
        self._hof_update(new_fit, off, self.spare, overlap=lambda: self._prefetch(g + 1, off, new_fit, self.store))
        self._mark("hall_of_fame")
        self.fitness = new_fit
        self.store, self.spare = self.spare, self.store
        self.generation = g
        rec = self._record(g, nevals, stats)
        self._mark("record")
        return rec

    def _buf(self, name, shape, dtype):
        return self.ws.tensor(name, shape, dtype)

    def _select(self, g: int, fitness: torch.Tensor) -> torch.Tensor:
        chosen = self._buf("chosen%d" % (g & 1), self.P, torch.int32)
        D.select_ranked(fitness, self.P, self.tournsize, self.seed, g, self.ws, chosen=chosen)
        return chosen

    def _shard_mask(self) -> torch.Tensor:
        if self._shard_pairs is None:
            self._shard_pairs = torch.zeros(self._n_pairs, dtype=torch.uint8, device=self.device)
            self._shard_pairs[self._skip[0]:self._skip[1]] = 1
        return self._shard_pairs

    def _complete(self, g: int, off: torch.Tensor, parents: torch.Tensor, rows: torch.Tensor, name: str,
                  exclude: Optional[torch.Tensor] = None) -> torch.Tensor:
        mask = self._buf("complete_" + name, self._n_pairs, torch.uint8)
        mask.zero_()
        D.mark_pairs(mask, rows, skip=self._skip, exclude=exclude)
        lst = self._buf("complete_list_" + name, self._n_pairs, torch.int32)
        cnt = self._buf("complete_count_" + name, 1, torch.int32)
        D.list_pairs(mask, lst, cnt)
        chosen = self._buf("chosen%d" % (g & 1), self.P, torch.int32)
        D.vary(parents, chosen, self.G, self.cxpb, self.mutpb, self.alpha, self.mu, self.sigma, self.indpb,
               seed=self.seed, generation=g, out=off, pair_list=(lst, cnt, min(rows.numel(), self._n_pairs)),
               invalid=self._buf("complete_inv_" + name, self.P, torch.uint8))
        return mask

    def _deal(self, inv_u8: torch.Tensor, g: int):
        P = self.P
        grows = self._buf("deal_rows", P, torch.int32)
        gcount = self._buf("deal_count", 1, torch.int32)
        D.order(P, 0, inv_u8, self.lineage_frames, True, grows, gcount, self.ws)
        n = self._n_eval
        pos = PD.deal_positions(n, self.rank, self.world, self.device)
        local = self._buf("local_rows%d" % (g & 1), n, torch.int32)
        local.copy_(grows[pos.clamp(max=P - 1)])
        count = self._buf("local_count%d" % (g & 1), 1, torch.int32)
        count.copy_((pos < gcount.long()).sum().to(torch.int32).reshape(1))
        return local, count

    def _gather_dealt(self, res, local: torch.Tensor, count: torch.Tensor) -> torch.Tensor:
        P, n = self.P, local.shape[0]
        played = torch.arange(n, device=self.device) < count
        rid = torch.where(played, local.long(), torch.full_like(local, P, dtype=torch.int64))
        longest = res.frames.max(dim=1).values.double()
        pack = torch.stack([rid.double(), res.fitness, longest], dim=1)
        allp = PD.gather_equal(pack, self.group)
        at = allp[:, 0].long()
        fit = torch.zeros(P + 1, dtype=torch.float64, device=self.device)
        fit.index_copy_(0, at, allp[:, 1])
        lin = torch.cat([self.lineage_frames, self.lineage_frames.new_zeros(1)])
        lin.index_copy_(0, at, allp[:, 2].float())
        self.lineage_frames.copy_(lin[:P])
        return fit[:P]

    def _next_gen_prep(self, g: int, parents: torch.Tensor, fitness: torch.Tensor, store: torch.Tensor,
                       cand_pairs: Optional[torch.Tensor] = None):
        chosen = self._select(g, fitness)
        if cand_pairs is not None:
            prev = self._dealt.get((g - 1) & 1)
            self._complete(g - 1, parents, store[self.H:], chosen, "parents",
                           exclude=cand_pairs if prev is None else (cand_pairs | prev))
        _, inv = D.vary(parents, chosen, self.G, self.cxpb, self.mutpb, self.alpha, self.mu, self.sigma, self.indpb,
                        seed=self.seed, generation=g, out=store[self.H:],
                        pair_mask=self._shard_mask() if self._sharded() else None,
                        invalid=self._buf("invalid%d" % (g & 1), self.P, torch.uint8) if self.persistent_bufs else None)
        inherited = self._buf("inherited", self.P, torch.float64)
        D.inherit(chosen, fitness, inherited, self.lineage_frames, self._lineage_alt)
        self.lineage_frames, self._lineage_alt = self._lineage_alt, self.lineage_frames
        if self._balanced():
            order = self._deal(inv, g)
            if self._sharded():
                self._dealt[g & 1] = self._complete(g, store[self.H:], parents, order[0], "dealt%d" % (g & 1))
        else:
            order = self._order(inv, g)
        self._next = (g, inv, inherited, order, self._early_prep(g, store[self.H:], order))

    def _early_prep(self, g: int, off: torch.Tensor, order):
        n = self._n_eval
        if (not self.early_prep or self.schedule != "selfplay" or self.H == 0 or self.hof_n != self.H or self.last is None
                or self.last.fitness.shape[0] != n):
            return None
        local, count = order
        sched = self.eval_schedule(g, n_hof=self.H, rows=local, out=self._sched_bufs(g, n))
        opponents = self._hall_buf[: self.H] if self._in_place() else self._opponents(self.spare, self.H)
        if self._in_place() and self._sliced(self.H):
            opponents = self._hall_buf[self._slice:self.H:self.hof_slices]
        self.ev.evaluate(off, *sched, opponents=opponents, out=self.last, validate=False,
                         hard_log=self.hard_log, rows=local, n_active=count, prep="genomes")
        return sched

    def _order(self, inv_u8: Optional[torch.Tensor], g: int = 0):
        n = self.hi - self.lo
        local = self._buf("local_rows%d" % (g & 1), n, torch.int32)
        count = self._buf("local_count%d" % (g & 1), 1, torch.int32)
        D.order(n, self.lo, inv_u8, self.lineage_frames, self.order_by_length, local, count, self.ws)
        return local, count

    def _evaluate_fused(self, g: int, rows: torch.Tensor, order, sched=None) -> torch.Tensor:
        lo, hi = self.lo, self.hi
        n = self._n_eval
        local, count = order
        if sched is None:
            kind, opp, mult = self.eval_schedule(g, rows=local, out=self._sched_bufs(g, n))
        else:
            kind, opp, mult = sched
        opponents = self._opponents(self.store, self.hof_n)
        opp = self._opp_slots(opp, self.hof_n)
        out = self.last if (self.last is not None and self.last.fitness.shape[0] == n) else None
        if self.eval_events is not None:
            self.eval_events[0].record()
        res, _ = self.ev.evaluate(rows, kind, opp, mult, opponents=opponents, out=out, validate=False,
                                  hard_log=self.hard_log, rows=local, n_active=count,
                                  prep="all" if sched is None else "rest")
        if self.eval_events is not None:
            self.eval_events[1].record()
        self.last, self.last_rows, self.last_count = res, local, count
        if self.on_evaluate is not None:
            self.on_evaluate(g, rows, self._opponents_by_position(self.hof_n), res)
        if self._balanced():
            return self._gather_dealt(res, local, count)
        shard = self._buf("shard_fit", n, torch.float64)
        D.scatter_fitness(res, n, lo, local, count, shard, self.lineage_frames)
        if not dist.is_initialized():
            return shard
        both = torch.stack([shard, self.lineage_frames[lo:hi].double()], dim=1)
        full = PD.gather_fitness(both, self.P, self.group)
        self.lineage_frames.copy_(full[:, 1].float())
        return full[:, 0].contiguous()

    def _merge(self, fit: torch.Tensor, inv: Optional[torch.Tensor], inherited: Optional[torch.Tensor],
               worst: Optional[float]):
        new_fit, cand, cand_fit, ev = self._merge_start(fit, inv, inherited, worst)
        return (new_fit, cand, cand_fit) + self._merge_finish(ev)

    def _merge_start(self, fit, inv, inherited, worst):
        new_fit = self._fit_alt
        cand = self._buf("cand", self.P, torch.int32)
        cand_fit = self._buf("cand_fit", self.P, torch.float64)
        summ = self._buf("summary", 8, torch.float64)
        D.merge_fitness(fit, inv, inherited, new_fit, worst, cand, cand_fit, summ, self.ws)
        self._summary_h.copy_(summ, non_blocking=True)
        ev = torch.cuda.Event()
        ev.record()
        return new_fit, cand, cand_fit, ev

    def _merge_finish(self, ev):
        ev.synchronize()
        v = self._summary_h.tolist()
        if v[0]:
            raise ZeroDivisionError("float division by zero (calculate_reward with total_frames == 0)")
        self._fit_alt = self.fitness
        return v[1:5], int(v[5]), int(v[6])

    def _hof_update_fused(self, rows: torch.Tensor, cand: torch.Tensor, cand_fit: torch.Tensor, k: int,
                          dst: torch.Tensor, overlap=None):
        if self.H == 0:
            if overlap:
                overlap()
            return
        old_n = self.hof_n
        in_place = self._in_place()
        if k == 0:
            if not in_place:
                dst[:old_n] = self.store[:old_n]
            if overlap:
                overlap()
            return
        if self.profile is not None:
            self.profile["hof_candidates"] = self.profile.get("hof_candidates", 0) + k
        main = torch.cuda.current_stream(self.device)
        side = ready = None
        if overlap and self.side_stream:
            if self._side is None:
                self._side = torch.cuda.Stream(self.device)
            side = self._side
            ready = torch.cuda.Event()
            ready.record(main)
            if not self.prepare_first:
                side.wait_event(ready)
                with torch.cuda.stream(side):
                    overlap()
                self._keep_on(main)
                overlap = None
        n = old_n + k
        cand, cand_fit = cand[:k], cand_fit[:k]
        cand_hash = self._buf("cand_hash", k, torch.int64)
        packed = self._buf("packed", n + k, torch.int64)
        D.hof_prepare_cand(self.hof_fitness[:old_n], self.hof_hash[:old_n], cand, cand_fit, rows, self.G, cand_hash,
                           packed, self.ws)
        packed_h = self._pin("packed", n + k, torch.int64)
        packed_h.copy_(packed, non_blocking=True)
        copied = torch.cuda.Event()
        copied.record()
        self._mark("hof_prepare", sub=True)
        if overlap and side is not None:
            side.wait_event(ready)
            with torch.cuda.stream(side):
                overlap()
            self._keep_on(main)
        elif overlap:
            overlap()
        if overlap:
            self._mark("next_select_vary", sub=True)
        copied.synchronize()
        M = max(self.H, 1)
        self._up_flip ^= 1
        up = self._pin("up%d" % self._up_flip, 4 * M, torch.int32)
        res = D.hof_update_packed(self.H, self._hof_fit_host, packed_h.numpy(), k, out=up.numpy(),
                                  slot_in=self._hof_slot_h if in_place else None, slots=in_place)
        src, new_fit = res[0], res[1]
        self._mark("hof_scan", sub=True)
        m = src.shape[0]
        up_d = self._up_dev
        up_d.copy_(up, non_blocking=True)
        src_d, fit_d = up_d[2 * M:2 * M + m], up_d[: 2 * M].view(torch.float64)[:m]
        if in_place:
            slot_d = up_d[3 * M:3 * M + m]
            D.hof_commit(self._hall_buf, None, rows, cand, src_d, old_n, self.G, self.hof_hash, cand_hash,
                         self._hof_hash_alt, fit_d, self._hof_fitness_alt, dst_slot=slot_d)
            self._hof_slot_h = res[2]
            self._slots_identity = False
        else:
            D.hof_commit(dst, self.store, rows, cand, src_d, old_n, self.G, self.hof_hash, cand_hash,
                         self._hof_hash_alt, fit_d, self._hof_fitness_alt)
        self.hof_hash, self._hof_hash_alt = self._hof_hash_alt, self.hof_hash
        self.hof_fitness, self._hof_fitness_alt = self._hof_fitness_alt, self.hof_fitness
        self.hof_n = int(m)
        self._hof_fit_host = new_fit
        self._up_keep = up
        if side is not None:
            main.wait_stream(side)

    def _pin(self, name: str, n: int, dtype) -> torch.Tensor:
        buf = self._pinned.get(name)
        if buf is None or buf.shape[0] < n or buf.dtype != dtype:
            buf = torch.empty(max(n, 1), dtype=dtype, pin_memory=True)
            self._pinned[name] = buf
        return buf[:n]

    def _keep_on(self, stream):
        if self._next is None:
            return
        for t in self._next[1:]:
            for x in (t if isinstance(t, tuple) else (t,)):
                if isinstance(x, torch.Tensor) and x.is_cuda:
                    x.record_stream(stream)

    def _step_fused(self) -> dict:
        worst = float(self._hof_fit_host[-1]) if (self.H and self.hof_n >= self.H) else None
        if self.generation < 0:
            inv = (~self.valid).to(torch.uint8)
            fit = self._evaluate_fused(0, self._rows, self._deal(inv, 0) if self._balanced() else self._order(inv))
            new_fit, cand, cand_fit, stats, nevals, k = self._merge(fit, inv, self.fitness, worst)
            self.fitness, self.valid = new_fit, torch.ones_like(self.valid)
            self._hof_update_fused(self._rows, cand, cand_fit, k, self.spare,
                                   overlap=lambda: self._next_gen_prep(1, self._rows, new_fit, self.spare))
            if not self._in_place():
                self.store[: self.hof_n] = self.spare[: self.hof_n]
            self.generation = 0
            return self._record(0, nevals, stats)
        g = self.generation + 1
        self._mark(None)
        off = self.spare[self.H:]
        if self._next is None or self._next[0] != g:
            self._next_gen_prep(g, self._rows, self.fitness, self.spare)
        _, inv, inherited, order, sched = self._next
        self._next = None
        self._mark("select_vary")
        fit = self._evaluate_fused(g, off, order, sched)
        new_fit, cand, cand_fit, merged = self._merge_start(fit, inv, inherited, worst)
        early_side = self.side_stream and self.presubmit and not self._balanced()
        cand_pairs = None
        if early_side:
            main = torch.cuda.current_stream(self.device)
            if self._side is None:
                self._side = torch.cuda.Stream(self.device)
            after = merged
            if self._sharded():
                if self.H:
                    if self._iota_P is None:
                        self._iota_P = torch.arange(self.P, dtype=torch.float64, device=self.device)
                    k_dev = self._buf("summary", 8, torch.float64)[6]
                    rows_all = torch.where(self._iota_P < k_dev, cand, torch.full_like(cand, -1))
                else:
                    rows_all = cand[:0]
                cand_pairs = self._complete(g, off, self._rows, rows_all, "cand")
                after = torch.cuda.Event()
                after.record(main)
            self._side.wait_event(after)
            with torch.cuda.stream(self._side):
                self._next_gen_prep(g + 1, off, new_fit, self.store, cand_pairs)
            self._keep_on(main)
        stats, nevals, k = self._merge_finish(merged)
        self._mark("evaluate")
        if self._sharded() and not early_side:
            cand_pairs = self._complete(g, off, self._rows, cand[:k] if self.H else cand[:0], "cand",
                                        exclude=self._dealt.get(g & 1) if self._balanced() else None)
            self._mark("complete", sub=True)
        self._hof_update_fused(off, cand, cand_fit, k, self.spare,
                               overlap=None if early_side else
                               (lambda: self._next_gen_prep(g + 1, off, new_fit, self.store, cand_pairs)))
        if early_side:
            torch.cuda.current_stream(self.device).wait_stream(self._side)
        self._mark("hall_of_fame")
        self.fitness = new_fit
        self.store, self.spare = self.spare, self.store
        self.generation = g
        rec = self._record(g, nevals, stats)
        self._mark("record")
        return rec

    def _prefetch(self, g: int, parents: torch.Tensor, fitness: torch.Tensor, store: torch.Tensor):
        self._next = (g,) + self._select_vary(g, parents, fitness, store[self.H:])

    def _mark(self, phase, sub: bool = False):
        if self.profile is None:
            return
        import time
        torch.cuda.synchronize(self.device)
        now = time.perf_counter()
        if sub:
            self.profile[phase] = self.profile.get(phase, 0.0) + (now - self._t_sub) * 1e3
# ... 25 lines not shown
```

Measured before the change: 13.11 billion.

## Build lane records inline in vary and hof_commit, skip eval prep pass

Builds the per-lane network records (scaled float weights plus certification bound) directly inside the variation kernel for offspring and inside the hall-of-fame commit kernel for opponents. The records are stored in persistent buffers indexed by row, which lets evaluation skip the separate k_prep_records launch (PG_PREP_NONE) and only reset counters. The aim is to remove a full pass that reads the f64 genomes and writes the records before each evaluation. In exchange, vary and commit do extra LDS work per row, and the new validity tracking (_hall_recs_ok) falls back to full prep whenever the records may be stale.

```diff
diff --git a/include/pong_ga.h b/include/pong_ga.h
--- a/include/pong_ga.h
+++ b/include/pong_ga.h
@@ -9,6 +9,7 @@
 #endif
 
 #define PG_ABI_VERSION 13
+#define PG_ABI_REVISION 1
 #define PG_MAX_NODES 9
 
 typedef enum pg_status {
@@ -50,7 +51,8 @@
 typedef enum pg_prep {
   PG_PREP_ALL = 0,
   PG_PREP_GENOMES = 1,
-  PG_PREP_REST = 2
+  PG_PREP_REST = 2      ,
+  PG_PREP_NONE = 3
 } pg_prep;
 
 typedef struct pg_net {
@@ -98,6 +100,8 @@
   int32_t horizon;
   int32_t timeout_thresh;
   int32_t win_score;
+  void *genome_records;
+  void *opponent_records;
 } pg_eval_args;
 
 
@@ -179,6 +183,9 @@
   const int32_t *pair_list;
   const int32_t *pair_count;
   int32_t pair_cap;
+  void *records;
+  pg_net rec_net;
+  int32_t rec_lanes;
 } pg_ga_args;
 
 typedef struct pg_select_args {
@@ -276,11 +283,13 @@
 
 const char *pg_version(void);
 int32_t pg_abi_version(void);
+int32_t pg_abi_revision(void);
 int32_t pg_build_flags(void);
 const char *pg_last_error(void);
 int32_t pg_device_count(void);
 size_t pg_eval_workspace_bytes(const pg_eval_args *args);
 int32_t pg_gene_count(const pg_net *net);
+int32_t pg_record_floats(const pg_net *net, int32_t group_lanes);
 
 int32_t pg_eval_population(const pg_eval_args *args, void *stream);
 int32_t pg_forward(const pg_forward_args *args, void *stream);
@@ -385,6 +394,9 @@
   const double *fitness_in;
   double *new_fitness;
   const int32_t *dst_slot;
+  void *records;
+  pg_net rec_net;
+  int32_t rec_lanes;
 } pg_hof_commit_args;
 int32_t pg_hof_commit(const pg_hof_commit_args *args, void *stream);
 
diff --git a/neuro-genetic-pong-self-play_amd/csrc/pg_cascade.hpp b/neuro-genetic-pong-self-play_amd/csrc/pg_cascade.hpp
--- a/neuro-genetic-pong-self-play_amd/csrc/pg_cascade.hpp
+++ b/neuro-genetic-pong-self-play_amd/csrc/pg_cascade.hpp
@@ -287,6 +287,103 @@
   for (int o = 0; o < O; ++o) n.c[o] = v[P * 14 + P * O * 2 + o];
   n.e = v[P * 14 + P * O * 2 + O];
   n.ct = make_cert(n.e);
+}
+
+__host__ __device__ constexpr int rec_floats_of(int U, int O) {
+  return ((U + 1) / 2 * 2 * (7 + O) + O + 1 + 3) / 4 * 4;
+}
+
+template <bool kFlip, typename RT>
+__device__ __forceinline__ void build_records_wave(const RT *row, int H, int b, int U, int O, float *st, float *rr,
+                                                   float *__restrict__ out, int lane) {
+  constexpr int HL = 4;
+  constexpr float kScaleX = -1.4426950408889634f / 320.f;
+  constexpr float kScaleB = -1.4426950408889634f;
+  const int P = (U + 1) / 2;
+  const int F = rec_floats_of(U, O);
+  const float orf = (float)(P + 2 + 3);
+  const int cols = 6 + b;
+  const long off2 = (long)H * cols;
+#pragma unroll 1
+  for (int t = lane; t < HL * 2 * P; t += 64) {
+    const int hl = t % HL, u = t / HL, p = u >> 1, h = u & 1;
+    const int j = hl + HL * u;
+    const bool ok = u < U && j < H;
+    const int jj = ok ? j : 0;
+    RT raw[7];
+#pragma unroll
+    for (int i = 0; i < 7; ++i) raw[i] = row[(long)jj * cols + ((i < 6 || b) ? i : 0)];
+    float wf[7];
+#pragma unroll
+    for (int i = 0; i < 7; ++i) wf[i] = (float)raw[i] * ((ok && (i < 6 || b)) ? 1.f : 0.f);
+    if (kFlip) {
+      const double bias = (((ok && b) ? (double)raw[6] : 0.0) + (ok ? (double)raw[0] : 0.0)) +
+                          (ok ? (double)raw[2] : 0.0);
+      const float w4 = wf[4];
+      wf[0] = -wf[0];
+      wf[2] = -wf[2];
+      wf[4] = wf[5];
+      wf[5] = w4;
+      wf[6] = (float)bias;
+    }
+    float *s = st + hl * F;
+    float r = 0.f;
+#pragma unroll
+    for (int i = 0; i < 7; ++i) {
+      r += fabsf(wf[i]);
+      s[(p * 7 + i) * 2 + h] = wf[i] * (i < 6 ? kScaleX : kScaleB);
+    }
+    rr[hl * 2 * P + u] = r;
+#pragma unroll
+    for (int o = 0; o < 4; ++o)
+      if (o < O) s[P * 14 + (p * O + o) * 2 + h] = (float)row[off2 + (long)o * (H + b) + jj] * (ok ? 1.f : 0.f);
+  }
+  wave_lds_sync();
+  {
+    const int hl = lane % HL;
+    float *s = st + hl * F;
+    float acc[4] = {0.f, 0.f, 0.f, 0.f};
+    float big = 0.f;
+#pragma unroll 4
+    for (int u = 0; u < 2 * P; ++u) {
+      const int p = u >> 1, h = u & 1;
+      const float r = rr[hl * 2 * P + u];
+      big += r;
+#pragma unroll
+      for (int o = 0; o < 4; ++o)
+        if (o < O) {
+          const float w = s[P * 14 + (p * O + o) * 2 + h];
+          acc[o] += fabsf(w) * (3.f * r + 5.f + orf);
+          big += fabsf(w);
+        }
+    }
+    float c[4] = {0.f, 0.f, 0.f, 0.f};
+#pragma unroll
+    for (int o = 0; o < 4; ++o)
+      if (o < O) {
+        c[o] = (float)row[off2 + (long)o * (H + b) + (b ? H : 0)] * (b ? 1.f : 0.f);
+        big += fabsf(c[o]);
+      }
+    float e = 0.f;
+#pragma unroll
+    for (int o = 0; o < 4; ++o)
+      if (o < O) e = fmaxf(e, 2.f * kU * (group_sum<HL>(acc[o]) + orf * fabsf(c[o])));
+    e = group_sum<HL>(weights_ok(big) ? 0.f : 1.f) > 0.f ? __builtin_inff() : e;
+    if (lane < HL) {
+      const int at = P * 14 + P * O * 2;
+#pragma unroll
+      for (int o = 0; o < 4; ++o)
+        if (o < O) s[at + o] = c[o];
+      s[at + O] = e;
+      for (int f = at + O + 1; f < F; ++f) s[f] = 0.f;
+    }
+  }
+  wave_lds_sync();
+  const float4 *s4 = reinterpret_cast<const float4 *>(st);
+  float4 *d4 = reinterpret_cast<float4 *>(out);
+#pragma unroll 1
+  for (int q = lane; q < HL * F / 4; q += 64) d4[q] = s4[q];
+  wave_lds_sync();
 }
 
 template <int U, int O, bool kBiasIn = false>
diff --git a/neuro-genetic-pong-self-play_amd/csrc/pg_eval.hpp b/neuro-genetic-pong-self-play_amd/csrc/pg_eval.hpp
--- a/neuro-genetic-pong-self-play_amd/csrc/pg_eval.hpp
+++ b/neuro-genetic-pong-self-play_amd/csrc/pg_eval.hpp
@@ -42,6 +42,8 @@
   int nodes[PG_MAX_NODES];
   int n_nodes, bias, max_width;
   float *recs;
+  float *orecs;
+  int rec_rows;
   int horizon;
   int timeout_thresh;
   int win_score;
@@ -97,6 +99,8 @@
 
 int num_cus();
 
+int32_t record_layout(const pg_net &n, int group_lanes, int *L_out, int *U_out);
+
 __device__ inline void log_hard_raw(uint32_t *hard_log, uint64_t *counters, int hard_cap, int row, int is_opp, int idx,
                                     int source, const int k[6]) {
   if (!hard_log || !counters) return;
diff --git a/neuro-genetic-pong-self-play_amd/csrc/pg_gen.hip b/neuro-genetic-pong-self-play_amd/csrc/pg_gen.hip
--- a/neuro-genetic-pong-self-play_amd/csrc/pg_gen.hip
+++ b/neuro-genetic-pong-self-play_amd/csrc/pg_gen.hip
@@ -1,10 +1,12 @@
 #include <hip/hip_runtime.h>
 
 #include <algorithm>
+#include <cstring>
 
 #include <rocprim/device/device_radix_sort.hpp>
 
 #include "pg_eval.hpp"
+#include "pg_cascade.hpp"
 
 
 namespace pg {
@@ -317,20 +319,34 @@
   iota[i] = i;
 }
 
+struct CommitRec {
+  float *recs;
+  int H, b, U, O;
+};
+constexpr int kCommitRecFloats = 4 * rec_floats_of(16, 4) + 4 * 16;
+
 template <typename WT>
 __global__ __launch_bounds__(256) void k_hof_commit(WT *dst, int64_t dst_stride, const WT *old_rows, int64_t old_stride,
                                                     const WT *rows, int64_t rows_stride, const int32_t *cand,
                                                     const int32_t *src, int m, int n_old, int64_t genes,
                                                     const uint64_t *old_hash, const uint64_t *cand_hash,
                                                     uint64_t *new_hash, const double *fit_in, double *new_fitness,
-                                                    const int32_t *dst_slot) {
+                                                    const int32_t *dst_slot, CommitRec cr) {
+  __shared__ float4 rec_lds[4][kCommitRecFloats / 4];
   const int lane = threadIdx.x & 63;
-  for (int j = blockIdx.x * 4 + (threadIdx.x >> 6); j < m; j += gridDim.x * 4) {
-    const int s = src[j];
+  const int wib = __builtin_amdgcn_readfirstlane((int)(threadIdx.x >> 6));
+  for (int j = blockIdx.x * 4 + wib; j < m; j += gridDim.x * 4) {
+    const int s = __builtin_amdgcn_readfirstlane(src[j]);
     if (!dst_slot || s >= n_old) {
       const WT *from = s < n_old ? old_rows + (long)s * old_stride : rows + (long)cand[s - n_old] * rows_stride;
-      WT *to = dst + (long)(dst_slot ? dst_slot[j] : j) * dst_stride;
+      const int slot = dst_slot ? __builtin_amdgcn_readfirstlane(dst_slot[j]) : j;
+      WT *to = dst + (long)slot * dst_stride;
       for (int64_t g = lane; g < genes; g += 64) to[g] = from[g];
+      if (cr.recs) {
+        const int F4 = 4 * rec_floats_of(cr.U, cr.O);
+        float *st = reinterpret_cast<float *>(rec_lds[wib]);
+        build_records_wave<true>(from, cr.H, cr.b, cr.U, cr.O, st, st + F4, cr.recs + (long)slot * F4, lane);
+      }
     }
     if (lane == 0) {
       new_hash[j] = s < n_old ? old_hash[s] : cand_hash[s - n_old];
@@ -502,6 +518,26 @@
       (a->m > 0 && a->n_old > 0 && ((!a->old_rows && !a->dst_slot) || !a->old_hash)) ||
       (a->m > 0 && (!a->rows || !a->cand || !a->cand_hash)))
     return fail(PG_ERR_INVALID, "hof_commit: bad sizes, dtype or NULL buffers");
+  CommitRec cr;
+  memset(&cr, 0, sizeof(cr));
+  if (a->records) {
+    if (!a->dst_slot) return fail(PG_ERR_INVALID, "hof_commit: records need the hall in place (dst_slot)");
+    int L = 0, U = 0;
+    const int32_t rc = record_layout(a->rec_net, a->rec_lanes, &L, &U);
+    if (rc != PG_OK) return rc;
+    if (L != 8)
+      return fail(PG_ERR_UNSUPPORTED, "hof_commit: records are written for the 8-lane split layouts only (H <= 64), not L=%d", L);
+    const int H = a->rec_net.nodes[1], O = a->rec_net.nodes[2], b = a->rec_net.bias ? 1 : 0;
+    if ((int64_t)H * (6 + b) + (int64_t)O * (H + b) != a->genes || a->rec_net.dtype != a->dtype)
+      return fail(PG_ERR_INVALID, "hof_commit: rec_net does not describe rows of %lld genes of dtype %d",
+                  (long long)a->genes, a->dtype);
+    if ((uintptr_t)a->records % 16) return fail(PG_ERR_INVALID, "hof_commit: records must be 16-byte aligned");
+    cr.recs = (float *)a->records;
+    cr.H = H;
+    cr.b = b;
+    cr.U = U;
+    cr.O = O;
+  }
   if (a->m == 0) return PG_OK;
   const hipStream_t s = (hipStream_t)stream;
   const dim3 grid((unsigned)std::min<int64_t>(((int64_t)a->m + 3) / 4, 2048));
@@ -509,12 +545,12 @@
     hipLaunchKernelGGL(k_hof_commit<double>, grid, dim3(256), 0, s, (double *)a->dst, a->dst_stride,
                        (const double *)a->old_rows, a->old_stride, (const double *)a->rows, a->rows_stride, a->cand,
                        a->src, (int)a->m, a->n_old, a->genes, a->old_hash, a->cand_hash,
-                       a->new_hash, a->fitness_in, a->new_fitness, a->dst_slot);
+                       a->new_hash, a->fitness_in, a->new_fitness, a->dst_slot, cr);
   else
     hipLaunchKernelGGL(k_hof_commit<float>, grid, dim3(256), 0, s, (float *)a->dst, a->dst_stride,
                        (const float *)a->old_rows, a->old_stride, (const float *)a->rows, a->rows_stride, a->cand,
                        a->src, (int)a->m, a->n_old, a->genes, a->old_hash, a->cand_hash,
-                       a->new_hash, a->fitness_in, a->new_fitness, a->dst_slot);
+                       a->new_hash, a->fitness_in, a->new_fitness, a->dst_slot, cr);
   PG_HIP(hipGetLastError());
   return PG_OK;
 }
diff --git a/neuro-genetic-pong-self-play_amd/csrc/pg_service.hpp b/neuro-genetic-pong-self-play_amd/csrc/pg_service.hpp
--- a/neuro-genetic-pong-self-play_amd/csrc/pg_service.hpp
+++ b/neuro-genetic-pong-self-play_amd/csrc/pg_service.hpp
@@ -124,6 +124,17 @@
   return d | 256;
 }
 
+constexpr int kRecOpp = 1 << 30;
+template <int HL, int U, int O>
+__device__ __forceinline__ const float *rec_at(const EvalParams &p, int rec) {
+  return ((rec & kRecOpp) ? p.orecs : p.recs) + (long)(rec & ~kRecOpp) * (HL * rec_floats<U, O>());
+}
+
+static __global__ void k_eval_reset(unsigned int *work, uint64_t *counters) {
+  work[threadIdx.x & 63] = 0u;
+  if (counters && threadIdx.x < 16) counters[threadIdx.x] = 0ull;
+}
+
 template <int L, int U, int O, typename WT>
 __global__ __launch_bounds__(256) void k_prep_records(EvalParams p) {
   constexpr int HL = L / 2;
@@ -139,17 +150,21 @@
   if (net >= end) return;
   const WT *g;
   int flip;
+  float *r;
   if (net < p.n_genomes) {
-    if (net >= active_genomes(p)) return;
-    g = (const WT *)p.genomes + (long)genome_row(p, (int)net) * p.gstride;
+    if (!p.rec_rows && net >= active_genomes(p)) return;
+    const int row = genome_row(p, (int)net);
+    g = (const WT *)p.genomes + (long)row * p.gstride;
+    r = p.recs + ((long)(p.rec_rows ? row : (int)net) * HL + hl) * F;
     flip = 0;
   } else {
     g = (const WT *)p.opponents + (net - p.n_genomes) * p.ostride;
+    r = p.orecs + ((net - p.n_genomes) * HL + hl) * F;
     flip = 1;
   }
   NetP<U, O> n;
   load_net_pk<HL, U, O, WT>(n, g, p.nodes[1], p.bias, hl, flip);
-  store_rec<U, O>(n, p.recs + (net * HL + hl) * F);
+  store_rec<U, O>(n, r);
 }
 
 #ifdef PG_PROBE_EXTRA
@@ -379,12 +394,13 @@
       const int i = w / p.n_games;
       const int g = w - i * p.n_games;
       kind = p.kind[w];
-      const WT *gr = genomes + (long)genome_row(p, i) * p.gstride;
+      const int grow = genome_row(p, i);
+      const WT *gr = genomes + (long)grow * p.gstride;
       const bool nn = side && kind == kOppNN && p.n_opponents > 0;
       const int oj = nn ? min(max(p.opp[w], 0), p.n_opponents - 1) : 0;
       gm = nn ? opponents + (long)oj * p.ostride : gr;
-      const int rec = nn ? p.n_genomes + oj : i;
-      load_rec<U, O>(net, p.recs + ((long)rec * HL + hl) * rec_floats<U, O>());
+      const int rec = nn ? kRecOpp | oj : (p.rec_rows ? grow : i);
+      load_rec<U, O>(net, rec_at<HL, U, O>(p, rec) + hl * rec_floats<U, O>());
       const int sx = slot_me();
       if (kInline && hl == 0) slots[sx].rec = rec;
 #pragma unroll
@@ -518,7 +534,7 @@
           for (int i = 0; i < 6; ++i) r.k[i] = __builtin_amdgcn_readlane(kn[i], src);
 #pragma unroll
           for (int i = 0; i < 6; ++i) r.kr[i] = __builtin_amdgcn_readlane(k[i], src);
-          r.rec = p.recs + (long)__builtin_amdgcn_readlane(slots[sx].rec, src) * HL * rec_floats<U, O>();
+          r.rec = rec_at<HL, U, O>(p, __builtin_amdgcn_readlane(slots[sx].rec, src));
 #pragma unroll
           for (int o = O; o < 4; ++o) r.z[o] = 0.f;
 #pragma unroll
@@ -551,9 +567,9 @@
         if constexpr (PG_INLINE_PRIO > 0) __builtin_amdgcn_s_setprio(0);
         {
 #if defined(PG_RELOAD_ALL)
-          load_rec<U, O>(net, p.recs + ((long)slots[sx].rec * HL + hl) * rec_floats<U, O>());
+          load_rec<U, O>(net, rec_at<HL, U, O>(p, slots[sx].rec) + hl * rec_floats<U, O>());
 #elif !defined(PG_NO_RELOAD)
-          load_rec_out<U, O>(net, p.recs + ((long)slots[sx].rec * HL + hl) * rec_floats<U, O>());
+          load_rec_out<U, O>(net, rec_at<HL, U, O>(p, slots[sx].rec) + hl * rec_floats<U, O>());
 #endif
 #ifndef PG_NO_RELOAD
 #pragma unroll
@@ -815,7 +831,9 @@
 }
 
 template <int L, int U, int O, typename WT, bool kSplitTrace = false>
-inline int32_t launch_service(const EvalParams &p, hipStream_t s) {
+inline int32_t launch_service(const EvalParams &p_in, hipStream_t s) {
+  EvalParams p = p_in;
+  if (!p.rec_rows) p.orecs = p.recs ? p.recs + (long)p.n_genomes * (L / 2) * rec_floats<U, O>() : nullptr;
   constexpr int kSvcThreads = svc_threads<U>();
   const bool inl = p.horizon > 0 ? inline_service<L, U, true>() : inline_service<L, U, false>();
   const int GPB = (kSvcThreads / 64 - (inl ? 0 : 1)) * (64 / L);
@@ -827,11 +845,16 @@
   if (!p.recs) return fail(PG_ERR_INVALID, "split kernel: no lane-record workspace");
   if (!kSplitTrace && p.horizon > 0)
     return fail(PG_ERR_UNSUPPORTED, "horizon mode: [6, 33..64, 3] networks on 8-lane groups only");
+  if (p.rec_rows && p.n_opponents > 0 && !p.orecs)
+    return fail(PG_ERR_INVALID, "split kernel: opponents without opponent_records");
   const long nets = p.prep == PG_PREP_GENOMES ? (long)p.n_genomes
                    : (p.prep == PG_PREP_REST ? (long)p.n_opponents : (long)p.n_genomes + p.n_opponents);
   const long prep_threads = nets * (L / 2);
   const unsigned prep_blocks = (unsigned)((prep_threads + 255) / 256);
-  hipLaunchKernelGGL((k_prep_records<L, U, O, WT>), dim3(prep_blocks > 0 ? prep_blocks : 1u), dim3(256), 0, s, p);
+  if (p.prep == PG_PREP_NONE)
+    hipLaunchKernelGGL(k_eval_reset, dim3(1), dim3(64), 0, s, p.work, p.counters);
+  else
+    hipLaunchKernelGGL((k_prep_records<L, U, O, WT>), dim3(prep_blocks > 0 ? prep_blocks : 1u), dim3(256), 0, s, p);
   if (p.prep == PG_PREP_GENOMES) {
     PG_HIP(hipGetLastError());
     return PG_OK;
diff --git a/neuro-genetic-pong-self-play_amd/csrc/pong_ga.hip b/neuro-genetic-pong-self-play_amd/csrc/pong_ga.hip
--- a/neuro-genetic-pong-self-play_amd/csrc/pong_ga.hip
+++ b/neuro-genetic-pong-self-play_amd/csrc/pong_ga.hip
@@ -335,24 +335,34 @@
   return (double)(splitmix64(key ^ b) >> 11) * 0x1.0p-53;
 }
 
-template <typename WT>
-__device__ __forceinline__ void vary_pair(const pg_ga_args &a, int pair);
-
-template <typename WT>
-__global__ __launch_bounds__(256) void k_vary(pg_ga_args a) {
-  const int wave = (int)blockIdx.x * 4 + __builtin_amdgcn_readfirstlane((int)(threadIdx.x >> 6));
+struct VaryRec {
+  int H, b, U, O;
+  int row_floats;
+  int wave_floats;
+};
+
+template <typename WT, bool kRecs>
+__device__ __forceinline__ void vary_pair(const pg_ga_args &a, int pair, const VaryRec &vr, float *lds);
+
+template <typename WT, bool kRecs>
+__global__ __launch_bounds__(256) void k_vary(pg_ga_args a, VaryRec vr) {
+  extern __shared__ float4 vary_lds[];
+  const int wib = __builtin_amdgcn_readfirstlane((int)(threadIdx.x >> 6));
+  const int wave = (int)blockIdx.x * 4 + wib;
+  float *lds = kRecs ? reinterpret_cast<float *>(vary_lds) + wib * vr.wave_floats : nullptr;
   if (a.pair_list) {
     const int count = __builtin_amdgcn_readfirstlane(*a.pair_count);
     const int waves = (int)gridDim.x * 4;
 #pragma unroll 1
-    for (int w = wave; w < count; w += waves) vary_pair<WT>(a, __builtin_amdgcn_readfirstlane(a.pair_list[w]));
+    for (int w = wave; w < count; w += waves)
+      vary_pair<WT, kRecs>(a, __builtin_amdgcn_readfirstlane(a.pair_list[w]), vr, lds);
     return;
   }
-  vary_pair<WT>(a, wave);
-}
-
-template <typename WT>
-__device__ __forceinline__ void vary_pair(const pg_ga_args &a, int pair) {
+  vary_pair<WT, kRecs>(a, wave, vr, lds);
+}
+
+template <typename WT, bool kRecs>
+__device__ __forceinline__ void vary_pair(const pg_ga_args &a, int pair, const VaryRec &vr, float *lds) {
   const int pairs = (a.n + 1) / 2;
   if (pair >= pairs) return;
   const int lane = threadIdx.x & 63;
@@ -397,8 +407,12 @@
     }
     o1[gene] = (WT)x1;
     if (has1) o2[gene] = (WT)x2;
+    if constexpr (kRecs) {
+      lds[gene] = (float)(WT)x1;
+      lds[vr.row_floats + gene] = (float)(WT)x2;
+    }
   };
-  constexpr int kVaryChunk = 4;
+  constexpr int kVaryChunk = kRecs ? 2 : 4;
   for (long g0 = 0; g0 < a.genes; g0 += 128 * kVaryChunk) {
     double x[kVaryChunk][2][2];
 #pragma unroll
@@ -419,6 +433,15 @@
         if (g < a.genes) one(g, x[c][h][0], x[c][h][1]);
       }
     }
+  }
+  if constexpr (kRecs) {
+    wave_lds_sync();
+    const int F4 = 4 * rec_floats_of(vr.U, vr.O);
+    float *st = lds + 2 * vr.row_floats, *rr = st + F4;
+    float *recs = (float *)a.records;
+#pragma unroll 1
+    for (int r = 0; r < (has1 ? 2 : 1); ++r)
+      build_records_wave<false>(lds + r * vr.row_floats, vr.H, vr.b, vr.U, vr.O, st, rr, recs + (long)(i0 + r) * F4, lane);
   }
 }
 
@@ -622,6 +645,18 @@
   return n.n_nodes == 3 && n.nodes[0] == 6 && n.nodes[1] <= 256 && n.nodes[2] >= 2 && n.nodes[2] <= 4;
 }
 
+int32_t record_layout(const pg_net &n, int group_lanes, int *L_out, int *U_out) {
+  if (!resident_shape_ok(n) || n.nodes[1] < 1 || n.activation != PG_ACT_SIGMOID)
+    return fail(PG_ERR_UNSUPPORTED, "lane records need a sigmoid NETWORK_SHAPE [6, H<=256, 2..4]");
+  const int H = n.nodes[1];
+  const int L = group_lanes > 0 ? group_lanes : choose_split_lanes(H);
+  const int U = (L == 8 || L == 16 || L == 32 || L == 64) ? service_units(L, H) : 0;
+  if (U <= 0) return fail(PG_ERR_UNSUPPORTED, "no split layout for H=%d on %d lanes per game", H, L);
+  *L_out = L;
+  *U_out = U;
+  return PG_OK;
+}
+
 }
 
 using namespace pg;
@@ -630,6 +665,7 @@
 
 const char *pg_version(void) { return PG_VERSION_STRING; }
 int32_t pg_abi_version(void) { return PG_ABI_VERSION; }
+int32_t pg_abi_revision(void) { return PG_ABI_REVISION; }
 int32_t pg_build_flags(void) { return 0; }
 const char *pg_last_error(void) { return g_last_error.c_str(); }
 
@@ -686,6 +722,13 @@
   int32_t rc = check_net(*net, false);
   if (rc != PG_OK) return rc;
   return gene_count(*net);
+}
+
+int32_t pg_record_floats(const pg_net *net, int32_t group_lanes) {
+  if (!net) return 0;
+  int L = 0, U = 0;
+  if (check_net(*net, true) != PG_OK || record_layout(*net, group_lanes, &L, &U) != PG_OK) return 0;
+  return (L / 2) * rec_floats_of(U, net->nodes[2]);
 }
 
 int32_t pg_eval_population(const pg_eval_args *a, void *stream) {
@@ -718,7 +761,16 @@
     return fail(PG_ERR_INVALID, "precision=%d", a->precision);
   if (a->trace && (a->trace_games < 0 || a->trace_cap < 1))
     return fail(PG_ERR_INVALID, "trace needs trace_games >= 0 and trace_cap >= 1");
-  if (a->prep < PG_PREP_ALL || a->prep > PG_PREP_REST) return fail(PG_ERR_INVALID, "prep=%d", a->prep);
+  if (a->prep < PG_PREP_ALL || a->prep > PG_PREP_NONE) return fail(PG_ERR_INVALID, "prep=%d", a->prep);
+  const bool own_recs = a->genome_records != nullptr;
+  if (a->opponent_records && !own_recs)
+    return fail(PG_ERR_INVALID, "opponent_records needs genome_records (both or neither)");
+  if (own_recs && a->opponents && a->n_opponents > 0 && !a->opponent_records)
+    return fail(PG_ERR_INVALID, "genome_records needs opponent_records when there are opponents");
+  if (own_recs && ((uintptr_t)a->genome_records % 16 || (uintptr_t)a->opponent_records % 16))
+    return fail(PG_ERR_INVALID, "genome_records and opponent_records must be 16-byte aligned");
+  if (a->prep == PG_PREP_NONE && !own_recs)
+    return fail(PG_ERR_INVALID, "prep=PG_PREP_NONE needs genome_records and opponent_records");
   if (a->net.activation == PG_ACT_RELU) {
     if (a->kernel == PG_KERNEL_SPLIT || a->kernel == PG_KERNEL_WIDE)
       return fail(PG_ERR_UNSUPPORTED, "activation relu: the %s kernel evaluates sigmoid networks only (use RELU or GENERAL)",
@@ -776,6 +828,7 @@
   p.win_score = a->win_score > 0 ? (a->win_score < kDoneScore ? a->win_score : kDoneScore) : kWinScore;
   const int kernel = resolve_kernel(a);
   if (kernel != PG_KERNEL_SPLIT) {
+    if (own_recs) return fail(PG_ERR_UNSUPPORTED, "genome_records: only the split kernel has lane records");
     if (a->prep == PG_PREP_GENOMES) return PG_OK;
     p.prep = PG_PREP_ALL;
     PG_HIP(hipMemsetAsync(a->workspace, 0, 256, s));
@@ -794,6 +847,11 @@
     const int H = a->net.nodes[1];
     const int L = a->group_lanes > 0 ? a->group_lanes : choose_split_lanes(H);
     p.recs = (float *)((char *)a->workspace + eval_base_workspace(a));
+    if (own_recs) {
+      p.recs = (float *)a->genome_records;
+      p.orecs = (float *)a->opponent_records;
+      p.rec_rows = 1;
+    }
     rc = a->net.dtype == PG_F64 ? launch_service_any<double>(p, L, a->net.nodes[2], s)
                                 : launch_service_any<float>(p, L, a->net.nodes[2], s);
     if (rc != PG_OK) return rc;
@@ -1012,11 +1070,37 @@
   int waves = a->pair_list ? (a->pair_cap < pairs ? a->pair_cap : pairs) : pairs;
   if (a->pair_list && waves > kListWaves) waves = kListWaves;
   if (waves == 0) return PG_OK;
+  VaryRec vr;
+  memset(&vr, 0, sizeof(vr));
+  size_t lds = 0;
+  if (a->records) {
+    int L = 0, U = 0;
+    const int32_t rc = record_layout(a->rec_net, a->rec_lanes, &L, &U);
+    if (rc != PG_OK) return rc;
+    if (L != 8)
+      return fail(PG_ERR_UNSUPPORTED, "varAnd: records are written for the 8-lane split layouts only (H <= 64), not L=%d", L);
+    if (gene_count(a->rec_net) != a->genes || a->rec_net.dtype != a->dtype)
+      return fail(PG_ERR_INVALID, "varAnd: rec_net has %d genes of dtype %d, the rows %lld of dtype %d",
+                  gene_count(a->rec_net), a->rec_net.dtype, (long long)a->genes, a->dtype);
+    if ((uintptr_t)a->records % 16) return fail(PG_ERR_INVALID, "varAnd: records must be 16-byte aligned");
+    vr.H = a->rec_net.nodes[1];
+    vr.b = a->rec_net.bias ? 1 : 0;
+    vr.U = U;
+    vr.O = a->rec_net.nodes[2];
+    vr.row_floats = (int)((a->genes + 3) / 4 * 4);
+    vr.wave_floats = 2 * vr.row_floats + 4 * rec_floats_of(U, vr.O) + 4 * 2 * ((U + 1) / 2);
+    lds = (size_t)4 * vr.wave_floats * sizeof(float);
+    if (lds > 64 * 1024) return fail(PG_ERR_UNSUPPORTED, "varAnd: records need %zu bytes of LDS per block", lds);
+  }
   const dim3 grid((unsigned)((waves + 3) / 4));
-  if (a->dtype == PG_F64)
-    hipLaunchKernelGGL(k_vary<double>, grid, dim3(256), 0, (hipStream_t)stream, *a);
+  if (a->records && a->dtype == PG_F64)
+    hipLaunchKernelGGL((k_vary<double, true>), grid, dim3(256), lds, (hipStream_t)stream, *a, vr);
+  else if (a->records)
+    hipLaunchKernelGGL((k_vary<float, true>), grid, dim3(256), lds, (hipStream_t)stream, *a, vr);
+  else if (a->dtype == PG_F64)
+    hipLaunchKernelGGL((k_vary<double, false>), grid, dim3(256), 0, (hipStream_t)stream, *a, vr);
   else
-    hipLaunchKernelGGL(k_vary<float>, grid, dim3(256), 0, (hipStream_t)stream, *a);
+    hipLaunchKernelGGL((k_vary<float, false>), grid, dim3(256), 0, (hipStream_t)stream, *a, vr);
   PG_HIP(hipGetLastError());
   return PG_OK;
 }
diff --git a/neuro-genetic-pong-self-play_amd/pong_amd/_lib.py b/neuro-genetic-pong-self-play_amd/pong_amd/_lib.py
--- a/neuro-genetic-pong-self-play_amd/pong_amd/_lib.py
+++ b/neuro-genetic-pong-self-play_amd/pong_amd/_lib.py
@@ -11,13 +11,14 @@
 HEADER_PATH = os.path.join(REPO_DIR, "include", "pong_ga.h")
 
 PG_ABI_VERSION = 13
+PG_ABI_REVISION = 1
 PG_MAX_NODES = 9
 
 PG_OK, PG_ERR_INVALID, PG_ERR_HIP, PG_ERR_UNSUPPORTED = 0, -1, -2, -3
 PG_F32, PG_F64 = 0, 1
 PG_ACT_SIGMOID, PG_ACT_RELU = 0, 1
 PG_OPP_HARDCODED, PG_OPP_ROM_CPU, PG_OPP_SCORE, PG_OPP_NN = 0, 1, 2, 3
-PG_PREP_ALL, PG_PREP_GENOMES, PG_PREP_REST = 0, 1, 2
+PG_PREP_ALL, PG_PREP_GENOMES, PG_PREP_REST, PG_PREP_NONE = 0, 1, 2, 3
 PG_PREC_CERTIFIED, PG_PREC_F64 = 0, 1
 PG_SCHED_REFERENCE, PG_SCHED_SELFPLAY = 0, 1
 PG_KERNEL_AUTO, PG_KERNEL_GENERAL, PG_KERNEL_RESIDENT, PG_KERNEL_SPLIT, PG_KERNEL_WIDE, PG_KERNEL_STAGED = 0, 1, 2, 3, 4, 5
@@ -55,6 +56,7 @@
         ("n_active", _vp),
         ("prep", ctypes.c_int32), ("horizon", ctypes.c_int32),
         ("timeout_thresh", ctypes.c_int32), ("win_score", ctypes.c_int32),
+        ("genome_records", _vp), ("opponent_records", _vp),
     ]
 
     def __init__(self, *args, **kw):
@@ -101,6 +103,7 @@
         ("mu", ctypes.c_double), ("sigma", ctypes.c_double), ("indpb", ctypes.c_double),
         ("seed", ctypes.c_uint64), ("generation", ctypes.c_uint64), ("pair_mask", _vp),
         ("pair_list", _vp), ("pair_count", _vp), ("pair_cap", ctypes.c_int32),
+        ("records", _vp), ("rec_net", PgNet), ("rec_lanes", ctypes.c_int32),
     ]
 
 
@@ -184,17 +187,20 @@
         ("m", ctypes.c_int32), ("genes", ctypes.c_int64), ("dtype", ctypes.c_int32), ("old_hash", _vp),
         ("cand_hash", _vp), ("new_hash", _vp), ("fitness_in", _vp), ("new_fitness", _vp),
         ("dst_slot", _vp),
+        ("records", _vp), ("rec_net", PgNet), ("rec_lanes", ctypes.c_int32),
     ]
 
 
 SIGNATURES = {
     "pg_version": (ctypes.c_char_p, []),
     "pg_abi_version": (ctypes.c_int32, []),
+    "pg_abi_revision": (ctypes.c_int32, []),
     "pg_build_flags": (ctypes.c_int32, []),
     "pg_last_error": (ctypes.c_char_p, []),
     "pg_device_count": (ctypes.c_int32, []),
     "pg_eval_workspace_bytes": (ctypes.c_size_t, [ctypes.POINTER(PgEvalArgs)]),
     "pg_gene_count": (ctypes.c_int32, [ctypes.POINTER(PgNet)]),
+    "pg_record_floats": (ctypes.c_int32, [ctypes.POINTER(PgNet), ctypes.c_int32]),
     "pg_eval_population": (ctypes.c_int32, [ctypes.POINTER(PgEvalArgs), _vp]),
     "pg_forward": (ctypes.c_int32, [ctypes.POINTER(PgForwardArgs), _vp]),
     "pg_decide": (ctypes.c_int32, [ctypes.POINTER(PgDecideArgs), _vp]),
@@ -259,11 +265,14 @@
                     "(hipcc --offload-arch=gfx950). There is no CPU fallback.")
             L = ctypes.CDLL(LIB_PATH)
             for name, (res, args) in SIGNATURES.items():
-                fn = getattr(L, name)
+                fn = getattr(L, name, None)
+                if fn is None:
+                    raise RuntimeError(f"{LIB_PATH}: {name} missing (an older ABI than {PG_ABI_VERSION}.{PG_ABI_REVISION})")
                 fn.restype = res
                 fn.argtypes = args
-            if L.pg_abi_version() != PG_ABI_VERSION:
-                raise RuntimeError(f"{LIB_PATH}: ABI {L.pg_abi_version()} != {PG_ABI_VERSION}")
+            if (L.pg_abi_version(), L.pg_abi_revision()) != (PG_ABI_VERSION, PG_ABI_REVISION):
+                raise RuntimeError(f"{LIB_PATH}: ABI {L.pg_abi_version()}.{L.pg_abi_revision()} != "
+                                   f"{PG_ABI_VERSION}.{PG_ABI_REVISION}")
             _lib = L
     return _lib
 
diff --git a/neuro-genetic-pong-self-play_amd/pong_amd/device.py b/neuro-genetic-pong-self-play_amd/pong_amd/device.py
--- a/neuro-genetic-pong-self-play_amd/pong_amd/device.py
+++ b/neuro-genetic-pong-self-play_amd/pong_amd/device.py
@@ -9,7 +9,7 @@
 from . import _lib as L
 
 PRECISIONS = {"certified": L.PG_PREC_CERTIFIED, "f64": L.PG_PREC_F64}
-PREPS = {"all": L.PG_PREP_ALL, "genomes": L.PG_PREP_GENOMES, "rest": L.PG_PREP_REST}
+PREPS = {"all": L.PG_PREP_ALL, "genomes": L.PG_PREP_GENOMES, "rest": L.PG_PREP_REST, "none": L.PG_PREP_NONE}
 KERNELS = {"auto": L.PG_KERNEL_AUTO, "general": L.PG_KERNEL_GENERAL, "split": L.PG_KERNEL_SPLIT,
            "wide": L.PG_KERNEL_WIDE, "relu": L.PG_KERNEL_RELU}
 ACTIVATIONS = {"sigmoid": L.PG_ACT_SIGMOID, "relu": L.PG_ACT_RELU}
@@ -89,6 +89,17 @@
         self._ws = None
         self._prep_key = self._prep_ws = None
 
+    def record_floats(self) -> int:
+        if self.precision != "certified" or self.kernel not in ("auto", "split") or self.horizon:
+            return 0
+        return int(L.lib().pg_record_floats(ctypes.byref(self.net), self.group_lanes))
+
+    def records(self, n: int) -> torch.Tensor:
+        f = self.record_floats()
+        if not f:
+            raise ValueError("this evaluator's kernel keeps no lane records")
+        return torch.zeros((int(n), f), dtype=torch.float32, device=self.device)
+
     def selfplay_schedule(self, n: int, n_opponents: int, offset: int = 0):
         dev = self.device
         gi = (torch.arange(n, device=dev, dtype=torch.int64) + offset)[:, None] * self.n_games
@@ -109,7 +120,8 @@
                  out: Optional[EvalResult] = None, precision: Optional[str] = None,
                  kernel: Optional[str] = None, group_lanes: Optional[int] = None, validate: bool = True,
                  hard_log: Optional[torch.Tensor] = None, rows: Optional[torch.Tensor] = None,
-                 n_active: Optional[torch.Tensor] = None, prep: str = "all", horizon: Optional[int] = None):
+                 n_active: Optional[torch.Tensor] = None, prep: str = "all", horizon: Optional[int] = None,
+                 genome_recs: Optional[torch.Tensor] = None, opp_recs: Optional[torch.Tensor] = None):
         dev = self.device
         n = genomes.shape[0] if rows is None else rows.shape[0]
         games = self.n_games
@@ -176,6 +188,19 @@
                 raise ValueError("hard_log must be [cap, 8] int32")
             a.hard_log, a.hard_cap = _ptr(hard_log), hard_log.shape[0]
         a.prep = PREPS[prep]
+        if genome_recs is not None:
+            f = self.record_floats()
+            _need(genome_recs, "genome_recs", torch.float32, dev, (genomes.shape[0], f))
+            a.genome_records = _ptr(genome_recs)
+            if opponents is not None and opponents.shape[0] > 0:
+                if opp_recs is None:
+                    raise ValueError("genome_recs needs opp_recs when there are opponents")
+                _need(opp_recs, "opp_recs", torch.float32, dev)
+                if opp_recs.dim() != 2 or opp_recs.shape[1] != f or opp_recs.shape[0] < opponents.shape[0]:
+                    raise ValueError(f"opp_recs must be [>= {opponents.shape[0]}, {f}]")
+                a.opponent_records = _ptr(opp_recs)
+        elif opp_recs is not None or prep == "none":
+            raise ValueError("opp_recs and prep='none' need genome_recs")
         if prep == "rest" and n and self._prep_key != self._prep_of(genomes, rows, n_active, n):
             raise ValueError("prep='rest' needs a preceding prep='genomes' call with the same genomes, rows, "
                              "n_active and row count on this evaluator")
@@ -359,7 +384,7 @@
 def vary(parents: torch.Tensor, chosen: torch.Tensor, genes: int, cxpb: float, mutpb: float, alpha: float,
          mu: float, sigma: float, indpb: float, seed: int, generation: int, out: Optional[torch.Tensor] = None,
          pair_mask: Optional[torch.Tensor] = None, invalid: Optional[torch.Tensor] = None,
-         pair_list: Optional[tuple] = None):
+         pair_list: Optional[tuple] = None, records: Optional[tuple] = None):
     dev = parents.device
     n = chosen.shape[0]
     _need(chosen, "chosen", torch.int32, dev, (n,))
@@ -382,11 +407,21 @@
         _need(lst, "pair_list", torch.int32, dev)
         _need(cnt, "pair_count", torch.int32, dev, (1,))
         a.pair_list, a.pair_count, a.pair_cap = _ptr(lst), _ptr(cnt), int(min(cap, lst.numel()))
+    if records is not None:
+        a.records, a.rec_net, a.rec_lanes = _rec_args(records, n, dev)
     if out.stride(0) != parents.stride(0):
         raise ValueError("offspring and parents must share the row stride")
     with torch.cuda.device(dev):
         L.check("pg_ga_vary", L.lib().pg_ga_vary(ctypes.byref(a), _stream(dev)))
     return out, invalid
+
+
+def _rec_args(records: tuple, rows: int, dev):
+    buf, ev = records
+    _need(buf, "records", torch.float32, dev)
+    if buf.dim() != 2 or buf.shape[0] < rows or buf.shape[1] != ev.record_floats() or not buf.shape[1]:
+        raise ValueError(f"records must be [>= {rows}, {ev.record_floats()}] f32 of an evaluator with lane records")
+    return _ptr(buf), ev.net, ev.group_lanes
 
 
 def list_pairs(mask: torch.Tensor, out: torch.Tensor, count: torch.Tensor) -> None:
@@ -733,7 +768,7 @@
 def hof_commit(dst: torch.Tensor, old_rows: Optional[torch.Tensor], rows: torch.Tensor, cand: torch.Tensor,
                src: torch.Tensor, n_old: int, genes: int, old_hash: torch.Tensor, cand_hash: torch.Tensor,
                new_hash: torch.Tensor, fitness_in: torch.Tensor, new_fitness: torch.Tensor,
-               dst_slot: Optional[torch.Tensor] = None) -> None:
+               dst_slot: Optional[torch.Tensor] = None, records: Optional[tuple] = None) -> None:
     dev = dst.device
     m = src.shape[0]
     _need(src, "src", torch.int32, dev, (m,))
@@ -755,5 +790,7 @@
                           _ptr(cand), _ptr(src), int(n_old), m, int(genes), DTYPES[dst.dtype], _ptr(old_hash),
                           _ptr(cand_hash), _ptr(new_hash), _ptr(fitness_in), _ptr(new_fitness),
                           _ptr(dst_slot) if dst_slot is not None else None)
+    if records is not None:
+        a.records, a.rec_net, a.rec_lanes = _rec_args(records, dst.shape[0], dev)
     with torch.cuda.device(dev):
         L.check("pg_hof_commit", L.lib().pg_hof_commit(ctypes.byref(a), _stream(dev)))
diff --git a/neuro-genetic-pong-self-play_amd/pong_amd/evolve.py b/neuro-genetic-pong-self-play_amd/pong_amd/evolve.py
--- a/neuro-genetic-pong-self-play_amd/pong_amd/evolve.py
+++ b/neuro-genetic-pong-self-play_amd/pong_amd/evolve.py
@@ -1,5 +1,6 @@
 from __future__ import annotations
 
+import os
 from typing import Optional
 
 import numpy as np
@@ -77,6 +78,10 @@
         self._t_mark = self._t_sub = 0.0
         self._next = None
         self.early_prep = True
+        self.inline_records = os.environ.get("PG_NO_INLINE_RECORDS") != "1"
+        self._genome_recs = self._hall_recs = None
+        self._hall_recs_ok = False
+        self.last_prep = None
         self.hard_log = None
         self.on_evaluate = None
         self.order_by_length = True
@@ -241,6 +246,7 @@
         if genomes is not None:
             self.store[:n] = genomes.to(device=self.device, dtype=self.dtype)
         self._next = None
+        self._hall_recs_ok = False
         self.hof_n = n
         self._hof_fit_host = fit.copy()
         if n and self._hall_buf.data_ptr() != self.store.data_ptr():
@@ -254,6 +260,7 @@
             self.hof_hash[:n] = D.row_hash(self.store[:n], self.G)
 
     def _set_hof_empty(self):
+        self._hall_recs_ok = False
         self.hof_n = 0
         self._hof_fit_host = np.zeros(0, np.float64)
         self._hof_slot_h = np.zeros(0, np.int32)
@@ -319,6 +326,7 @@
         return invalid.bool(), inherited
 
     def _hof_update(self, fit: torch.Tensor, rows: torch.Tensor, dst: torch.Tensor, overlap=None):
+        self._hall_recs_ok = False
         if self.H == 0:
             if overlap:
                 overlap()
@@ -436,6 +444,20 @@
     def _buf(self, name, shape, dtype):
         return self.ws.tensor(name, shape, dtype)
 
+    def _inline(self) -> bool:
+        if not (self.inline_records and self.fused and self._in_place() and self.schedule == "selfplay"
+                and self.world == 1 and not dist.is_initialized() and self.hof_slices == 1):
+            return False
+        if self._genome_recs is None:
+            ev = self.ev
+            f = ev.record_floats()
+            if not f or ev.nodes[1] > 64 or (ev.group_lanes not in (0, 8)):
+                self.inline_records = False
+                return False
+            self._genome_recs = ev.records(self.P)
+            self._hall_recs = ev.records(self.H)
+        return True
+
     def _select(self, g: int, fitness: torch.Tensor) -> torch.Tensor:
         chosen = self._buf("chosen%d" % (g & 1), self.P, torch.int32)
         D.select_ranked(fitness, self.P, self.tournsize, self.seed, g, self.ws, chosen=chosen)
@@ -496,10 +518,12 @@
             prev = self._dealt.get((g - 1) & 1)
             self._complete(g - 1, parents, store[self.H:], chosen, "parents",
                            exclude=cand_pairs if prev is None else (cand_pairs | prev))
+        recs = self._inline() and self.hof_n == self.H
         _, inv = D.vary(parents, chosen, self.G, self.cxpb, self.mutpb, self.alpha, self.mu, self.sigma, self.indpb,
                         seed=self.seed, generation=g, out=store[self.H:],
                         pair_mask=self._shard_mask() if self._sharded() else None,
-                        invalid=self._buf("invalid%d" % (g & 1), self.P, torch.uint8) if self.persistent_bufs else None)
+                        invalid=self._buf("invalid%d" % (g & 1), self.P, torch.uint8) if self.persistent_bufs else None,
+                        records=(self._genome_recs, self.ev) if recs else None)
         inherited = self._buf("inherited", self.P, torch.float64)
         D.inherit(chosen, fitness, inherited, self.lineage_frames, self._lineage_alt)
         self.lineage_frames, self._lineage_alt = self._lineage_alt, self.lineage_frames
@@ -509,15 +533,17 @@
                 self._dealt[g & 1] = self._complete(g, store[self.H:], parents, order[0], "dealt%d" % (g & 1))
         else:
             order = self._order(inv, g)
-        self._next = (g, inv, inherited, order, self._early_prep(g, store[self.H:], order))
-
-    def _early_prep(self, g: int, off: torch.Tensor, order):
+        self._next = (g, inv, inherited, order, self._early_prep(g, store[self.H:], order, recs), recs)
+
+    def _early_prep(self, g: int, off: torch.Tensor, order, inline: bool = False):
         n = self._n_eval
         if (not self.early_prep or self.schedule != "selfplay" or self.H == 0 or self.hof_n != self.H or self.last is None
                 or self.last.fitness.shape[0] != n):
             return None
         local, count = order
         sched = self.eval_schedule(g, n_hof=self.H, rows=local, out=self._sched_bufs(g, n))
+        if inline:
+            return sched
         opponents = self._hall_buf[: self.H] if self._in_place() else self._opponents(self.spare, self.H)
         if self._in_place() and self._sliced(self.H):
             opponents = self._hall_buf[self._slice:self.H:self.hof_slices]
@@ -532,7 +558,7 @@
         D.order(n, self.lo, inv_u8, self.lineage_frames, self.order_by_length, local, count, self.ws)
         return local, count
 
-    def _evaluate_fused(self, g: int, rows: torch.Tensor, order, sched=None) -> torch.Tensor:
+    def _evaluate_fused(self, g: int, rows: torch.Tensor, order, sched=None, recs_current: bool = False) -> torch.Tensor:
         lo, hi = self.lo, self.hi
         n = self._n_eval
         local, count = order
@@ -543,11 +569,21 @@
         opponents = self._opponents(self.store, self.hof_n)
         opp = self._opp_slots(opp, self.hof_n)
         out = self.last if (self.last is not None and self.last.fitness.shape[0] == n) else None
+        inline = self._inline() and self.hof_n == self.H
+        kw = {}
+        if inline:
+            prep = "none" if (recs_current and self._hall_recs_ok) else "all"
+            kw = dict(genome_recs=self._genome_recs, opp_recs=self._hall_recs)
+        else:
+            prep = "all" if (sched is None or recs_current) else "rest"
+            self._hall_recs_ok = False
+        self.last_prep = prep
         if self.eval_events is not None:
             self.eval_events[0].record()
         res, _ = self.ev.evaluate(rows, kind, opp, mult, opponents=opponents, out=out, validate=False,
-                                  hard_log=self.hard_log, rows=local, n_active=count,
-                                  prep="all" if sched is None else "rest")
+                                  hard_log=self.hard_log, rows=local, n_active=count, prep=prep, **kw)
+        if inline:
+            self._hall_recs_ok = True
         if self.eval_events is not None:
             self.eval_events[1].record()
         self.last, self.last_rows, self.last_count = res, local, count
@@ -652,11 +688,15 @@
         src_d, fit_d = up_d[2 * M:2 * M + m], up_d[: 2 * M].view(torch.float64)[:m]
         if in_place:
             slot_d = up_d[3 * M:3 * M + m]
+            recs = self._hall_recs_ok and self._inline()
+            self._hall_recs_ok = recs
             D.hof_commit(self._hall_buf, None, rows, cand, src_d, old_n, self.G, self.hof_hash, cand_hash,
-                         self._hof_hash_alt, fit_d, self._hof_fitness_alt, dst_slot=slot_d)
+                         self._hof_hash_alt, fit_d, self._hof_fitness_alt, dst_slot=slot_d,
+                         records=(self._hall_recs, self.ev) if recs else None)
             self._hof_slot_h = res[2]
             self._slots_identity = False
         else:
+            self._hall_recs_ok = False
             D.hof_commit(dst, self.store, rows, cand, src_d, old_n, self.G, self.hof_hash, cand_hash,
                          self._hof_hash_alt, fit_d, self._hof_fitness_alt)
         self.hof_hash, self._hof_hash_alt = self._hof_hash_alt, self.hof_hash
@@ -700,10 +740,10 @@
         off = self.spare[self.H:]
         if self._next is None or self._next[0] != g:
             self._next_gen_prep(g, self._rows, self.fitness, self.spare)
-        _, inv, inherited, order, sched = self._next
+        _, inv, inherited, order, sched, recs = self._next
         self._next = None
         self._mark("select_vary")
-        fit = self._evaluate_fused(g, off, order, sched)
+        fit = self._evaluate_fused(g, off, order, sched, recs)
         new_fit, cand, cand_fit, merged = self._merge_start(fit, inv, inherited, worst)
         early_side = self.side_stream and self.presubmit and not self._balanced()
         cand_pairs = None
```

Result: faster. 13.41 billion (median of 6 runs) (+2.3%).
